# charles-kmc/Semi-blind-image-deblurring-problems-with-TV

Hardware: AMD Instinct MI355X
Metric: SALSA outer-iters/sec + final PSNR, 2048x2048 Gaussian blur (higher is better)
Workload: dtype f64; 1 GPU; SALSA_v2 TV deblur, one 2048x2048 image per GPU, Gaussian PSF 7x7, BSNR 30 dB, TViters=10; images_per_gpu=1, parallelism=images x1

## Files before the change

semi-blind-image-deblurring-problems-with-tv_amd/csrc/ctx.hip:

```cpp
#include <chrono>
#include <cmath>
#include <cstring>
#include <algorithm>
#include <mutex>
#include <thread>
#include <vector>

#include "sbtv_internal.h"

namespace sbtv {

static std::string g_error;
static std::mutex g_error_mu;

void set_global_error(const std::string &msg) {
    std::lock_guard<std::mutex> lk(g_error_mu);
    g_error = msg;
}

int fail(sbtv_ctx *ctx, int code, const std::string &msg) {
    if (ctx) ctx->err = msg;
    set_global_error(msg);
    return code;
}
// ... 348 lines not shown
    const int rc = init();
    if (rc != 0) {
        const std::string msg = ctx->err;
        (void)sbtv_ctx_destroy(ctx);
        return fail(nullptr, rc, msg);
    }
    *out = ctx;
    return 0;
}

int sbtv_ctx_destroy(sbtv_ctx *ctx) {
    if (!ctx) return 0;
    if (ctx->lanes) (void)sbtv_group_destroy(ctx->lanes);
    ctx->lanes = nullptr;
    (void)hipSetDevice(ctx->device);
    if (ctx->stream) (void)hipStreamSynchronize(ctx->stream);
    for (auto &kv : ctx->ws)
        if (kv.second.base) (void)hipFree(kv.second.base);
    if (ctx->canary_desc) (void)hipFree(ctx->canary_desc);
    if (ctx->canary_bad) (void)hipFree(ctx->canary_bad);
    for (auto &kv : ctx->twiddles) (void)hipFree(kv.second);
    for (auto &kv : ctx->any_axes) (void)hipFree(kv.second);
    if (ctx->pinned) (void)hipHostFree(ctx->pinned);
    for (auto &l : ctx->stage) {
        for (int k = 0; k < 2; ++k) {
            if (l.pin[k]) (void)hipHostFree(l.pin[k]);
            if (l.ev[k]) (void)hipEventDestroy(l.ev[k]);
        }
        if (l.s) (void)hipStreamDestroy(l.s);
    }
    for (auto &ev : ctx->ev)
        if (ev) (void)hipEventDestroy(ev);
    for (auto &ev : ctx->loop_ev)
        if (ev) (void)hipEventDestroy(ev);
    if (ctx->own_stream && ctx->stream) (void)hipStreamDestroy(ctx->stream);
    delete ctx;
    return 0;
}

int sbtv_ctx_set_stream(sbtv_ctx *ctx, void *hip_stream) {
    if (!ctx) return SBTV_ERR_BADARG;
    SBTV_HIP(ctx, hipSetDevice(ctx->device));
    SBTV_HIP(ctx, hipStreamSynchronize(ctx->stream));
    if (hip_stream == nullptr) {
        if (!ctx->own_stream) {
            SBTV_HIP(ctx, hipStreamCreateWithFlags(&ctx->stream, hipStreamNonBlocking));
            ctx->own_stream = true;
        }
        return 0;
    }
    if (ctx->own_stream && ctx->stream) SBTV_HIP(ctx, hipStreamDestroy(ctx->stream));
    ctx->stream = (hipStream_t)hip_stream;
    ctx->own_stream = false;
    return 0;
}

int sbtv_ctx_sync(sbtv_ctx *ctx) {
    if (!ctx) return SBTV_ERR_BADARG;
    SBTV_HIP(ctx, hipStreamSynchronize(ctx->stream));
    return 0;
}

int sbtv_callcounter_get(const sbtv_ctx *ctx, long long *calls) {
    if (!ctx || !calls) return SBTV_ERR_BADARG;
    *calls = ctx->calls;
    return 0;
}

int sbtv_callcounter_reset(sbtv_ctx *ctx) {
    if (!ctx) return SBTV_ERR_BADARG;
    ctx->calls = 0;
    return 0;
}

int sbtv_last_timing(const sbtv_ctx *ctx, double out[4]) {
    if (!ctx || !out) return SBTV_ERR_BADARG;
    for (int i = 0; i < 4; ++i) out[i] = ctx->timing[i];
    return 0;
}

int sbtv_last_host_stats(const sbtv_ctx *ctx, double out[14]) {
    if (!ctx || !out) return SBTV_ERR_BADARG;
    const HostStats &h = ctx->hstat;
    const double v[14] = {h.waits, h.ready_at_once, h.waits_slept, h.sleeps, h.stream_queries,
                          h.wait_s, h.wait_max_s, h.enqueue_s, h.enqueue_max_s, h.wait_max_outer,
                          h.nvcsw, h.nivcsw, h.minflt, h.majflt};
    for (int i = 0; i < 14; ++i) out[i] = v[i];
    return 0;
}

int sbtv_host_transpose(const double *src, double *dst, int batch, int rows, int cols) {
    if (!src || !dst || batch < 0 || rows < 0 || cols < 0) return SBTV_ERR_BADARG;
    constexpr int BS = 64;
    const long long nbr = ((long long)rows + BS - 1) / BS;
    const long long jobs = nbr * batch;
    auto work = [&](int t, int T) {
        for (long long job = t; job < jobs; job += T) {
            const int b = (int)(job / nbr), r0 = (int)(job % nbr) * BS, r1 = std::min(rows, r0 + BS);
            const double *s = src + (size_t)b * rows * cols;
            double *d = dst + (size_t)b * rows * cols;
            for (int c0 = 0; c0 < cols; c0 += BS) {
                const int c1 = std::min(cols, c0 + BS);
                for (int c = c0; c < c1; ++c)
                    for (int r = r0; r < r1; ++r) d[(size_t)c * rows + r] = s[(size_t)r * cols + c];
            }
        }
    };
    const size_t bytes = (size_t)batch * rows * cols * sizeof(double);
    const int T = bytes >= ((size_t)4 << 20) ? 4 : 1;
    std::vector<std::thread> th;
    int started = 1;
    try {
        for (int t = 1; t < T; ++t, ++started) th.emplace_back(work, t, T);
    } catch (...) {
    }
    work(0, T);
    for (auto &x : th) x.join();
    for (int t = started; t < T; ++t) work(t, T);
    return 0;
}

int sbtv_diag_solve_stats(const sbtv_ctx *ctx, double out[4]) {
    if (!ctx || !out) return SBTV_ERR_BADARG;
    for (int i = 0; i < 4; ++i) out[i] = ctx->solve_stats[i];
    if (ctx->lanes)
        for (int r = 0; r < sbtv_group_size(ctx->lanes); ++r)
            for (int i = 0; i < 4; ++i) out[i] += sbtv_group_ctx(ctx->lanes, r)->solve_stats[i];
    return 0;
}

int sbtv_diag_stage_stats(const sbtv_ctx *ctx, double out[4]) {
    if (!ctx || !out) return SBTV_ERR_BADARG;
    for (int i = 0; i < 4; ++i) out[i] = ctx->stage_stats[i];
    if (ctx->lanes)
        for (int r = 0; r < sbtv_group_size(ctx->lanes); ++r)
            for (int i = 0; i < 4; ++i) out[i] += sbtv_group_ctx(ctx->lanes, r)->stage_stats[i];
    return 0;
}

int sbtv_diag_workspace(sbtv_ctx *ctx, const char *name, void **dptr, size_t *bytes) {
    if (!ctx || !name || !dptr) return SBTV_ERR_BADARG;
    auto it = ctx->ws.find(name);
    if (it == ctx->ws.end() || !it->second.p) return fail(ctx, SBTV_ERR_BADARG, std::string("no workspace named '") + name + "'");
    *dptr = it->second.p;
    if (bytes) *bytes = it->second.bytes;
    return 0;
}

int sbtv_diag_switches(char *buf, size_t cap) {
    static const char *const names[] = {
        "SBTV_CANARY", "SBTV_COLLECT_RIDE", "SBTV_EXACT", "SBTV_FFT_WAVE", "SBTV_FISTA_FUSED_STEP", "SBTV_FISTA_LAG",
        "SBTV_FUSED_VARIANT", "SBTV_GRAPH", "SBTV_INLINE_CTRL", "SBTV_PROX_SPEC", "SBTV_SAPG_DEFER",
        "SBTV_SAPG_FUSED_MYULA", "SBTV_SAPG_HOST", "SBTV_SINGLE_STEP", "SBTV_SPIN", "SBTV_TAG_SPIN_US", "SBTV_TILE_ORDER", "SBTV_SALSA_NOX", "SBTV_CSALSA_SPECTRAL",
        "SBTV_CORAL_BATCH", "SBTV_ROWS_FOLD", "SBTV_ERR_SUBSET", "SBTV_LANES", "SBTV_LANE_COUNT", "SBTV_STAGE_THREADS", "SBTV_TEST_FAIL_SAPG", "SBTV_FUSED_STAGGER"};
    if (!buf || cap == 0) return SBTV_ERR_BADARG;
    std::string s;
    int nset = 0;
    for (const char *n : names)
        if (const char *e = getenv(n)) {
            s += (nset++ ? " " : "");
            s += n;
            s += "=";
            s += e;
        }
    if (s.size() + 1 > cap) s.resize(cap - 1);
    memcpy(buf, s.c_str(), s.size() + 1);
    return nset;
}

int sbtv_diag_canary(sbtv_ctx *ctx, int poke, int *enabled, int *nbuf, int *nbad) {
    if (!ctx) return SBTV_ERR_BADARG;
    SBTV_HIP(ctx, hipSetDevice(ctx->device));
    if (enabled) *enabled = ctx->canary ? 1 : 0;
    int nb = 0, bad = 0;
    if (ctx->canary && poke) {
        for (auto &kv : ctx->ws)
            if (kv.second.base) {
                SBTV_HIP(ctx, hipMemsetAsync(static_cast<unsigned char *>(kv.second.p) + kv.second.bytes, 0, 8, ctx->stream));
                break;
            }
    }
    std::string name;
    SBTV_TRY(canary_verify(ctx, &nb, &bad, &name));
    if (ctx->canary && poke && bad) {
        for (auto &kv : ctx->ws)
            if (kv.second.base) {
                SBTV_HIP(ctx, hipMemsetAsync(static_cast<unsigned char *>(kv.second.p) + kv.second.bytes, kGuardByte, kGuard, ctx->stream));
                break;
            }
        SBTV_HIP(ctx, hipStreamSynchronize(ctx->stream));
    }
    if (nbuf) *nbuf = nb;
    if (nbad) *nbad = bad;
    return 0;
}

int sbtv_malloc(sbtv_ctx *ctx, size_t bytes, void **dptr) {
    if (!ctx || !dptr) return SBTV_ERR_BADARG;
    SBTV_HIP(ctx, hipSetDevice(ctx->device));
    SBTV_HIP(ctx, hipMalloc(dptr, bytes));
    return 0;
}

int sbtv_free(sbtv_ctx *ctx, void *dptr) {
    if (!ctx) return SBTV_ERR_BADARG;
    SBTV_HIP(ctx, hipStreamSynchronize(ctx->stream));
    SBTV_HIP(ctx, hipFree(dptr));
    return 0;
}

int sbtv_memcpy_h2d(sbtv_ctx *ctx, void *dst, const void *src, size_t bytes) {
    if (!ctx) return SBTV_ERR_BADARG;
    SBTV_HIP(ctx, hipSetDevice(ctx->device));
    if (stage_threaded(bytes)) {
        SBTV_HIP(ctx, hipStreamSynchronize(ctx->stream));
        return stage_copy(ctx, dst, src, bytes, true);
    }
    SBTV_HIP(ctx, hipMemcpyAsync(dst, src, bytes, hipMemcpyHostToDevice, ctx->stream));
    SBTV_HIP(ctx, hipStreamSynchronize(ctx->stream));
    return 0;
}

int sbtv_memcpy_d2h(sbtv_ctx *ctx, void *dst, const void *src, size_t bytes) {
    if (!ctx) return SBTV_ERR_BADARG;
    SBTV_HIP(ctx, hipSetDevice(ctx->device));
    if (stage_threaded(bytes)) {
        SBTV_HIP(ctx, hipStreamSynchronize(ctx->stream));
        return stage_copy(ctx, dst, src, bytes, false);
    }
    SBTV_HIP(ctx, hipMemcpyAsync(dst, src, bytes, hipMemcpyDeviceToHost, ctx->stream));
    SBTV_HIP(ctx, hipStreamSynchronize(ctx->stream));
    return 0;
}

static double spectral_norm_sq(const double *D, int t) {
    double B[15 * 15];
    for (int i = 0; i < t; ++i)
        for (int j = 0; j < t; ++j) {
            double s = 0.0;
            for (int k = 0; k < t; ++k) s += D[i * t + k] * D[j * t + k];
            B[i * t + j] = s;
        }
    for (int sweep = 0; sweep < 60; ++sweep) {
        double off = 0.0, diag = 0.0;
        for (int i = 0; i < t; ++i)
            for (int j = 0; j < t; ++j) (i == j ? diag : off) += B[i * t + j] * B[i * t + j];
        if (off <= 1e-34 * diag || off == 0.0) break;
        for (int p = 0; p < t - 1; ++p)
            for (int q = p + 1; q < t; ++q) {
                const double apq = B[p * t + q];
                if (apq == 0.0) continue;
                const double theta = (B[q * t + q] - B[p * t + p]) / (2.0 * apq);
                const double tt = (theta >= 0 ? 1.0 : -1.0) / (fabs(theta) + sqrt(theta * theta + 1.0));
                const double cs = 1.0 / sqrt(tt * tt + 1.0), sn = tt * cs;
                for (int k = 0; k < t; ++k) {
                    const double bkp = B[k * t + p], bkq = B[k * t + q];
                    B[k * t + p] = cs * bkp - sn * bkq;
                    B[k * t + q] = sn * bkp + cs * bkq;
                }
                for (int k = 0; k < t; ++k) {
                    const double bpk = B[p * t + k], bqk = B[q * t + k];
                    B[p * t + k] = cs * bpk - sn * bqk;
                    B[q * t + k] = sn * bpk + cs * bqk;
                }
            }
    }
    double mx = 0.0;
    for (int i = 0; i < t; ++i) mx = fmax(mx, B[i * t + i]);
    return mx;
}

int sbtv_err_psf(int kind, int taille, const double *ps, int n, const double *p_true, double phi, double *out) {
    if (kind < 0 || kind > 2 || taille < 1 || taille > 15 || !ps || !p_true || !out || n < 1)
        return fail(nullptr, SBTV_ERR_PSF, "sbtv_err_psf: bad arguments");
    const int t2 = taille * taille;
    double truth[225], cur[225], D[225];
    double pt[3] = {p_true[0], kind == SBTV_PSF_LAPLACE ? 0.0 : p_true[1], kind == SBTV_PSF_GAUSSIAN ? phi : 0.0};
    int rc = sbtv_psf_taps(kind, taille, pt, truth, nullptr, nullptr);
    if (rc != 0) return rc;
    for (int i = 0; i < n; ++i) {
        if (kind == SBTV_PSF_MOFFAT && i == 0) {
            out[0] = 0.0;
            continue;
        }
        double p[3] = {ps[i], 0.0, kind == SBTV_PSF_GAUSSIAN ? phi : 0.0};
        if (kind == SBTV_PSF_GAUSSIAN) p[1] = ps[n + (i > 0 ? i - 1 : 0)];
        if (kind == SBTV_PSF_MOFFAT) p[1] = ps[n + i];
        rc = sbtv_psf_taps(kind, taille, p, cur, nullptr, nullptr);
        if (rc != 0) return rc;
        for (int q = 0; q < t2; ++q) D[q] = cur[q] - truth[q];
        out[i] = spectral_norm_sq(D, taille);
    }
    return 0;
}

int sbtv_psf_taps(int kind, int taille, const double *p, double *taps, double *d0, double *d1) {
    if (taille < 1 || taille > 15 || !p || !taps)
        return fail(nullptr, SBTV_ERR_PSF, "sbtv_psf_taps: bad arguments (1 <= taille <= 15)");
    const int t = taille;
    if (kind != SBTV_PSF_GAUSSIAN && kind != SBTV_PSF_MOFFAT && kind != SBTV_PSF_LAPLACE)
        return fail(nullptr, SBTV_ERR_PSF, "sbtv_psf_taps: unknown PSF kind");
    std::vector<double> f(t * t), e0(t * t, 0.0), e1(t * t, 0.0);
    double s = 0, s0 = 0, s1 = 0;
    for (int q = 0; q < t * t; ++q) psf_taps_point(kind, t, p, q, &f[q], &e0[q], &e1[q]);
    for (int q = 0; q < t * t; ++q) { s += f[q]; s0 += e0[q]; s1 += e1[q]; }
    for (int q = 0; q < t * t; ++q) {
        taps[q] = f[q] / s;
// ... 8 lines not shown
```

semi-blind-image-deblurring-problems-with-tv_amd/csrc/elementwise.hip:

```cpp
#include "sbtv_internal.h"

#pragma clang fp contract(off)

namespace sbtv {

constexpr int EWB = 256;

__device__ __forceinline__ double ew_wave_sum(double v) {
#pragma unroll
    for (int off = 32; off > 0; off >>= 1) v += __shfl_xor(v, off, 64);
    return v;
}

template <int NQ>
__device__ __forceinline__ void ew_block_sum(double (&v)[NQ], double *red ) {
    const int lane = threadIdx.x & 63, w = threadIdx.x >> 6;
#pragma unroll
    for (int c = 0; c < NQ; ++c) {
        const double a = ew_wave_sum(v[c]);
        if (lane == 0) red[c * 4 + w] = a;
    }
    __syncthreads();
    if (threadIdx.x == 0) {
#pragma unroll
        for (int c = 0; c < NQ; ++c) v[c] = (red[c * 4] + red[c * 4 + 1]) + (red[c * 4 + 2] + red[c * 4 + 3]);
    }
}

int ew_blocks(size_t P) {
    size_t nb = (P / 2 + EWB - 1) / EWB;
    if (nb > 1024) nb = 1024;
    if (nb < 1) nb = 1;
    return (int)nb;
}

__global__ __launch_bounds__(EWB) void salsa_zero_start_kernel(const double *__restrict__ y, const double *__restrict__ tru,
                                                                double *__restrict__ x, double *__restrict__ u,
                                                                double *__restrict__ bu, double *__restrict__ accp,
                                                                double *__restrict__ postp, size_t P, double scale) {
    const int b = blockIdx.y;
    __shared__ double red[2 * 4];
    const size_t base = (size_t)b * P;
    double acc[2] = {0, 0};
    for (size_t q = (size_t)blockIdx.x * EWB + threadIdx.x; q < P; q += (size_t)gridDim.x * EWB) {
        const double yv = y[base + q];
        const double tv = tru ? tru[base + q] : 0.0;
        acc[0] += yv * yv;
        acc[1] += tv * tv;
        x[base + q] = 0.0;
        u[base + q] = 0.0;
        bu[base + q] = 0.0;
    }
    ew_block_sum<2>(acc, red);
    if (threadIdx.x == 0) {
        const size_t G = gridDim.x;
        for (int q = 0; q < 3; ++q) accp[((size_t)b * 3 + q) * G + blockIdx.x] = (q == 0) ? acc[0] * scale : 0.0;
        for (int q = 0; q < 6; ++q) postp[((size_t)b * 6 + q) * G + blockIdx.x] = (q == 0) ? acc[1] : 0.0;
    }
}

__global__ __launch_bounds__(EWB) void pair_sums_kernel(const double *__restrict__ a, const double *__restrict__ c,
                                                         double *__restrict__ partials, size_t P) {
    const int b = blockIdx.y;
    __shared__ double red[3 * 4];
    __shared__ double redm[4];
    const size_t base = (size_t)b * P;
    double acc[3] = {0, 0, 0};
    double mx = -1.0e308;
    for (size_t q = (size_t)blockIdx.x * EWB + threadIdx.x; q < P; q += (size_t)gridDim.x * EWB) {
        const double av = a[base + q];
        const double cv = c ? c[base + q] : 0.0;
        const double d = av - cv;
        acc[0] += d * d;
        acc[1] += av * av;
        acc[2] += cv * cv;
        mx = fmax(mx, av);
    }
    for (int off = 32; off > 0; off >>= 1) mx = fmax(mx, __shfl_xor(mx, off, 64));
    if ((threadIdx.x & 63) == 0) redm[threadIdx.x >> 6] = mx;
    ew_block_sum<3>(acc, red);
    if (threadIdx.x == 0) {
        for (int q = 0; q < 3; ++q) partials[((size_t)b * 4 + q) * gridDim.x + blockIdx.x] = acc[q];
        partials[((size_t)b * 4 + 3) * gridDim.x + blockIdx.x] = fmax(fmax(redm[0], redm[1]), fmax(redm[2], redm[3]));
    }
}

__global__ __launch_bounds__(256) void reduce_max_kernel(const double *__restrict__ partials, int n,
                                                          double *__restrict__ out) {
    __shared__ double redm[4];
    const double *p = partials + (size_t)blockIdx.x * n;
    double mx = -1.0e308;
    for (int q = threadIdx.x; q < n; q += 256) mx = fmax(mx, p[q]);
    for (int off = 32; off > 0; off >>= 1) mx = fmax(mx, __shfl_xor(mx, off, 64));
    if ((threadIdx.x & 63) == 0) redm[threadIdx.x >> 6] = mx;
    __syncthreads();
    if (threadIdx.x == 0) out[blockIdx.x] = fmax(fmax(redm[0], redm[1]), fmax(redm[2], redm[3]));
}

__global__ __launch_bounds__(EWB) void axpy_kernel(double *__restrict__ y, const double *__restrict__ gr, double a,
                                                    size_t Ptot, ProxArm arm, int batch) {
    if (arm.ctrl && blockIdx.x == 0 && (int)threadIdx.x < batch) {
        const int b = threadIdx.x;
        ProxCtrl c = arm.ctrl[b];
        c.k = 0;
        c.done = (arm.frozen && arm.frozen[b]) ? 1 : 0;
        c.cur = 0;
        c.maxiter = arm.maxiter;
        c.redo = 0;
        c.f_valid = 0;
        c.err = 0.0;
        c.lambda = arm.lambda[b];
        c.tol = arm.tol;
        c.tau = arm.tau;
        arm.ctrl[b] = c;
    }
    for (size_t q = (size_t)blockIdx.x * EWB + threadIdx.x; q < Ptot / 2; q += (size_t)gridDim.x * EWB) {
        double2 yv = *reinterpret_cast<double2 *>(y + 2 * q);
        const double2 gv = *reinterpret_cast<const double2 *>(gr + 2 * q);
        yv.x = yv.x - a * gv.x;
        yv.y = yv.y - a * gv.y;
        *reinterpret_cast<double2 *>(y + 2 * q) = yv;
    }
}
__global__ __launch_bounds__(EWB) void fista_momentum_kernel(const double *__restrict__ x, const double *__restrict__ xold,
                                                              double *__restrict__ y, const double *__restrict__ tru,
                                                              double c, double *__restrict__ partials, size_t P,
                                                              const int *__restrict__ frozen) {
    const int b = blockIdx.y;
    if (frozen && frozen[b]) return;
    __shared__ double red[3 * 4];
    const size_t base = (size_t)b * P;
    double acc[3] = {0, 0, 0};
    for (size_t q = (size_t)blockIdx.x * EWB + threadIdx.x; q < P / 2; q += (size_t)gridDim.x * EWB) {
        const size_t o = base + 2 * q;
        const double2 xv = *reinterpret_cast<const double2 *>(x + o);
        const double2 xo = *reinterpret_cast<const double2 *>(xold + o);
        const double d0 = xv.x - xo.x, d1 = xv.y - xo.y;
        *reinterpret_cast<double2 *>(y + o) = make_double2(xv.x + c * d0, xv.y + c * d1);
        if (tru) {
            const double2 tv = *reinterpret_cast<const double2 *>(tru + o);
            const double e0 = xv.x - tv.x, e1 = xv.y - tv.y;
            acc[0] += e0 * e0 + e1 * e1;
        }
        acc[1] += d0 * d0 + d1 * d1;
        acc[2] += xv.x * xv.x + xv.y * xv.y;
    }
    ew_block_sum<3>(acc, red);
    if (threadIdx.x == 0)
        for (int q = 0; q < 3; ++q) partials[((size_t)b * 3 + q) * gridDim.x + blockIdx.x] = acc[q];
}

template <bool MOM>
__global__ __launch_bounds__(EWB) void myula_step_kernel(double *__restrict__ X, const double *__restrict__ prox,
                                                          const double *__restrict__ grad,
                                                          const double *__restrict__ Z,
                                                          const double *__restrict__ sigma2, double gam, double lamb,
                                                          double sq2g, size_t P, RngArgs rng, ProxArm arm, MomArgs mom) {
    const int b = blockIdx.y;
    if (arm.ctrl && blockIdx.x == 0 && threadIdx.x == 0) {
        ProxCtrl c = arm.ctrl[b];
        c.k = 0;
        c.done = 0;
        c.cur = 0;
        c.maxiter = arm.maxiter;
        c.redo = 0;
        c.f_valid = 0;
        c.err = 0.0;
        c.lambda = arm.lambda[b];
        c.tol = arm.tol;
        c.tau = arm.tau;
        arm.ctrl[b] = c;
    }
    const size_t base = (size_t)b * P;
    const double s2 = sigma2[b];
    const unsigned step = rng.step_dev ? (unsigned)rng.step_dev[0] : rng.step;
    const int k = MOM ? mom_sample(mom) : 0;
    const double rk = 1.0 / (double)(k > 0 ? k : 1);
    for (size_t q = (size_t)blockIdx.x * EWB + threadIdx.x; q < P / 2; q += (size_t)gridDim.x * EWB) {
        const size_t o = base + 2 * q;
        const double2 xv = *reinterpret_cast<const double2 *>(X + o);
        const double2 pv = *reinterpret_cast<const double2 *>(prox + o);
        const double2 gv = *reinterpret_cast<const double2 *>(grad + o);
        const double2 zv = Z ? *reinterpret_cast<const double2 *>(Z + o)
                             : philox_normal_pair(q, step, rng.chain0 + (unsigned)b, rng.seed);
        double2 r;
        r.x = myula_nocontract(xv.x, pv.x, gv.x, 1.0, zv.x, gam, lamb, s2, sq2g);
        r.y = myula_nocontract(xv.y, pv.y, gv.y, 1.0, zv.y, gam, lamb, s2, sq2g);
        *reinterpret_cast<double2 *>(X + o) = r;
        if (MOM && k > 0) moments_pair(mom, o, r, k, rk);
    }
}

template <bool MOM>
__global__ __launch_bounds__(EWB) void myula_plain_kernel(double *__restrict__ X, const double *__restrict__ prox,
                                                           const double *__restrict__ grad,
                                                           const double *__restrict__ Z,
                                                           const double *__restrict__ sigma2, double gam, double lamb,
                                                           double sq2g, size_t P, RngArgs rng, ProxArm arm, MomArgs mom) {
    const int b = blockIdx.y;
    if (arm.ctrl && blockIdx.x == 0 && threadIdx.x == 0) {
        ProxCtrl c = arm.ctrl[b];
        c.k = 0;
        c.done = 0;
        c.cur = 0;
        c.maxiter = arm.maxiter;
        c.redo = 0;
        c.f_valid = 0;
        c.err = 0.0;
        c.lambda = arm.lambda[b];
        c.tol = arm.tol;
        c.tau = arm.tau;
        arm.ctrl[b] = c;
    }
    const size_t base = (size_t)b * P;
    const double s2 = sigma2[b], keep = 1.0 - gam / lamb;
    const int k = MOM ? mom_sample(mom) : 0;
    const double rk = 1.0 / (double)(k > 0 ? k : 1);
    for (size_t q = (size_t)blockIdx.x * EWB + threadIdx.x; q < P / 2; q += (size_t)gridDim.x * EWB) {
        const size_t o = base + 2 * q;
        const double2 xv = *reinterpret_cast<const double2 *>(X + o);
        const double2 pv = *reinterpret_cast<const double2 *>(prox + o);
        const double2 gv = *reinterpret_cast<const double2 *>(grad + o);
        const double2 zv = Z ? *reinterpret_cast<const double2 *>(Z + o)
                             : philox_normal_pair(q, rng.step, rng.chain0 + (unsigned)b, rng.seed);
        double2 r;
        r.x = (keep * xv.x - gam * (gv.x / s2 - pv.x / lamb)) + sq2g * zv.x;
        r.y = (keep * xv.y - gam * (gv.y / s2 - pv.y / lamb)) + sq2g * zv.y;
        *reinterpret_cast<double2 *>(X + o) = r;
        if (MOM && k > 0) moments_pair(mom, o, r, k, rk);
    }
}

__global__ __launch_bounds__(EWB) void moments_seed_kernel(const double *__restrict__ X, double *__restrict__ mean,
                                                           double *__restrict__ m2, size_t n2) {
    const MomArgs m{mean, m2, 1, nullptr, 1, 1};
    for (size_t q = (size_t)blockIdx.x * EWB + threadIdx.x; q < n2; q += (size_t)gridDim.x * EWB)
        moments_pair(m, 2 * q, *reinterpret_cast<const double2 *>(X + 2 * q), 1, 1.0);
}

__global__ __launch_bounds__(EWB) void moments_finish_kernel(const double *__restrict__ mean, const double *__restrict__ m2,
                                                             size_t P, int batch, double n, int pooled, int raw,
                                                             double *__restrict__ mean_out, double *__restrict__ var_out) {
#pragma clang fp contract(off)
    const int b = blockIdx.y;
    for (size_t i = (size_t)blockIdx.x * EWB + threadIdx.x; i < P; i += (size_t)gridDim.x * EWB) {
        double mu = mean[(size_t)b * P + i], s = m2[(size_t)b * P + i], na = n;
        if (pooled) {
            for (int c = 1; c < batch; ++c) {
                const double mb = mean[(size_t)c * P + i], sb = m2[(size_t)c * P + i];
                const double nt = na + n, d = mb - mu;
                mu = mu + d * (n / nt);
                s = (s + sb) + d * d * (na * n / nt);
                na = nt;
            }
        }
        mean_out[(size_t)b * P + i] = mu;
        if (var_out) var_out[(size_t)b * P + i] = raw ? s : (na > 1.0 ? s / (na - 1.0) : 0.0);
    }
}

int myula_plain_step(sbtv_ctx *ctx, double *X, const double *prox, const double *grad, const double *Z,
                     const double *sigma2_dev, double gam, double lamb, size_t P, int batch, const RngArgs *rng,
                     const ProxArm *arm, const MomArgs *mom) {
    if (!Z && !rng) return fail(ctx, SBTV_ERR_BADARG, "myula_plain_step: neither a noise array nor generator arguments");
    const RngArgs r = rng ? *rng : RngArgs{0ull, 0u, 0u, nullptr};
    const ProxArm pa = arm ? *arm : ProxArm{nullptr, nullptr, 0, 0.0, 0.0, nullptr};
    if (mom)
        hipLaunchKernelGGL(myula_plain_kernel<true>, dim3(ew_blocks(P), batch), dim3(EWB), 0, ctx->stream, X, prox, grad, Z,
                           sigma2_dev, gam, lamb, sqrt(2 * gam), P, r, pa, *mom);
    else
        hipLaunchKernelGGL(myula_plain_kernel<false>, dim3(ew_blocks(P), batch), dim3(EWB), 0, ctx->stream, X, prox, grad, Z,
                           sigma2_dev, gam, lamb, sqrt(2 * gam), P, r, pa, MomArgs{});
    SBTV_HIP(ctx, hipGetLastError());
    return 0;
}

int moments_seed(sbtv_ctx *ctx, const double *X, double *mean, double *m2, size_t P, int batch) {
    const size_t n = P * batch;
    hipLaunchKernelGGL(moments_seed_kernel, dim3(ew_blocks(n)), dim3(EWB), 0, ctx->stream, X, mean, m2, n / 2);
    SBTV_HIP(ctx, hipGetLastError());
    return 0;
}

int moments_finish(sbtv_ctx *ctx, const double *mean, const double *m2, size_t P, int batch, long long n, const MomReq &req) {
    const int pooled = req.pooled && !req.raw;
    const size_t nout = P * (pooled ? 1 : batch);
    double *mo = nullptr, *vo = nullptr;
    const int fl = req.dev ? SBTV_DEVICE_PTRS : SBTV_HOST_PTRS;
    SBTV_TRY(stage_out_buf(ctx, "mom.mean_out", req.mean, nout, fl, &mo));
    if (req.var) SBTV_TRY(stage_out_buf(ctx, "mom.var_out", req.var, nout, fl, &vo));
    hipLaunchKernelGGL(moments_finish_kernel, dim3(ew_blocks(2 * P), pooled ? 1 : batch), dim3(EWB), 0, ctx->stream, mean,
                       m2, P, batch, (double)n, pooled, req.raw ? 1 : 0, mo, vo);
    SBTV_HIP(ctx, hipGetLastError());
    SBTV_TRY(stage_out_copy(ctx, req.mean, mo, nout, fl));
    if (req.var) SBTV_TRY(stage_out_copy(ctx, req.var, vo, nout, fl));
    if (req.count)
        for (size_t c = 0; c < (pooled ? 1 : (size_t)batch); ++c) req.count[c] = pooled ? n * batch : n;
    return 0;
}

int pair_sums(sbtv_ctx *ctx, const double *a, const double *c, size_t P, int batch, double *out4_dev) {
    const int nb = ew_blocks(P);
    double *partials = nullptr;
    SBTV_TRY(ws_get_t(ctx, "ew.pair.partials", (size_t)batch * 4 * nb, &partials));
    hipLaunchKernelGGL(pair_sums_kernel, dim3(nb, batch), dim3(EWB), 0, ctx->stream, a, c, partials, P);
    SBTV_HIP(ctx, hipGetLastError());
    for (int b = 0; b < batch; ++b) {
        SBTV_TRY(reduce_partials(ctx, partials + (size_t)b * 4 * nb, 3, nb, out4_dev + (size_t)b * 4));
        hipLaunchKernelGGL(reduce_max_kernel, dim3(1), dim3(256), 0, ctx->stream, partials + ((size_t)b * 4 + 3) * nb,
                           nb, out4_dev + (size_t)b * 4 + 3);
    }
    SBTV_HIP(ctx, hipGetLastError());
    return 0;
}

int salsa_zero_start(sbtv_ctx *ctx, const double *y, const double *tru, double *x, double *u, double *bu, size_t P, int batch,
                     double scale, double **accp, double **postp, int *nblk) {
    const int G = ew_blocks(2 * P);
    SBTV_TRY(ws_get_t(ctx, "ew.zero.acc", (size_t)batch * 3 * G, accp));
    SBTV_TRY(ws_get_t(ctx, "ew.zero.post", (size_t)batch * 6 * G, postp));
    hipLaunchKernelGGL(salsa_zero_start_kernel, dim3(G, batch), dim3(EWB), 0, ctx->stream, y, tru, x, u, bu, *accp, *postp, P,
                       scale);
    SBTV_HIP(ctx, hipGetLastError());
    *nblk = G;
    return 0;
}

int axpy(sbtv_ctx *ctx, double *y, const double *gr, double a, size_t Ptot, const ProxArm *arm, int batch) {
    if (arm && batch > EWB) return fail(ctx, SBTV_ERR_BADARG, "axpy: cannot arm more than 256 control blocks");
    const ProxArm pa = arm ? *arm : ProxArm{nullptr, nullptr, 0, 0.0, 0.0, nullptr};
    hipLaunchKernelGGL(axpy_kernel, dim3(ew_blocks(Ptot)), dim3(EWB), 0, ctx->stream, y, gr, a, Ptot, pa, batch);
    SBTV_HIP(ctx, hipGetLastError());
    return 0;
}

int fista_momentum(sbtv_ctx *ctx, const double *x, const double *xold, double *y, const double *tru, double coef,
                   double *partials, size_t P, int batch, const int *frozen) {
    hipLaunchKernelGGL(fista_momentum_kernel, dim3(ew_blocks(P), batch), dim3(EWB), 0, ctx->stream, x, xold, y, tru,
                       coef, partials, P, frozen);
    SBTV_HIP(ctx, hipGetLastError());
    return 0;
}

int myula_step(sbtv_ctx *ctx, double *X, const double *prox, const double *grad, const double *Z,
               const double *sigma2_dev, double gam, double lamb, size_t P, int batch, const RngArgs *rng,
               const ProxArm *arm, const MomArgs *mom) {
    if (!Z && !rng) return fail(ctx, SBTV_ERR_BADARG, "myula_step: neither a noise array nor generator arguments");
    const RngArgs r = rng ? *rng : RngArgs{0ull, 0u, 0u, nullptr};
    const ProxArm pa = arm ? *arm : ProxArm{nullptr, nullptr, 0, 0.0, 0.0, nullptr};
    if (mom)
        hipLaunchKernelGGL(myula_step_kernel<true>, dim3(ew_blocks(P), batch), dim3(EWB), 0, ctx->stream, X, prox, grad, Z,
                           sigma2_dev, gam, lamb, sqrt(2 * gam), P, r, pa, *mom);
    else
        hipLaunchKernelGGL(myula_step_kernel<false>, dim3(ew_blocks(P), batch), dim3(EWB), 0, ctx->stream, X, prox, grad, Z,
                           sigma2_dev, gam, lamb, sqrt(2 * gam), P, r, pa, MomArgs{});
    SBTV_HIP(ctx, hipGetLastError());
    return 0;
}

}

using namespace sbtv;

extern "C" {

static int metric_common(sbtv_ctx *ctx, const double *x_true, const double *x, int M, int N, int batch, double *out,
                         int flags, bool psnr) {
    if (!ctx) return SBTV_ERR_BADARG;
    if (!x_true || !x || !out || M < 1 || N < 1 || batch < 1) return fail(ctx, SBTV_ERR_BADARG, "metric: bad arguments");
    SBTV_HIP(ctx, hipSetDevice(ctx->device));
    const size_t P = (size_t)M * N;
    const double *a = nullptr, *c = nullptr;
    SBTV_TRY(stage_in(ctx, "metric.a", x_true, P * batch, flags, &a));
    SBTV_TRY(stage_in(ctx, "metric.c", x, P * batch, flags, &c));
    double *o4 = nullptr;
    SBTV_TRY(ws_get_t(ctx, "metric.out", (size_t)batch * 4, &o4));
    SBTV_TRY(pair_sums(ctx, a, c, P, batch, o4));
    std::vector<double> h((size_t)batch * 4);
    SBTV_HIP(ctx, hipMemcpyAsync(h.data(), o4, sizeof(double) * batch * 4, hipMemcpyDeviceToHost, ctx->stream));
    SBTV_HIP(ctx, hipStreamSynchronize(ctx->stream));
    for (int b = 0; b < batch; ++b) {
        const double se = h[(size_t)b * 4], mx = h[(size_t)b * 4 + 3];
        if (psnr)
            out[b] = 10 * log10(mx * mx) - 10 * log10(se / (double)P);
        else
            out[b] = 10 * log10(se / (double)P);
    }
    return canary_epilogue(ctx, 0);
}

int sbtv_PSNR(sbtv_ctx *ctx, const double *x_true, const double *x, int M, int N, int batch, double *out, int flags) {
    return metric_common(ctx, x_true, x, M, N, batch, out, flags, true);
}
int sbtv_MSE(sbtv_ctx *ctx, const double *x_true, const double *x, int M, int N, int batch, double *out, int flags) {
    return metric_common(ctx, x_true, x, M, N, batch, out, flags, false);
}

}
```

semi-blind-image-deblurring-problems-with-tv_amd/csrc/fft.hip:

```cpp
#include <type_traits>

#include "sbtv_internal.h"

namespace sbtv {

__device__ __forceinline__ double2 cadd(double2 a, double2 b) { return make_double2(a.x + b.x, a.y + b.y); }
__device__ __forceinline__ double2 csub(double2 a, double2 b) { return make_double2(a.x - b.x, a.y - b.y); }
__device__ __forceinline__ double2 cmul(double2 a, double2 b) {
    return make_double2(a.x * b.x - a.y * b.y, a.x * b.y + a.y * b.x);
}
__device__ __forceinline__ double2 cmulc(double2 a, double2 b) {
    return make_double2(a.x * b.x + a.y * b.y, a.y * b.x - a.x * b.y);
}
__device__ __forceinline__ double2 cconj(double2 a) { return make_double2(a.x, -a.y); }
__device__ __forceinline__ double2 cscale(double2 a, double s) { return make_double2(a.x * s, a.y * s); }
__device__ __forceinline__ double cabs2(double2 a) { return a.x * a.x + a.y * a.y; }

constexpr int TWS = 2;
constexpr int TW = 1 << TWS;
__device__ __forceinline__ size_t s_tiled(int k, int l, int n1) {
    return (((size_t)(l >> TWS) * n1 + k) << TWS) + (l & (TW - 1));
}
__device__ __forceinline__ size_t u_tiled(int k, int l, int n1) { return ((size_t)(l >> TWS) * (n1 + 1) + k) * TW + (l & (TW - 1)); }

// ... 839 lines not shown
    hipLaunchKernelGGL((fft_cols_inv_kernel<L, true>), dim3(cd.wgs, pl.batch), dim3(cd.threads), 0,
                       ctx->stream, S, x, pl.tw_n1, pl.tw_M, pl.N, scale, frozen, post);
}

#define SBTV_DISPATCH_LOG2(L, CALL)                                    \
    switch (L) {                                                       \
        case 3: CALL(3); break;                                        \
        case 4: CALL(4); break;                                        \
        case 5: CALL(5); break;                                        \
        case 6: CALL(6); break;                                        \
        case 7: CALL(7); break;                                        \
        case 8: CALL(8); break;                                        \
        case 9: CALL(9); break;                                        \
        case 10: CALL(10); break;                                      \
        case 11: CALL(11); break;                                      \
        default: return fail(ctx, SBTV_ERR_SIZE, "unsupported FFT length"); \
    }

bool fft_cols_tv_ok(const FftPlan &pl) { return !pl.generic; }
int fft_cols_fwd_f(sbtv_ctx *ctx, const FftPlan &pl, const double *x, const double *add, double2 *S,
                   const int *frozen, double *tvp) {
    if (tvp && (!fft_cols_tv_ok(pl) || add)) return fail(ctx, SBTV_ERR_BADARG, "fft_cols_fwd: TV partials not available for this call");
    if (pl.generic) return any_cols_fwd(ctx, pl, x, add, S, frozen);
    if (pl.wave) {
        const PassDims cd = cols_dims(pl);
        const dim3 grid(cd.wgs, pl.batch), block(cd.threads);
        if (pl.n1 == 1024)
            hipLaunchKernelGGL((cols_fwd_wave_kernel<10, 16>), grid, block, 0, ctx->stream, x, add, S, pl.tw_n1, pl.tw_M,
                               pl.N, frozen, tvp);
        else
            hipLaunchKernelGGL((cols_fwd_wave_kernel<9, 8>), grid, block, 0, ctx->stream, x, add, S, pl.tw_n1, pl.tw_M,
                               pl.N, frozen, tvp);
        SBTV_HIP(ctx, hipGetLastError());
        return 0;
    }
    const int L = ilog2(pl.n1);
#define CALL(LL) launch_cols_fwd<LL>(ctx, pl, x, add, S, frozen, tvp)
    SBTV_DISPATCH_LOG2(L, CALL)
#undef CALL
    SBTV_HIP(ctx, hipGetLastError());
    return 0;
}
int fft_cols_fwd(sbtv_ctx *ctx, const FftPlan &pl, const double *x, const double *add, double2 *S) {
    return fft_cols_fwd_f(ctx, pl, x, add, S, nullptr, nullptr);
}

int fft_cols_inv_f(sbtv_ctx *ctx, const FftPlan &pl, const double2 *S, double *x, double scale, const int *frozen) {
    if (pl.generic) return any_cols_inv(ctx, pl, S, x, scale, frozen, nullptr);
    if (pl.wave) {
        const PassDims cd = cols_dims(pl);
        const dim3 grid(cd.wgs, pl.batch), block(cd.threads);
        if (pl.n1 == 1024)
            hipLaunchKernelGGL((cols_inv_wave_kernel<10, 16, 0>), grid, block, 0, ctx->stream, S, x, pl.tw_n1,
                               pl.tw_M, pl.N, scale, frozen, ColsPost{});
        else
            hipLaunchKernelGGL((cols_inv_wave_kernel<9, 8, 0>), grid, block, 0, ctx->stream, S, x, pl.tw_n1, pl.tw_M,
                               pl.N, scale, frozen, ColsPost{});
        SBTV_HIP(ctx, hipGetLastError());
        return 0;
    }
    const int L = ilog2(pl.n1);
#define CALL(LL) launch_cols_inv<LL>(ctx, pl, S, x, scale, frozen)
    SBTV_DISPATCH_LOG2(L, CALL)
#undef CALL
    SBTV_HIP(ctx, hipGetLastError());
    return 0;
}
bool fft_cols_inv_step_ok(const FftPlan &pl) { return !pl.generic && pl.wave; }
static int fft_cols_step_check(sbtv_ctx *ctx, const FftPlan &pl, const char *who) {
    if (!fft_cols_inv_step_ok(pl)) return fail(ctx, SBTV_ERR_BADARG, std::string(who) + ": size not on the wave-granular path");
    return 0;
}
int fft_cols_inv_step(sbtv_ctx *ctx, const FftPlan &pl, const double2 *S, double *y, double scale, double alpha,
                      const int *frozen) {
    SBTV_TRY(fft_cols_step_check(ctx, pl, "fft_cols_inv_step"));
    ColsPost post;
    post.ystep = y;
    post.alpha = alpha;
    const PassDims cd = cols_dims(pl);
        const dim3 grid(cd.wgs, pl.batch), block(cd.threads);
    if (pl.n1 == 1024)
        hipLaunchKernelGGL((cols_inv_wave_kernel<10, 16, 8>), grid, block, 0, ctx->stream, S, (double *)nullptr, pl.tw_n1,
                           pl.tw_M, pl.N, scale, frozen, post);
    else
        hipLaunchKernelGGL((cols_inv_wave_kernel<9, 8, 8>), grid, block, 0, ctx->stream, S, (double *)nullptr, pl.tw_n1, pl.tw_M,
                           pl.N, scale, frozen, post);
    SBTV_HIP(ctx, hipGetLastError());
    return 0;
}
int fft_cols_inv_sub(sbtv_ctx *ctx, const FftPlan &pl, const double2 *S, double *x, double scale, const double *b, double *g) {
    SBTV_TRY(fft_cols_step_check(ctx, pl, "fft_cols_inv_sub"));
    ColsPost post;
    post.bu_in = b;
    post.g = g;
    const PassDims cd = cols_dims(pl);
        const dim3 grid(cd.wgs, pl.batch), block(cd.threads);
    if (pl.n1 == 1024)
        hipLaunchKernelGGL((cols_inv_wave_kernel<10, 16, 64>), grid, block, 0, ctx->stream, S, x, pl.tw_n1, pl.tw_M, pl.N, scale,
                           (const int *)nullptr, post);
    else
        hipLaunchKernelGGL((cols_inv_wave_kernel<9, 8, 64>), grid, block, 0, ctx->stream, S, x, pl.tw_n1, pl.tw_M, pl.N, scale,
                           (const int *)nullptr, post);
    SBTV_HIP(ctx, hipGetLastError());
    return 0;
}
int fft_cols_inv_myula(sbtv_ctx *ctx, const FftPlan &pl, const double2 *S, double scale, double *X, const double *prox,
                       const double *Z, const double *sigma2_dev, double gam, double lamb, const RngArgs *rng,
                       const ProxArm *arm, const MomArgs *mom) {
    SBTV_TRY(fft_cols_step_check(ctx, pl, "fft_cols_inv_myula"));
    if (!Z && !rng) return fail(ctx, SBTV_ERR_BADARG, "fft_cols_inv_myula: neither a noise array nor generator arguments");
    ColsPost post;
    post.ystep = X;
    post.mprox = prox;
    post.mZ = Z;
    post.msig2 = sigma2_dev;
    post.mgam = gam;
    post.mlamb = lamb;
    post.msq2g = sqrt(2 * gam);
    if (rng) post.mrng = *rng;
    if (arm) post.marm = *arm;
    const PassDims cd = cols_dims(pl);
        const dim3 grid(cd.wgs, pl.batch), block(cd.threads);
    if (mom) {
        post.mom = *mom;
        if (pl.n1 == 1024)
            hipLaunchKernelGGL((cols_inv_wave_kernel<10, 16, 16 | 128>), grid, block, 0, ctx->stream, S, (double *)nullptr,
                               pl.tw_n1, pl.tw_M, pl.N, scale, (const int *)nullptr, post);
        else
            hipLaunchKernelGGL((cols_inv_wave_kernel<9, 8, 16 | 128>), grid, block, 0, ctx->stream, S, (double *)nullptr,
                               pl.tw_n1, pl.tw_M, pl.N, scale, (const int *)nullptr, post);
    } else if (pl.n1 == 1024)
        hipLaunchKernelGGL((cols_inv_wave_kernel<10, 16, 16>), grid, block, 0, ctx->stream, S, (double *)nullptr, pl.tw_n1,
                           pl.tw_M, pl.N, scale, (const int *)nullptr, post);
    else
        hipLaunchKernelGGL((cols_inv_wave_kernel<9, 8, 16>), grid, block, 0, ctx->stream, S, (double *)nullptr, pl.tw_n1, pl.tw_M,
                           pl.N, scale, (const int *)nullptr, post);
    SBTV_HIP(ctx, hipGetLastError());
    return 0;
}
int fft_cols_inv(sbtv_ctx *ctx, const FftPlan &pl, const double2 *S, double *x, double scale) {
    return fft_cols_inv_f(ctx, pl, S, x, scale, nullptr);
}
int fft_cols_blocks(const FftPlan &pl) { return (pl.wave || pl.generic) ? pl.N : pl.N / cols_nseq(pl); }
int fft_cols_inv_post(sbtv_ctx *ctx, const FftPlan &pl, const double2 *S, double *x, double scale, const int *frozen,
                      const ColsPost &post) {
    if ((!pl.wave && (post.bu_in || post.skip_x)) || (post.bu_in && !post.skip_x))
        return fail(ctx, SBTV_ERR_BADARG, "fft_cols_inv_post: bu_in + skip_x go together and need the wave-granular column pass");
    if (pl.generic) return any_cols_inv(ctx, pl, S, x, scale, frozen, &post);
    if (pl.wave) {
        const PassDims cd = cols_dims(pl);
        const dim3 grid(cd.wgs, pl.batch), block(cd.threads);
        if (post.skip_x && (!post.bu_in || post.bu_in == post.bu || post.xprev))
            return fail(ctx, SBTV_ERR_BADARG, "fft_cols_inv_post: skip_x needs a separate bu_in and no xprev");
        const int pm = 1 + (post.tru ? 2 : 0) + (post.xprev ? 4 : 0) + (post.skip_x ? 32 : 0);
#define SBTV_POST_CASE(PM_)                                                                                          \
    case PM_:                                                                                                        \
        if (pl.n1 == 1024)                                                                                           \
            hipLaunchKernelGGL((cols_inv_wave_kernel<10, 16, PM_>), grid, block, 0, ctx->stream, S, x, pl.tw_n1,       \
                               pl.tw_M, pl.N, scale, frozen, post);                                                  \
        else                                                                                                         \
            hipLaunchKernelGGL((cols_inv_wave_kernel<9, 8, PM_>), grid, block, 0, ctx->stream, S, x, pl.tw_n1,         \
                               pl.tw_M, pl.N, scale, frozen, post);                                                  \
        break;
        switch (pm) {
            SBTV_POST_CASE(1)
            SBTV_POST_CASE(3)
            SBTV_POST_CASE(5)
            SBTV_POST_CASE(7)
            SBTV_POST_CASE(33)
            SBTV_POST_CASE(35)
        }
#undef SBTV_POST_CASE
        SBTV_HIP(ctx, hipGetLastError());
        return 0;
    }
    const int L = ilog2(pl.n1);
#define CALL(LL) launch_cols_inv_post<LL>(ctx, pl, S, x, scale, frozen, post)
    SBTV_DISPATCH_LOG2(L, CALL)
#undef CALL
    SBTV_HIP(ctx, hipGetLastError());
    return 0;
}

static inline int rows_rk(const FftPlan &pl) {
    const int N = pl.N;
    if (N == 4096) return 2;
    const int rk = (N >= 512) ? 4 : 8;
    const int small = (N == 512) ? 1 : (N == 256) ? 2 : rk;
    return (pl.n1 / rk < 128) ? small : rk;
}
static inline PassDims rows_dims(const FftPlan &pl) {
    if (pl.generic) return {0, ANY_SPEC_THREADS, ANY_SPEC_BLOCKS};
    if (pl.wave) return {4, pl.N / 4, pl.n1 / 4};
    const int rk = rows_rk(pl);
    return {rk, rk * (pl.N / 8), pl.n1 / rk};
}
bool fft_rows_csalsa_ok(const FftPlan &pl) { return !pl.generic; }
static int fft_rows_check(sbtv_ctx *ctx, const FftPlan &pl, int op) {
    if (op == OP_CSALSA && !fft_rows_csalsa_ok(pl)) return fail(ctx, SBTV_ERR_SIZE, "row pass: OP_CSALSA is not built for this plan");
    return 0;
}
int fft_rows_blocks(const FftPlan &pl) {
    return rows_dims(pl).wgs;
}

static inline bool rows_fold_ok(const FftPlan &pl, int shared_spec) {
    static const bool fold_wanted = [] {
        const char *e = getenv("SBTV_ROWS_FOLD");
        return !(e && e[0] == '0');
    }();
    return fold_wanted && pl.wave && shared_spec && pl.batch > 1 && ((pl.n1 / 4) % 8 == 0);
}
template <int L>
static void launch_rows_pipe(sbtv_ctx *ctx, const FftPlan &pl, const RowsParams &p0) {
    RowsParams p = p0;
    const bool fold = rows_fold_ok(pl, p.shared_spec);
    p.fold = fold ? pl.batch : 0;
    const PassDims rd = rows_dims(pl);
    const dim3 grid(fold ? rd.wgs * pl.batch : rd.wgs, fold ? 1 : pl.batch), block(rd.threads);
#define SBTV_ROWS_OP(OP_)                                                                                     \
    case OP_: hipLaunchKernelGGL((rows_pipe_kernel<L, OP_>), grid, block, 0, ctx->stream, p); break;
    switch (p.op) {
        SBTV_ROWS_OP(OP_NONE)
        SBTV_ROWS_OP(OP_MUL_H)
        SBTV_ROWS_OP(OP_MUL_HC)
        SBTV_ROWS_OP(OP_INVLS)
        SBTV_ROWS_OP(OP_SALSA)
        SBTV_ROWS_OP(OP_RESID)
        SBTV_ROWS_OP(OP_GRAD)
        SBTV_ROWS_OP(OP_ATA)
        SBTV_ROWS_OP(OP_GRADF)
        SBTV_ROWS_OP(OP_CSALSA)
        default: break;
    }
#undef SBTV_ROWS_OP
}

template <int L, int RK>
static void launch_rows(sbtv_ctx *ctx, const FftPlan &pl, const RowsParams &p) {
    const PassDims rd = rows_dims(pl);
    const dim3 grid(rd.wgs, pl.batch), block(rd.threads);
#define SBTV_ROWS_OP(OP_)                                                                                     \
    case OP_: hipLaunchKernelGGL((fft_rows_kernel<L, RK, OP_>), grid, block, 0, ctx->stream, p); break;
    switch (p.op) {
        SBTV_ROWS_OP(OP_NONE)
        SBTV_ROWS_OP(OP_MUL_H)
        SBTV_ROWS_OP(OP_MUL_HC)
        SBTV_ROWS_OP(OP_INVLS)
        SBTV_ROWS_OP(OP_SALSA)
        SBTV_ROWS_OP(OP_RESID)
        SBTV_ROWS_OP(OP_GRAD)
        SBTV_ROWS_OP(OP_ATA)
        SBTV_ROWS_OP(OP_GRADF)
        SBTV_ROWS_OP(OP_CSALSA)
        default: break;
    }
#undef SBTV_ROWS_OP
}

int fft_rows(sbtv_ctx *ctx, const FftPlan &pl, const double2 *Sin, double2 *Sout, const RowsArgs &a) {
    RowsParams p;
    p.Sin = Sin;
    p.Sout = Sout;
    p.tw = pl.tw_N;
    p.H = a.H;
    p.Y = a.Y;
    p.D1 = a.D1;
    p.D2 = a.D2;
    p.E = a.E;
    p.cs = a.cs;
    p.mu = a.mu;
    p.acc = a.acc;
    p.frozen = a.frozen;
    p.n1 = pl.n1;
    p.fwd = a.dir_fwd;
    p.inv = a.dir_inv;
    p.op = a.op;
    p.shared_spec = a.shared_spec;
    p.fold = 0;
    p.u_img = pl.u_img;
    p.u_tiled = pl.u_tiled;
    SBTV_TRY(fft_rows_check(ctx, pl, a.op));
    if (pl.generic) return any_rows(ctx, pl, p, Sout);
    const int L = ilog2(pl.N);
    if (L > 12) return fail(ctx, SBTV_ERR_SIZE, "row FFT: N must be <= 4096");
    if (pl.wave) {
        if (L == 11) launch_rows_pipe<11>(ctx, pl, p);
        else launch_rows_pipe<10>(ctx, pl, p);
        SBTV_HIP(ctx, hipGetLastError());
        return 0;
    }
    if (pl.N >= 512) {
        switch (L) {
            case 9:
                if (rows_rk(pl) == 1) launch_rows<9, 1>(ctx, pl, p);
                else launch_rows<9, 4>(ctx, pl, p);
                break;
            case 10: launch_rows<10, 4>(ctx, pl, p); break;
            case 11: launch_rows<11, 4>(ctx, pl, p); break;
            case 12: launch_rows<12, 2>(ctx, pl, p); break;
            default: break;
        }
    } else {
        switch (L) {
            case 4: launch_rows<4, 8>(ctx, pl, p); break;
            case 5: launch_rows<5, 8>(ctx, pl, p); break;
            case 6: launch_rows<6, 8>(ctx, pl, p); break;
            case 7: launch_rows<7, 8>(ctx, pl, p); break;
            case 8:
                if (rows_rk(pl) == 2) launch_rows<8, 2>(ctx, pl, p);
                else launch_rows<8, 8>(ctx, pl, p);
                break;
            default: return fail(ctx, SBTV_ERR_SIZE, "row FFT: N must be >= 16");
        }
    }
    SBTV_HIP(ctx, hipGetLastError());
    return 0;
}

int spec_unpack(sbtv_ctx *ctx, const FftPlan &pl, const double2 *S, double2 *U) {
    if (pl.generic) {
        SBTV_HIP(ctx, hipMemcpyAsync(U, S, sizeof(double2) * pl.s_img * pl.batch, hipMemcpyDeviceToDevice, ctx->stream));
        return 0;
    }
    if (pl.wave) {
        hipLaunchKernelGGL(spec_unpack_tiled_kernel, dim3((pl.N + 63) / 64, pl.n1 + 1, pl.batch), dim3(64), 0,
                           ctx->stream, S, U, pl.n1, pl.N, pl.u_tiled);
        SBTV_HIP(ctx, hipGetLastError());
        return 0;
    }
    const int thr = 64;
    hipLaunchKernelGGL(spec_unpack_kernel, dim3((pl.n1 + 1 + thr - 1) / thr, pl.N, pl.batch), dim3(thr), 0,
                       ctx->stream, S, U, pl.n1, pl.N);
    SBTV_HIP(ctx, hipGetLastError());
    return 0;
}

static inline int psf_lch(const FftPlan &pl) {
    const size_t elems = (size_t)(pl.n1 + 1) * pl.N * pl.batch;
    const int lch = (int)(elems >> 19);
    return lch < 1 ? 1 : (lch > 16 ? 16 : lch);
}
int psf_spectrum_sets(sbtv_ctx *ctx, const FftPlan &pl, const double *const *taps_dev, int taille, double2 *const *U, int nsets) {
    const int thr = 64;
    if (taille > PSF_TMAX) return fail(ctx, SBTV_ERR_PSF, "PSF larger than 15 x 15");
    if (nsets < 1 || nsets > 3) return fail(ctx, SBTV_ERR_BADARG, "psf_spectrum_sets: 1..3 tap sets");
    if (pl.generic) {
        for (int q = 0; q < nsets; ++q) SBTV_TRY(any_psf_spectrum(ctx, pl, taps_dev[q], taille, U[q]));
        return 0;
    }
    const int lch = psf_lch(pl);
    PsfSets ps{};
    for (int q = 0; q < 3; ++q) {
        ps.taps[q] = taps_dev[q < nsets ? q : 0];
        ps.U[q] = U[q < nsets ? q : 0];
    }
    const dim3 grid = pl.u_tiled ? dim3(((pl.n1 + 1) * 4 + thr - 1) / thr, ((pl.N >> 2) + lch - 1) / lch, pl.batch * nsets)
                                 : dim3((pl.n1 + 1 + thr - 1) / thr, (pl.N + lch - 1) / lch, pl.batch * nsets);
    if (taille == 7)
        hipLaunchKernelGGL(psf_spectrum_kernel<7>, grid, dim3(thr), 0, ctx->stream, ps, taille, pl.batch, pl.n1, pl.M, pl.N,
                           pl.tw_M, pl.tw_N, lch, pl.u_tiled);
    else
        hipLaunchKernelGGL(psf_spectrum_kernel<0>, grid, dim3(thr), 0, ctx->stream, ps, taille, pl.batch, pl.n1, pl.M, pl.N,
                           pl.tw_M, pl.tw_N, lch, pl.u_tiled);
    SBTV_HIP(ctx, hipGetLastError());
    return 0;
}
int psf_spectrum(sbtv_ctx *ctx, const FftPlan &pl, const double *taps_dev, int taille, double2 *U) {
    return psf_spectrum_sets(ctx, pl, &taps_dev, taille, &U, 1);
}

}

using namespace sbtv;

extern "C" {

int sbtv_rfft2_packed(sbtv_ctx *ctx, const double *in, double *out, int M, int N, int batch, int inverse, int flags) {
    if (!ctx) return SBTV_ERR_BADARG;
    if (!in || !out || batch < 1) return fail(ctx, SBTV_ERR_BADARG, "rfft2_packed: bad arguments");
    SBTV_HIP(ctx, hipSetDevice(ctx->device));
    FftPlan pl;
    SBTV_TRY(fft_plan(ctx, M, N, batch, &pl));
    if (pl.generic)
        return fail(ctx, SBTV_ERR_SIZE, "rfft2_packed: the packed half-spectrum format exists for powers of two 16..4096 only");
// ... 397 lines not shown
```

semi-blind-image-deblurring-problems-with-tv_amd/csrc/fft_wave.inc:

```


struct SyncWave {
    static __device__ __forceinline__ void sync() {
        __builtin_amdgcn_fence(__ATOMIC_RELEASE, "wavefront");
        __builtin_amdgcn_wave_barrier();
        __builtin_amdgcn_fence(__ATOMIC_ACQUIRE, "wavefront");
    }
};
struct SyncBlock {
    static __device__ __forceinline__ void sync() { __syncthreads(); }
};

template <class SYNC>
struct XSeq {
    double2 *buf;
    static __device__ __forceinline__ int idx(int pos) { return pos + (pos >> 4); }
    static __device__ __forceinline__ void sync() { SYNC::sync(); }
};
template <class SYNC>
struct XSwz {
    double2 *buf;
    static __device__ __forceinline__ int idx(int pos) {
        const int m = pos >> 4;
        return pos ^ ((m & 7) ^ ((m & 4) << 1));
// ... 59 lines not shown
        } else {
            bfly2<INV>(v[q], v[q + G]);
        }
    }
}

template <int V, int LOG2N, int LOG2NS, int LR, bool INV, class TW>
__device__ __forceinline__ void twiddles_v(double2 (&v)[V], int t, TW tw) {
    if constexpr (LOG2NS > 0) {
        constexpr int T = (1 << LOG2N) / V;
        constexpr int R = 1 << LR, G = V / R;
        constexpr int SH = LOG2N - LOG2NS - LR;
#pragma unroll
        for (int q = 0; q < G; ++q) {
            const int k = (t + q * T) & ((1 << LOG2NS) - 1);
            if constexpr (R == 16) {
                const double2 w1 = twid<INV>(tw, k << SH), w2 = twid<INV>(tw, (2 * k) << SH);
                const double2 w4 = twid<INV>(tw, (4 * k) << SH), w8 = twid<INV>(tw, (8 * k) << SH);
                const double2 w3 = cmul(w1, w2), w5 = cmul(w1, w4), w6 = cmul(w2, w4), w7 = cmul(w3, w4);
                v[q + 1 * G] = cmul(v[q + 1 * G], w1);
                v[q + 2 * G] = cmul(v[q + 2 * G], w2);
                v[q + 3 * G] = cmul(v[q + 3 * G], w3);
                v[q + 4 * G] = cmul(v[q + 4 * G], w4);
                v[q + 5 * G] = cmul(v[q + 5 * G], w5);
                v[q + 6 * G] = cmul(v[q + 6 * G], w6);
                v[q + 7 * G] = cmul(v[q + 7 * G], w7);
                v[q + 8 * G] = cmul(v[q + 8 * G], w8);
                v[q + 9 * G] = cmul(v[q + 9 * G], cmul(w1, w8));
                v[q + 10 * G] = cmul(v[q + 10 * G], cmul(w2, w8));
                v[q + 11 * G] = cmul(v[q + 11 * G], cmul(w3, w8));
                v[q + 12 * G] = cmul(v[q + 12 * G], cmul(w4, w8));
                v[q + 13 * G] = cmul(v[q + 13 * G], cmul(w5, w8));
                v[q + 14 * G] = cmul(v[q + 14 * G], cmul(w6, w8));
                v[q + 15 * G] = cmul(v[q + 15 * G], cmul(w7, w8));
            } else {
#pragma unroll
                for (int r = 1; r < R; ++r) v[q + r * G] = cmul(v[q + r * G], twid<INV>(tw, (r * k) << SH));
            }
        }
    }
}

template <int V, int LOG2N, int LOG2NS, int LR, class X>
__device__ __forceinline__ void exchange_v(double2 (&v)[V], int t, const X &x) {
    constexpr int T = (1 << LOG2N) / V;
    constexpr int R = 1 << LR, G = V / R;
#pragma unroll
    for (int q = 0; q < G; ++q) {
        const int j = t + q * T;
        const int k = j & ((1 << LOG2NS) - 1);
        const int j0 = ((j >> LOG2NS) << (LOG2NS + LR)) + k;
#pragma unroll
        for (int r = 0; r < R; ++r) x.buf[X::idx(j0 + (r << LOG2NS))] = v[q + r * G];
    }
    X::sync();
#pragma unroll
    for (int s = 0; s < V; ++s) v[s] = x.buf[X::idx(t + s * T)];
    X::sync();
}

template <int V, int LOG2N, int LOG2NS, bool INV, class X, class TW>
__device__ __forceinline__ void stages_v(double2 (&v)[V], int t, TW tw, const X &x) {
    constexpr int left = LOG2N - LOG2NS;
    constexpr int LV = (V == 16) ? 4 : 3;
    if constexpr (left > 0) {
        constexpr int LR = left >= LV ? LV : left;
        twiddles_v<V, LOG2N, LOG2NS, LR, INV>(v, t, tw);
        butterflies_v<V, LR, INV>(v);
        if constexpr (left - LR > 0) {
            exchange_v<V, LOG2N, LOG2NS, LR>(v, t, x);
            stages_v<V, LOG2N, LOG2NS + LR, INV>(v, t, tw, x);
        }
    }
}

template <int LOG2N, int V>
__global__ __launch_bounds__(64 * TW, 2) void cols_fwd_wave_kernel(const double *__restrict__ x,
                                                                 const double *__restrict__ add,
                                                                 double2 *__restrict__ S,
                                                                 const double2 *__restrict__ tw_n1,
                                                                 const double2 *__restrict__ tw_M, int N,
                                                                 const int *__restrict__ frozen,
                                                                 double *__restrict__ tvp) {
    constexpr int n = 1 << LOG2N;
    static_assert(n == 64 * V, "one wave per column");
    constexpr int REG = xseq_elems(n);
    __shared__ __attribute__((aligned(16))) double2 lds[TW * REG];
    const int b = blockIdx.y;
    if (frozen && frozen[b]) return;
    const int w = __builtin_amdgcn_readfirstlane(threadIdx.x >> 6), lane = threadIdx.x & 63;
    const int tile = blockIdx.x;
    const int j = tile * TW + w;
    const size_t colbase = ((size_t)b * N + j) * n;
    const double2 *__restrict__ xin = reinterpret_cast<const double2 *>(x) + colbase;
    XSeq<SyncWave> X{lds + w * REG};
    double2 v[V];
#pragma unroll
    for (int s = 0; s < V; ++s) v[s] = xin[lane + s * 64];
    if (tvp) {
        constexpr int M = 2 * n;
        const double *__restrict__ xl = x + ((size_t)b * N + (j > 0 ? j - 1 : N - 1)) * M;
        double carry = __shfl(v[V - 1].y, 63, 64);
        double a = 0.0;
#pragma unroll
        for (int s = 0; s < V; ++s) {
            const double2 ul = *reinterpret_cast<const double2 *>(xl + 2 * (size_t)(lane + s * 64));
            double upv = __shfl_up(v[s].y, 1, 64);
            if (lane == 0) upv = carry;
            carry = __shfl(v[s].y, 63, 64);
            const double h0 = v[s].x - ul.x, v0 = v[s].x - upv, h1 = v[s].y - ul.y, v1 = v[s].y - v[s].x;
            a += sqrt(h0 * h0 + v0 * v0) + sqrt(h1 * h1 + v1 * v1);
        }
#pragma unroll
        for (int off = 32; off > 0; off >>= 1) a += __shfl_xor(a, off, 64);
        if (lane == 0) tvp[(size_t)b * N + j] = a;
    }
    if (add) {
        const double2 *__restrict__ ain = reinterpret_cast<const double2 *>(add) + colbase;
#pragma unroll
        for (int s = 0; s < V; ++s) v[s] = cadd(v[s], ain[lane + s * 64]);
    }
    stages_v<V, LOG2N, 0, false>(v, lane, tw_n1, X);
    SyncWave::sync();
#pragma unroll
    for (int s = 0; s < V; ++s) X.buf[XSeq<SyncWave>::idx(lane + s * 64)] = v[s];
    __syncthreads();
    double2 *__restrict__ out = S + ((size_t)b * (N >> TWS) + tile) * ((size_t)n << TWS);
#pragma unroll
    for (int i = 0; i < V; ++i) {
        const int flat = i * (64 * TW) + threadIdx.x;
        const int k = flat >> TWS, c = flat & (TW - 1);
        const double2 *reg = lds + c * REG;
        const double2 Z = reg[XSeq<SyncWave>::idx(k)];
        const double2 Zm = cconj(reg[XSeq<SyncWave>::idx((n - k) & (n - 1))]);
        double2 r;
        if (k == 0) {
            r = make_double2(Z.x + Z.y, Z.x - Z.y);
        } else {
            const double2 wv = tw_M[k];
            const double2 su = cadd(Z, Zm), di = csub(Z, Zm);
            const double2 wd = cmul(wv, di);
            r = make_double2(0.5 * (su.x + wd.y), 0.5 * (su.y - wd.x));
        }
        out[flat] = r;
    }
}

__device__ __forceinline__ double2 step_nocontract(double2 y, double a, double2 x) {
#pragma clang fp contract(off)
    const double t0 = a * x.x, t1 = a * x.y;
    return make_double2(y.x - t0, y.y - t1);
}

template <int LOG2N, int V, int PM>
__global__ __launch_bounds__(64 * TW, 2) void cols_inv_wave_kernel(const double2 *__restrict__ S, double *__restrict__ x,
                                                                 const double2 *__restrict__ tw_n1,
                                                                 const double2 *__restrict__ tw_M, int N, double scale,
                                                                 const int *__restrict__ frozen, ColsPost post) {
    constexpr int n = 1 << LOG2N;
    constexpr bool POST = (PM & 1) != 0, HAS_TRU = (PM & 2) != 0, HAS_XPREV = (PM & 4) != 0;
    constexpr bool NOX = (PM & 32) != 0;
    static_assert(n == 64 * V, "one wave per column");
    constexpr int REG = xseq_elems(n);
    __shared__ __attribute__((aligned(16))) double2 lds[TW * REG];
    const int b = blockIdx.y;
    if (frozen && frozen[b]) return;
    const int w = __builtin_amdgcn_readfirstlane(threadIdx.x >> 6), lane = threadIdx.x & 63;
    const int tile = blockIdx.x;
    const int j = tile * TW + w;
    const double2 *__restrict__ in = S + ((size_t)b * (N >> TWS) + tile) * ((size_t)n << TWS);
    {
        double2 a[V];
#pragma unroll
        for (int i = 0; i < V; ++i) a[i] = in[i * (64 * TW) + threadIdx.x];
#pragma unroll
        for (int i = 0; i < V; ++i) {
            const int flat = i * (64 * TW) + threadIdx.x;
            lds[(flat & (TW - 1)) * REG + XSeq<SyncWave>::idx(flat >> TWS)] = a[i];
        }
    }
    __syncthreads();
    XSeq<SyncWave> X{lds + w * REG};
    double2 v[V];
#pragma unroll
    for (int s = 0; s < V; ++s) {
        const int e = lane + s * 64;
        const double2 Xk = X.buf[XSeq<SyncWave>::idx(e)];
        const double2 Xm = cconj(X.buf[XSeq<SyncWave>::idx((n - e) & (n - 1))]);
        if (e == 0) {
            v[s] = make_double2(0.5 * (Xk.x + Xk.y), 0.5 * (Xk.x - Xk.y));
        } else {
            const double2 E = cscale(cadd(Xk, Xm), 0.5);
            const double2 O = cmulc(cscale(csub(Xk, Xm), 0.5), tw_M[e]);
            v[s] = make_double2(E.x - O.y, E.y + O.x);
        }
        if ((s & 3) == 3) __builtin_amdgcn_sched_barrier(0);
    }
    SyncWave::sync();
    stages_v<V, LOG2N, 0, true>(v, lane, tw_n1, X);
    const size_t colbase = ((size_t)b * N + j) * n;
    double2 *__restrict__ out = reinterpret_cast<double2 *>(x) + colbase;
    if constexpr (PM == 8) {
        double2 *__restrict__ yp = reinterpret_cast<double2 *>(post.ystep) + colbase;
        double2 yv[V];
#pragma unroll
        for (int s = 0; s < V; ++s) yv[s] = yp[lane + s * 64];
#pragma unroll
        for (int s = 0; s < V; ++s) {
            const double2 xv = cscale(v[s], scale);
            yp[lane + s * 64] = step_nocontract(yv[s], post.alpha, xv);
        }
    } else if constexpr ((PM & ~128) == 16) {
        if (post.marm.ctrl && blockIdx.x == 0 && threadIdx.x == 0) {
            ProxCtrl c = post.marm.ctrl[b];
            c.k = 0;
            c.done = 0;
            c.cur = 0;
            c.maxiter = post.marm.maxiter;
            c.redo = 0;
            c.f_valid = 0;
            c.err = 0.0;
            c.lambda = post.marm.lambda[b];
            c.tol = post.marm.tol;
            c.tau = post.marm.tau;
            post.marm.ctrl[b] = c;
        }
        double2 *__restrict__ xp = reinterpret_cast<double2 *>(post.ystep) + colbase;
        const double2 *__restrict__ pp = reinterpret_cast<const double2 *>(post.mprox) + colbase;
        const double2 *__restrict__ zp = post.mZ ? reinterpret_cast<const double2 *>(post.mZ) + colbase : nullptr;
        const double s2 = post.msig2[b];
        const unsigned step = post.mrng.step_dev ? (unsigned)post.mrng.step_dev[0] : post.mrng.step;
        const size_t q0 = (size_t)j * n;
        constexpr bool MOM = (PM & 128) != 0;
        int mk = 0;
        double mrk = 1.0;
        if constexpr (MOM) {
            mk = mom_sample(post.mom);
            mrk = 1.0 / (double)(mk > 0 ? mk : 1);
        }
        constexpr int CH = 4;
#pragma unroll
        for (int c0 = 0; c0 < V; c0 += CH) {
            double2 xv[CH], pv[CH], zv[CH];
#pragma unroll
            for (int q = 0; q < CH; ++q) {
                const int e = lane + (c0 + q) * 64;
                xv[q] = xp[e];
                pv[q] = pp[e];
                if (zp) zv[q] = zp[e];
            }
#pragma unroll
            for (int q = 0; q < CH; ++q) {
                const int e = lane + (c0 + q) * 64;
                if (!zp) zv[q] = philox_normal_pair(q0 + e, step, post.mrng.chain0 + (unsigned)b, post.mrng.seed);
                const double2 gv = cscale(v[c0 + q], scale);
                double2 r;
                r.x = myula_nocontract(xv[q].x, pv[q].x, gv.x, 1.0, zv[q].x, post.mgam, post.mlamb, s2, post.msq2g);
                r.y = myula_nocontract(xv[q].y, pv[q].y, gv.y, 1.0, zv[q].y, post.mgam, post.mlamb, s2, post.msq2g);
                xp[e] = r;
                if constexpr (MOM)
                    if (mk > 0) moments_pair(post.mom, 2 * (colbase + e), r, mk, mrk);
            }
            __builtin_amdgcn_sched_barrier(0);
        }
    } else if constexpr (PM == 64) {
        const double2 *__restrict__ bp = reinterpret_cast<const double2 *>(post.bu_in) + colbase;
        double2 *__restrict__ gp = reinterpret_cast<double2 *>(post.g) + colbase;
        double2 bb[V];
#pragma unroll
        for (int s = 0; s < V; ++s) bb[s] = bp[lane + s * 64];
#pragma unroll
        for (int s = 0; s < V; ++s) {
            const double2 xv = cscale(v[s], scale);
            out[lane + s * 64] = xv;
            gp[lane + s * 64] = make_double2(xv.x - bb[s].x, xv.y - bb[s].y);
        }
    } else if constexpr (!POST) {
#pragma unroll
        for (int s = 0; s < V; ++s) out[lane + s * 64] = cscale(v[s], scale);
    } else {
        constexpr int M = 2 * n;
        const size_t ibase = (size_t)b * N * M;
        const size_t cb = ibase + (size_t)j * M;
        const size_t cl = ibase + (size_t)(j > 0 ? j - 1 : N - 1) * M;
        const double *__restrict__ up_ = post.u + cb + 2 * lane, *__restrict__ ulp = post.u + cl + 2 * lane;
        double *__restrict__ bup = post.bu + cb + 2 * lane, *__restrict__ gp = post.g + cb + 2 * lane;
        const double *__restrict__ bin = NOX ? post.bu_in + cb + 2 * lane : nullptr;
        const double *__restrict__ trp = HAS_TRU ? post.tru + cb + 2 * lane : nullptr;
        const double *__restrict__ xpp = HAS_XPREV ? post.xprev + cb + 2 * lane : nullptr;
        double acc[6] = {0.0, 0.0, 0.0, 0.0, 0.0, 0.0};
        constexpr int CH = 2, NCH = V / CH;
        double2 ub[2][CH], bb[2][CH], tb[2][CH], lb[2][CH], xb[2][CH];
        auto fetch = [&](int c, int slot) {
#pragma unroll
            for (int q = 0; q < CH; ++q) {
                const int off = (c * CH + q) * 128;
                ub[slot][q] = *reinterpret_cast<const double2 *>(up_ + off);
                bb[slot][q] = *reinterpret_cast<const double2 *>((NOX ? bin : (const double *)bup) + off);
                lb[slot][q] = *reinterpret_cast<const double2 *>(ulp + off);
                if constexpr (HAS_TRU) tb[slot][q] = nt_load2(trp + off);
                if constexpr (HAS_XPREV) xb[slot][q] = *reinterpret_cast<const double2 *>(xpp + off);
            }
        };
        __builtin_amdgcn_sched_barrier(0);
        double carry = post.u[cb + M - 1];
        fetch(0, 0);
#pragma unroll
        for (int c = 0; c < NCH; ++c) {
            if (c + 1 < NCH) fetch(c + 1, (c + 1) & 1);
            __builtin_amdgcn_sched_barrier(0);
#pragma unroll
            for (int q = 0; q < CH; ++q) {
                const int s = c * CH + q, off = s * 128;
                const double2 xv = cscale(v[s], scale);
                if constexpr (!NOX) nt_store2(reinterpret_cast<double *>(out + lane + s * 64), xv);
                const double2 uv = ub[c & 1][q], ul = lb[c & 1][q];
                double2 bv = bb[c & 1][q];
                bv.x = bv.x + (uv.x - xv.x);
                bv.y = bv.y + (uv.y - xv.y);
                *reinterpret_cast<double2 *>(bup + off) = bv;
                *reinterpret_cast<double2 *>(gp + off) = make_double2(xv.x - bv.x, xv.y - bv.y);
                if constexpr (HAS_TRU) {
                    const double2 tv = tb[c & 1][q];
                    const double e0 = xv.x - tv.x, e1 = xv.y - tv.y;
                    acc[0] += e0 * e0 + e1 * e1;
                }
                const double d0 = xv.x - uv.x, d1 = xv.y - uv.y;
                acc[1] += d0 * d0 + d1 * d1;
                acc[2] += xv.x * xv.x + xv.y * xv.y;
                acc[3] += uv.x * uv.x + uv.y * uv.y;
                if constexpr (HAS_XPREV) {
                    const double2 xo = xb[c & 1][q];
                    const double p0 = xv.x - xo.x, p1 = xv.y - xo.y;
                    acc[4] += p0 * p0 + p1 * p1;
                }
                double upv = __shfl_up(uv.y, 1, 64);
                if (lane == 0) upv = carry;
                carry = __shfl(uv.y, 63, 64);
                const double h0 = uv.x - ul.x, v0 = uv.x - upv, h1 = uv.y - ul.y, v1 = uv.y - uv.x;
                acc[5] += sqrt(h0 * h0 + v0 * v0) + sqrt(h1 * h1 + v1 * v1);
            }
            __builtin_amdgcn_sched_barrier(0);
        }
#pragma unroll
        for (int c = 0; c < 6; ++c) {
#pragma unroll
            for (int off = 32; off > 0; off >>= 1) acc[c] += __shfl_xor(acc[c], off, 64);
        }
        if (lane == 0) {
#pragma unroll
            for (int c = 0; c < 6; ++c) post.partials[((size_t)b * 6 + c) * N + j] = acc[c];
        }
    }
}

template <int LOG2N, int OP>
__global__ __launch_bounds__((1 << LOG2N) / 4, 1) void rows_pipe_kernel(RowsParams p) {
    constexpr int N = 1 << LOG2N, V = 8, T = N / V, RK = 2, NT = RK * T, NW = NT / 64;
    constexpr int REG = N;
    constexpr bool needH = (OP != OP_NONE);
    constexpr bool CS = (OP == OP_CSALSA);
    constexpr bool needY = (OP == OP_SALSA || OP == OP_RESID || OP == OP_GRADF || OP == OP_GRAD || CS);
    constexpr bool needD = (OP == OP_GRAD);
    constexpr bool needD1 = needD || CS, noAhead = needD || CS;
#ifndef SBTV_CS_LATE_Y
#define SBTV_CS_LATE_Y 1
#endif
    constexpr bool lateY = CS && (SBTV_CS_LATE_Y != 0) && LOG2N == 11;
    __shared__ __attribute__((aligned(16))) double2 lds[RK * REG];
    __shared__ __attribute__((aligned(16))) double2 twl_buf[LdsTw::elems(N)];
    const LdsTw twl{twl_buf};
    __shared__ double red[3 * NW];
    const int fold = p.fold;
    const int ntk = fold ? (int)gridDim.x / fold : (int)gridDim.x;
    int b = blockIdx.y;
    int kb;
    {
        const int bid = blockIdx.x, xx = bid & 7;
        int o = bid >> 3;
        if (fold) {
            b = o % fold;
            o /= fold;
        }
        const int q8 = ntk >> 3, r8 = ntk & 7;
        kb = (xx < r8 ? xx * (q8 + 1) : r8 * (q8 + 1) + (xx - r8) * q8) + o;
    }
    if (p.frozen && p.frozen[b]) return;
    const int q = (threadIdx.x >> 5) & 1, t = (threadIdx.x & 31) | ((threadIdx.x >> 6) << 5);
    const int n1 = p.n1;
    const int k0 = kb * RK + q, k1 = (n1 >> 1) + kb * RK + q;
    const size_t ibase = (size_t)b * n1 * N;
    const double2 *__restrict__ in = p.Sin + ibase;
    double2 *__restrict__ out = p.Sout ? p.Sout + ibase : nullptr;
    XSwz<SyncBlock> X{lds + q * REG};
    const size_t hbase = p.shared_spec ? 0 : (size_t)b * p.u_img;
    const double mu = p.mu ? p.mu[b] : 0.0;
    const double2 z = make_double2(0.0, 0.0);
    const int sb = p.u_tiled ? 1 : n1 + 1, sc = p.u_tiled ? TW : 1;
    auto uidx = [&](int kk, int l) -> size_t {
        return hbase + (size_t)(l >> TWS) * (TW * (n1 + 1)) + (size_t)((l & (TW - 1)) * sb + kk * sc);
    };
    for (int i = threadIdx.x; i < N; i += NT) twl_buf[LdsTw::idx(i)] = p.tw[i];
    __syncthreads();

    double2 v[V], sn[V], h[V], y[V], d1[needD1 ? V : 1], d2[needD ? V : 1];
    if constexpr (!needD1) d1[0] = z;
    const CsPar cp = CS ? CsPar{p.cs[0], p.cs[1], p.cs[2]} : CsPar{0.0, 0.0, 0.0};
    auto apply = [&](double2 V_, double2 H_, double2 Y_, double2 &E_, double2 D2_, double wgt, double (&acc_)[3]) -> double2 {
        if constexpr (CS) return spec_apply_cs(V_, H_, Y_, E_, mu, cp, wgt, acc_);
        else return spec_apply<OP>(V_, H_, Y_, E_, D2_, mu, wgt, acc_);
    };
    auto dd1 = [&](int s) -> double2 & { return d1[needD1 ? s : 0]; };
    auto dd2 = [&](int s) -> double2 { return needD ? d2[needD ? s : 0] : z; };
#pragma unroll
    for (int s = 0; s < V; ++s) v[s] = in[s_tiled(k0, t + s * T, n1)];
    if constexpr (needH) {
#pragma unroll
        for (int s = 0; s < V; ++s) {
            h[s] = p.H[uidx(k0, t + s * T)];
            if constexpr (needY && !lateY) y[s] = p.Y[uidx(k0, t + s * T)];
            if constexpr (needD) {
                d1[s] = p.D1[uidx(k0, t + s * T)];
                d2[s] = p.D2[uidx(k0, t + s * T)];
            }
            if constexpr (CS) d1[s] = p.E[uidx(k0, t + s * T)];
        }
    }
    if constexpr (!noAhead) {
#pragma unroll
        for (int s = 0; s < V; ++s) sn[s] = in[s_tiled(k1, t + s * T, n1)];
    }
    double acc[3] = {0.0, 0.0, 0.0};

    if (p.fwd) stages_v<V, LOG2N, 0, false>(v, t, twl, X);
    if constexpr (lateY) {
#pragma unroll
        for (int s = 0; s < V; ++s) y[s] = p.Y[uidx(k0, t + s * T)];
    }
    if constexpr (needH) {
        if (kb == 0) {
#pragma unroll
            for (int s = 0; s < V; ++s) X.buf[XSwz<SyncBlock>::idx(t + s * T)] = v[s];
            SyncBlock::sync();
#pragma unroll
            for (int s = 0; s < V; ++s) {
                const int l = t + s * T;
                if (q == 0) {
                    const size_t hn = uidx(n1, l);
                    const double2 P = v[s], Q = cconj(X.buf[XSwz<SyncBlock>::idx((N - l) & (N - 1))]);
                    const double2 A = cscale(cadd(P, Q), 0.5);
                    const double2 dB = csub(P, Q);
                    const double2 B = make_double2(0.5 * dB.y, -0.5 * dB.x);
                    double2 en = needD ? p.D1[hn] : (CS ? p.E[hn] : z);
                    const double2 A2 = apply(A, h[s], needY ? y[s] : z, dd1(s), dd2(s), 1.0, acc);
                    const double2 B2 = apply(B, p.H[hn], needY ? p.Y[hn] : z, en, needD ? p.D2[hn] : z, 1.0, acc);
                    if constexpr (CS) p.E[hn] = en;
                    v[s] = make_double2(A2.x - B2.y, A2.y + B2.x);
                } else {
                    v[s] = apply(v[s], h[s], needY ? y[s] : z, dd1(s), dd2(s), 2.0, acc);
                }
                if constexpr (CS) p.E[uidx(k0, t + s * T)] = d1[s];
            }
            SyncBlock::sync();
        } else {
#pragma unroll
            for (int s = 0; s < V; ++s) {
                v[s] = apply(v[s], h[s], needY ? y[s] : z, dd1(s), dd2(s), 2.0, acc);
                if constexpr (CS) p.E[uidx(k0, t + s * T)] = d1[s];
            }
        }
        asm volatile("" : "+v"(acc[0]), "+v"(acc[1]), "+v"(acc[2]));
#pragma unroll
        for (int s = 0; s < V; ++s) {
            h[s] = p.H[uidx(k1, t + s * T)];
            if constexpr (needY && !lateY) y[s] = p.Y[uidx(k1, t + s * T)];
            if constexpr (needD) {
                d1[s] = p.D1[uidx(k1, t + s * T)];
                d2[s] = p.D2[uidx(k1, t + s * T)];
            }
            if constexpr (CS) d1[s] = p.E[uidx(k1, t + s * T)];
        }
    }
    if (p.inv) stages_v<V, LOG2N, 0, true>(v, t, twl, X);
    int ts = t;
    asm volatile("" : "+v"(ts));
    if (out) {
#pragma unroll
        for (int s = 0; s < V; ++s) out[s_tiled(k0, ts + s * T, n1)] = v[s];
    }
#pragma unroll
    for (int s = 0; s < V; ++s) v[s] = noAhead ? in[s_tiled(k1, t + s * T, n1)] : sn[s];
    if (p.fwd) stages_v<V, LOG2N, 0, false>(v, t, twl, X);
    if constexpr (lateY) {
#pragma unroll
        for (int s = 0; s < V; ++s) y[s] = p.Y[uidx(k1, t + s * T)];
    }
    if constexpr (needH) {
#pragma unroll
        for (int s = 0; s < V; ++s) {
            v[s] = apply(v[s], h[s], needY ? y[s] : z, dd1(s), dd2(s), 2.0, acc);
            if constexpr (CS) p.E[uidx(k1, t + s * T)] = d1[s];
        }
        asm volatile("" : "+v"(acc[0]), "+v"(acc[1]), "+v"(acc[2]));
    }
    if (p.inv) stages_v<V, LOG2N, 0, true>(v, t, twl, X);
    asm volatile("" : "+v"(ts));
    if (out) {
#pragma unroll
        for (int s = 0; s < V; ++s) out[s_tiled(k1, ts + s * T, n1)] = v[s];
    }
    if constexpr (needY) {
        const int lane = threadIdx.x & 63, w = threadIdx.x >> 6;
#pragma unroll
        for (int c = 0; c < 3; ++c) {
#pragma unroll
            for (int off = 32; off > 0; off >>= 1) acc[c] += __shfl_xor(acc[c], off, 64);
        }
        if (lane == 0) {
#pragma unroll
            for (int c = 0; c < 3; ++c) red[c * NW + w] = acc[c];
        }
        __syncthreads();
        if (threadIdx.x < 3) {
            double a = 0.0;
            for (int ww = 0; ww < NW; ++ww) a += red[threadIdx.x * NW + ww];
            p.acc[((size_t)b * 3 + threadIdx.x) * ntk + kb] = a;
        }
    }
}

__global__ void s_relayout_kernel(const double2 *__restrict__ in, double2 *__restrict__ out, int n1, int N, int to_tiled) {
    const size_t per = (size_t)n1 * N;
    const double2 *ib = in + (size_t)blockIdx.y * per;
    double2 *ob = out + (size_t)blockIdx.y * per;
    for (size_t q = (size_t)blockIdx.x * blockDim.x + threadIdx.x; q < per; q += (size_t)gridDim.x * blockDim.x) {
        const int c = (int)(q & (TW - 1));
        const size_t rest = q >> TWS;
        const int k = (int)(rest % n1), lt = (int)(rest / n1);
        const size_t plain = (size_t)(lt * TW + c) * n1 + k;
        if (to_tiled) ob[q] = ib[plain];
        else ob[plain] = ib[q];
    }
}

__global__ void spec_unpack_tiled_kernel(const double2 *__restrict__ S, double2 *__restrict__ U, int n1, int N, int utiled) {
    const int b = blockIdx.z;
    const int l = blockIdx.x * blockDim.x + threadIdx.x;
    const int k = blockIdx.y;
    if (l >= N) return;
    const double2 *s = S + (size_t)b * n1 * N;
    double2 *u = U + (size_t)b * (n1 + 1) * N;
    double2 r;
    if (k == 0 || k == n1) {
        const double2 P = s[s_tiled(0, l, n1)];
        const double2 Q = cconj(s[s_tiled(0, (N - l) & (N - 1), n1)]);
        if (k == 0) {
            r = cscale(cadd(P, Q), 0.5);
        } else {
            const double2 d = csub(P, Q);
            r = make_double2(0.5 * d.y, -0.5 * d.x);
        }
    } else {
        r = s[s_tiled(k, l, n1)];
    }
    if (utiled) u[u_tiled(k, l, n1)] = r;
    else u[(size_t)l * (n1 + 1) + k] = r;
}
```

semi-blind-image-deblurring-problems-with-tv_amd/csrc/salsa.hip:

```cpp
#include <algorithm>
#include <chrono>
#include <cmath>

#include <time.h>

#include "sbtv_internal.h"

namespace sbtv {

__global__ void salsa_setup_kernel(const double *__restrict__ src, double *__restrict__ par, int npar, int *__restrict__ frozen,
                                   int batch) {
    for (int i = threadIdx.x; i < npar; i += blockDim.x) par[i] = src[i];
    for (int b = threadIdx.x; b < batch; b += blockDim.x) frozen[b] = 0;
}

__global__ __launch_bounds__(256) void salsa_recover_x_kernel(const double *__restrict__ g, const double *__restrict__ bu,
                                                               double *__restrict__ x, size_t P) {
#pragma clang fp contract(off)
    for (size_t q = (size_t)blockIdx.x * 256 + threadIdx.x; q < P / 2; q += (size_t)gridDim.x * 256) {
        const double2 a = *reinterpret_cast<const double2 *>(g + 2 * q), b = *reinterpret_cast<const double2 *>(bu + 2 * q);
        *reinterpret_cast<double2 *>(x + 2 * q) = make_double2(a.x + b.x, a.y + b.y);
    }
}

__global__ __launch_bounds__(256) void salsa_collect_kernel(Collect c, ProxCtrl *__restrict__ ctrl,
                                                             unsigned long long out_addr,
                                                             const int *__restrict__ frozen, int rearm,
                                                             unsigned long long tags_addr, double seq) {
    __shared__ double red[4];
    salsa_collect_block(c, ctrl, out_addr, frozen, rearm, tags_addr, seq, blockIdx.x, blockIdx.y, red);
}

}

using namespace sbtv;

extern "C" {

void sbtv_salsa_opts_default(sbtv_salsa_opts *o) {
    if (!o) return;
    o->stopcriterion = 1;
    o->maxiter = 10000;
    o->TViters = 5;
    o->initialization = 0;
    o->compute_mse = 0;
    o->speculate = 1;
    o->tolA = 0.001;
    o->chambolle_tol = 1e-3;
    o->chambolle_tau = 0.249;
}

}

namespace {

struct SalsaRun {
    sbtv_ctx *ctx; const double *yd; int M, N, batch; const double *taps; int taille; const double *tau, *mu;
    const sbtv_salsa_opts *opts; const double *td, *xi; double *x_out, *objective, *distance, *times, *mses;
    int *numA, *numAt, *n_outer; int flags; bool spec_wanted;

    BlurOp op{};
    ProxPlan pp;
    size_t P = 0, cnt = 0, npar = 0;
    int maxiter = 0, lag = 0, nrb = 0, npb = 0, nl_prox = 0;
    bool want_mse = false, crit2 = false, zero_start = false, direct_last_ok = false, direct_last = false, nox = false,
         spec_ok = false, use_graph = false;
    double *xbuf[2] = {nullptr, nullptr}, *u = nullptr, *gb[2] = {nullptr, nullptr}, *bub[2] = {nullptr, nullptr};
    double *par = nullptr, *taps_d = nullptr, *mu_d = nullptr, *thr_d = nullptr;
    double *acc = nullptr, *postp = nullptr, *o4 = nullptr;
    int *frozen_d = nullptr;
    SalsaScal *scal_h = nullptr, *scal_hd = nullptr, *init_h = nullptr, *init_hd = nullptr;
    double *psum_h = nullptr, *psum_hd = nullptr, *tags_h = nullptr, *tags_hd = nullptr, *init_tags_h = nullptr,
           *init_tags_hd = nullptr;
    int *frozen_h = nullptr;
    hipEvent_t ev_done[2], ev_p0[2], ev_p1[2];

    std::vector<int> h_numA, h_numAt, frozen, h_nouter;
    std::vector<double> obj_prev;
    bool init_read = false;
    int active = 0;
    double ms_prox = 0.0;
    long long prox_iters_run = 0, prox_iters_timed = 0;
    GraphExecs graphs;
    std::chrono::steady_clock::time_point t0;
    bool prox_timed[2] = {false, false}, slot_tagged[2] = {false, false}, slot_spec[2] = {false, false};
    struct PendingCollect {
        bool valid = false;
        int outer = 0;
        bool spec = false;
    } pend;

    int open() {
        SBTV_TRY(op_open(ctx, "salsa", M, N, batch, "Y", &op));
        SBTV_TRY(prox_plan(ctx, M, N, batch, &pp));
        P = op.P;
        cnt = P * batch;
        maxiter = opts->maxiter;
        want_mse = (td != nullptr);
        crit2 = (opts->stopcriterion == 2);
        zero_start = (opts->initialization == 0);
        lag = (opts->speculate & 1) ? 1 : 0;
        SBTV_TRY(ws_get_t(ctx, "salsa.x0", cnt, &xbuf[0]));
        SBTV_TRY(ws_get_t(ctx, "salsa.x1", cnt, &xbuf[1]));
        direct_last_ok = x_out && (flags & SBTV_DEVICE_PTRS) && !graph_wanted(cnt) && !overlaps(yd, x_out, cnt) &&
                         !overlaps(td, x_out, cnt) && !overlaps(xi, x_out, cnt);
        SBTV_TRY(ws_get_t(ctx, "salsa.u", cnt, &u));
        SBTV_TRY(ws_get_t(ctx, "salsa.bu", cnt, &bub[0]));
        SBTV_TRY(ws_get_t(ctx, "salsa.g", cnt, &gb[0]));
        static const bool env_nox = [] {
            const char *e = getenv("SBTV_SALSA_NOX");
            return !(e && e[0] == '0');
        }();
        nox = env_nox && fft_cols_inv_step_ok(op.fp) && !crit2 && !graph_wanted(cnt) && x_out != nullptr;
        gb[1] = gb[0];
        bub[1] = bub[0];
        if (nox) {
            SBTV_TRY(ws_get_t(ctx, "salsa.bu1", cnt, &bub[1]));
            SBTV_TRY(ws_get_t(ctx, "salsa.g1", cnt, &gb[1]));
        }
        direct_last = direct_last_ok && !nox;
        const size_t nt = (size_t)batch * taille * taille;
        npar = nt + 2 * (size_t)batch;
        SBTV_TRY(ws_get_t(ctx, "salsa.par", npar, &par));
        taps_d = par;
        mu_d = par + nt;
        thr_d = mu_d + batch;
        SBTV_TRY(ws_get_t(ctx, "salsa.frozen", (size_t)batch, &frozen_d));
        nrb = fft_rows_blocks(op.fp);
        npb = fft_cols_blocks(op.fp);
        SBTV_TRY(ws_get_t(ctx, "salsa.acc", (size_t)batch * 3 * nrb, &acc));
        SBTV_TRY(ws_get_t(ctx, "salsa.post", (size_t)batch * 6 * npb, &postp));
        SalsaScal *scal_d = nullptr;
        SBTV_TRY(ws_get_t(ctx, "salsa.scal", 2 * (size_t)batch, &scal_d));
        SBTV_TRY(ws_get_t(ctx, "salsa.o4", (size_t)batch * 4, &o4));

        PinnedLayout lay;
        const auto f_scal = lay.add<SalsaScal>(2 * (size_t)batch);
        const auto f_init = lay.add<SalsaScal>((size_t)batch);
        const auto f_psum = lay.add<double>(2 * (size_t)batch * FSTRIDE);
        const auto f_tags = lay.add<double>(2 * (size_t)batch * SALSA_TAGS);
        const auto f_itag = lay.add<double>((size_t)batch * SALSA_TAGS);
        const auto f_par = lay.add<double>(npar);
        const auto f_frozen = lay.add<int>((size_t)batch);
        void *ph = nullptr, *pd = nullptr;
        SBTV_TRY(pinned_get(ctx, lay.bytes(), &ph, &pd));
        scal_h = f_scal.at(ph), scal_hd = f_scal.at(pd);
        init_h = f_init.at(ph), init_hd = f_init.at(pd);
        psum_h = f_psum.at(ph), psum_hd = f_psum.at(pd);
        tags_h = f_tags.at(ph), tags_hd = f_tags.at(pd);
        init_tags_h = f_itag.at(ph), init_tags_hd = f_itag.at(pd);
        frozen_h = f_frozen.at(ph);
        for (int b = 0; b < batch; ++b) frozen_h[b] = 0;
        for (size_t i = 0; i < f_tags.count; ++i) tags_h[i] = 0.0;
        for (size_t i = 0; i < f_itag.count; ++i) init_tags_h[i] = 0.0;
        double *par_stage = f_par.at(ph);
        for (size_t q = 0; q < nt; ++q) par_stage[q] = taps[q];
        for (int b = 0; b < batch; ++b) {
            par_stage[nt + b] = mu[b];
            par_stage[nt + batch + b] = tau[b] / mu[b];
        }
        hipLaunchKernelGGL(salsa_setup_kernel, dim3(1), dim3(256), 0, ctx->stream, (const double *)f_par.at(pd), par, (int)npar,
                           frozen_d, batch);
        SBTV_HIP(ctx, hipGetLastError());
        return 0;
    }

    int spectra() {
        const long long dims[6] = {M, N, batch, taille, op.fp.u_tiled, (long long)op.fp.u_img};
        const size_t nt = (size_t)batch * taille * taille;
        const bool same = ctx->salsa_h_ptr == (const void *)op.Hs && std::equal(dims, dims + 6, ctx->salsa_h_dims) &&
                          ctx->salsa_h_taps.size() == nt && std::equal(taps, taps + nt, ctx->salsa_h_taps.begin());
        if (!same) {
            ctx->salsa_h_ptr = nullptr;
            SBTV_TRY(psf_spectrum(ctx, op.fp, taps_d, taille, op.Hs));
            ctx->salsa_h_taps.assign(taps, taps + nt);
            std::copy(dims, dims + 6, ctx->salsa_h_dims);
            ctx->salsa_h_ptr = (const void *)op.Hs;
        }
        SBTV_TRY(op_spectrum(ctx, op.fp, yd, nullptr, op.S, op.Ys));
        h_numA.assign(batch, 0);
        h_numAt.assign(batch, 1);
        ctx->calls += 2LL * batch;
        return 0;
    }

    int start() {
        double *x = xbuf[0], *bu = bub[0], *g = gb[0];
        if (zero_start) ctx->calls += batch;
        else SBTV_TRY(op_init_x(ctx, op, opts->initialization, yd, xi, x));
        if (!zero_start) {
            SBTV_HIP(ctx, hipMemcpyAsync(u, x, sizeof(double) * cnt, hipMemcpyDeviceToDevice, ctx->stream));
            SBTV_HIP(ctx, hipMemcpyAsync(g, x, sizeof(double) * cnt, hipMemcpyDeviceToDevice, ctx->stream));
            SBTV_HIP(ctx, hipMemsetAsync(bu, 0, sizeof(double) * cnt, ctx->stream));
        }
        SBTV_TRY(prox_reset(ctx, pp, thr_d, 1.0, opts->TViters, opts->chambolle_tol, opts->chambolle_tau, false, nullptr));
        obj_prev.assign(batch, 0.0);
        Collect c{};
        if (zero_start) {
            double *accz = nullptr, *postz = nullptr;
            int nz = 0;
            SBTV_TRY(salsa_zero_start(ctx, yd, want_mse ? td : nullptr, x, u, bu, P, batch, (double)M * (double)N, &accz, &postz,
                                      &nz));
            c = Collect{accz, nz, nullptr, 0, postz, nz, nullptr, 0, 0, 0ull, nullptr};
        } else {
            double *tvp = nullptr;
            int ntv = 0;
            RowsArgs a{};
            a.dir_fwd = 1;
            a.op = OP_RESID;
            a.H = op.Hs;
            a.Y = op.Ys;
            a.acc = acc;
            SBTV_TRY(fft_cols_fwd(ctx, op.fp, x, nullptr, op.S));
            SBTV_TRY(tvnorm_partials(ctx, u, M, N, batch, &tvp, &ntv));
            SBTV_TRY(fft_rows(ctx, op.fp, op.S, nullptr, a));
            if (want_mse) SBTV_TRY(pair_sums(ctx, x, td, P, batch, o4));
            c = Collect{acc, nrb, tvp, ntv, nullptr, 0, nullptr, 0, 0, 0ull, want_mse ? o4 : nullptr};
        }
        hipLaunchKernelGGL(salsa_collect_kernel, dim3(7, batch), dim3(256), 0, ctx->stream, c, (ProxCtrl *)nullptr,
                           (unsigned long long)(uintptr_t)init_hd, (const int *)nullptr, 0,
                           (unsigned long long)(uintptr_t)init_tags_hd, 1.0);
        SBTV_HIP(ctx, hipGetLastError());
        ctx->calls += batch;
        return 0;
    }

    int read_initial() {
        if (init_read) return 0;
        init_read = true;
        volatile const double *tg = init_tags_h;
        for (unsigned spin = 0;; ++spin) {
            bool ready = true;
            for (int b = 0; b < batch && ready; ++b)
                for (int i = 0; i < 8 && ready; ++i) ready = (tg[(size_t)b * SALSA_TAGS + i] == 1.0);
            if (ready) break;
            if (spin > 2000) {
                SBTV_HIP(ctx, hipStreamSynchronize(ctx->stream));
                break;
            }
            struct timespec ts = {0, 5000};
            nanosleep(&ts, nullptr);
        }
        __atomic_thread_fence(__ATOMIC_ACQUIRE);
        for (int b = 0; b < batch; ++b) {
            h_numA[b] += 1;
            const double f0 = 0.5 * (init_h[b].resid2 * op.parseval) + tau[b] * init_h[b].tv_u;
            obj_prev[b] = f0;
            if (objective) objective[(size_t)b * (maxiter + 1)] = f0;
            if (times) times[(size_t)b * (maxiter + 1)] = 0.0;
            if (mses && want_mse) mses[(size_t)b * (maxiter + 1)] = init_h[b].mse_num / (double)P;
        }
        return 0;
    }

    Collect make_collect(int outer, bool spec) const {
        const int slot = outer & 1;
        return Collect{acc, nrb, nullptr, 0, postp, npb, spec ? pp.partials + (size_t)slot * pp.part_stride : nullptr, pp.fnblk,
                       opts->TViters, (unsigned long long)(uintptr_t)(psum_hd + (size_t)slot * batch * FSTRIDE), nullptr};
    }
    int launch_collect(int outer, bool spec, bool tagged) {
        const int slot = outer & 1;
        const Collect c = make_collect(outer, spec);
        hipLaunchKernelGGL(salsa_collect_kernel, dim3(spec ? 7 + opts->TViters : 7, batch), dim3(256), 0, ctx->stream, c, pp.ctrl,
                           (unsigned long long)(uintptr_t)(scal_hd + (size_t)slot * batch), (const int *)frozen_d, 1,
                           tagged ? (unsigned long long)(uintptr_t)(tags_hd + (size_t)slot * batch * SALSA_TAGS) : 0ull, (double)outer);
        SBTV_HIP(ctx, hipGetLastError());
        return 0;
    }
    int flush_pending() {
        if (!pend.valid) return 0;
        pend.valid = false;
        return launch_collect(pend.outer, pend.spec, true);
    }

    int enqueue_body(int outer, bool eager) {
        static const bool piggyback = [] {
            const char *e = getenv("SBTV_COLLECT_RIDE");
            return !(e && e[0] == '0');
        }();
        const int slot = outer & 1;
        const bool tagged = eager;
        const bool spec = spec_ok && outer >= 2;
        const bool timed = eager && ((outer & 31) == 4 || outer == 12);
        slot_tagged[slot] = tagged;
        slot_spec[slot] = spec;
        double *xn = (direct_last && outer == maxiter) ? x_out : xbuf[slot];
        const double *xprev = xbuf[slot ^ 1];
        SideJob side{};
        if (pend.valid && spec) {
            const int ps = pend.outer & 1;
            side.c = make_collect(pend.outer, pend.spec);
            side.out_addr = (unsigned long long)(uintptr_t)(scal_hd + (size_t)ps * batch);
            side.tags_addr = (unsigned long long)(uintptr_t)(tags_hd + (size_t)ps * batch * SALSA_TAGS);
            side.frozen = frozen_d;
            side.seq = (double)pend.outer;
            side.nblocks = 7 + (pend.spec ? opts->TViters : 0);
            pend.valid = false;
        } else {
            SBTV_TRY(flush_pending());
        }
        if (timed) SBTV_HIP(ctx, hipEventRecord(ev_p0[slot], ctx->stream));
        ProxPlan pps = pp;
        pps.partials = pp.partials + (size_t)slot * pp.part_stride;
        if (!(zero_start && outer == 1))
            SBTV_TRY(prox_iterate(ctx, pps, gb[(outer - 1) & 1], opts->TViters, u, outer == (zero_start ? 2 : 1), spec,
                                  spec ? ((outer - 2) * nl_prox) & 1 : 0, side.nblocks ? &side : nullptr));
        if (timed) SBTV_HIP(ctx, hipEventRecord(ev_p1[slot], ctx->stream));
        prox_timed[slot] = timed;
        RowsArgs a{};
        a.dir_fwd = 1;
        a.dir_inv = 1;
        a.op = OP_SALSA;
        a.H = op.Hs;
        a.Y = op.Ys;
        a.mu = mu_d;
        a.acc = acc;
        a.frozen = frozen_d;
        SBTV_TRY(fft_cols_fwd_f(ctx, op.fp, u, bub[(outer - 1) & 1], op.S, frozen_d));
        SBTV_TRY(fft_rows(ctx, op.fp, op.S, op.S, a));
        ColsPost cp;
        cp.u = u;
        cp.bu = bub[outer & 1];
        cp.g = gb[outer & 1];
        if (nox) {
            cp.bu_in = bub[(outer - 1) & 1];
            cp.skip_x = 1;
        }
        cp.tru = td;
        cp.xprev = crit2 ? xprev : nullptr;
        cp.partials = postp;
        SBTV_TRY(fft_cols_inv_post(ctx, op.fp, op.S, xn, op.inv_scale, frozen_d, cp));
        if (spec && eager && lag == 1 && outer < maxiter && piggyback) {
            pend.valid = true;
            pend.outer = outer;
            pend.spec = spec;
            return 0;
        }
        return launch_collect(outer, spec, tagged);
    }
    int enqueue(int outer) {
        const int slot = outer & 1;
        hipGraphExec_t(&gexec)[2] = graphs.g;
        if (use_graph && outer >= 3) {
            if (!gexec[slot]) {
                if (graph_begin(ctx) != 0 || graph_end(ctx, enqueue_body(outer, false), &gexec[slot]) != 0) {
                    use_graph = false;
                    gexec[slot] = nullptr;
                }
            }
            if (gexec[slot]) {
                SBTV_HIP(ctx, hipGraphLaunch(gexec[slot], ctx->stream));
                SBTV_HIP(ctx, hipEventRecord(ev_done[slot], ctx->stream));
                return 0;
            }
        }
        return enqueue_body(outer, true);
    }

    int process(int outer) {
        const int slot = outer & 1;
        SBTV_TRY(read_initial());
        if (pend.valid && pend.outer == outer) SBTV_TRY(flush_pending());
        if (slot_tagged[slot])
            SBTV_TRY(wait_tags(ctx, tags_h + (size_t)slot * batch * SALSA_TAGS, batch, SALSA_TAGS, 8,
                               slot_spec[slot] ? opts->TViters : 0, (double)outer));
        else SBTV_TRY(wait_event(ctx, ev_done[slot]));
        if (prox_timed[slot]) {
            float ms = 0.f;
            SBTV_HIP(ctx, hipEventSynchronize(ev_p1[slot]));
            SBTV_HIP(ctx, hipEventElapsedTime(&ms, ev_p0[slot], ev_p1[slot]));
            ms_prox += ms;
            for (int b = 0; b < batch; ++b)
                if (!frozen[b]) prox_iters_timed += slot_spec[slot] ? (long long)opts->TViters : (long long)scal_h[(size_t)slot * batch + b].pad;
            prox_timed[slot] = false;
        }
        if (slot_spec[slot])
            SBTV_TRY(spec_stop_rule(ctx, pp, psum_h + (size_t)slot * batch * FSTRIDE, opts->TViters, opts->chambolle_tol,
                                    frozen.data()));
        const double tnow = std::chrono::duration<double>(std::chrono::steady_clock::now() - t0).count();
        bool changed = false;
        for (int b = 0; b < batch; ++b) {
            if (frozen[b]) continue;
            const SalsaScal &s = scal_h[(size_t)slot * batch + b];
            h_numA[b] += 1;
            h_nouter[b] = outer;
            double prox_k = s.pad;
            if (zero_start && outer == 1) prox_k = 1.0;
            if (slot_spec[slot]) prox_k = (double)opts->TViters;
            prox_iters_run += (long long)prox_k;
            ctx->calls += 2;
            const double f = 0.5 * (s.resid2 * op.parseval) + tau[b] * s.tv_u;
            if (objective) objective[(size_t)b * (maxiter + 1) + outer] = f;
            if (mses && want_mse) mses[(size_t)b * (maxiter + 1) + outer] = s.mse_num / (double)P;
            if (distance) distance[(size_t)b * maxiter + (outer - 1)] = sqrt(s.dist_num) / sqrt(s.x2 + s.u2);
            if (times) times[(size_t)b * (maxiter + 1) + outer] = tnow;
            const bool stop = salsa_stop(opts->stopcriterion, outer, f, obj_prev[b], s.dx2, s.x2, opts->tolA);
            obj_prev[b] = f;
            if (stop) {
                frozen[b] = 1;
                frozen_h[b] = 1;
                --active;
                changed = true;
            }
        }
        if (changed && active > 0) SBTV_TRY(upload_frozen(ctx, frozen_h, frozen_d, batch, pp.ctrl));
        return 0;
    }

    int result() {
        if (!x_out) return 0;
        for (int b = 0; b < batch; ++b) {
            double *out = x_out + (size_t)b * P;
            if (!nox) {
                if (direct_last && h_nouter[b] == maxiter) continue;
                const double *src = xbuf[h_nouter[b] & 1] + (size_t)b * P;
                if (flags & SBTV_DEVICE_PTRS)
                    SBTV_HIP(ctx, hipMemcpyAsync(out, src, sizeof(double) * P, hipMemcpyDeviceToDevice, ctx->stream));
                else
                    SBTV_TRY(stage_out_copy(ctx, out, src, P, flags));
                continue;
            }
            const int par = h_nouter[b] & 1;
            const bool dev_direct = direct_last_ok;
            double *dst = dev_direct ? out : xbuf[0] + (size_t)b * P;
            const int nblk = (int)std::min<size_t>((P / 2 + 255) / 256, 2048);
            if (h_nouter[b] == 0) {
                SBTV_HIP(ctx, hipMemcpyAsync(dst, xbuf[0] + (size_t)b * P, sizeof(double) * P, hipMemcpyDeviceToDevice, ctx->stream));
            } else {
                hipLaunchKernelGGL(salsa_recover_x_kernel, dim3(nblk), dim3(256), 0, ctx->stream,
                                   (const double *)(gb[par] + (size_t)b * P), (const double *)(bub[par] + (size_t)b * P), dst, P);
                SBTV_HIP(ctx, hipGetLastError());
            }
            if (!dev_direct && (flags & SBTV_DEVICE_PTRS))
                SBTV_HIP(ctx, hipMemcpyAsync(out, dst, sizeof(double) * P, hipMemcpyDeviceToDevice, ctx->stream));
            else if (!dev_direct)
                SBTV_TRY(stage_out_copy(ctx, out, dst, P, flags));
        }
        return 0;
    }

    int finish() {
        SBTV_TRY(loop_timing(ctx, prox_iters_timed > 0 ? ms_prox * ((double)prox_iters_run / (double)prox_iters_timed) : 0.0,
                             prox_iters_run, batch, P));
        for (int b = 0; b < batch; ++b) {
            if (numA) numA[b] = h_numA[b];
            if (numAt) numAt[b] = h_numAt[b];
            if (n_outer) n_outer[b] = h_nouter[b];
        }
        return 0;
    }

    int run() {
        SBTV_TRY(open());
        SBTV_TRY(spectra());
        SBTV_TRY(start());
        frozen.assign(batch, 0);
        h_nouter.assign(batch, 0);
        active = batch;
        for (auto &e : ctx->loop_ev)
            if (!e) SBTV_HIP(ctx, hipEventCreate(&e));
        for (int s = 0; s < 2; ++s) {
            ev_done[s] = ctx->loop_ev[s];
            ev_p0[s] = ctx->loop_ev[2 + s];
            ev_p1[s] = ctx->loop_ev[4 + s];
        }
        t0 = std::chrono::steady_clock::now();
        spec_ok = spec_wanted && !graph_wanted(cnt) && prox_spec_ok(pp, gb[0], u, opts->TViters);
        nl_prox = prox_launches(pp, opts->TViters);
        use_graph = graph_wanted(cnt);
        int done = 0;
        SBTV_TRY(pipelined_loop(ctx, &done, maxiter, lag, true, [&](int k) { return enqueue(k); }, [&](int k) { return process(k); },
                                [&] { return active > 0; }));
        SBTV_TRY(read_initial());
        SBTV_HIP(ctx, hipEventRecord(ctx->ev[1], ctx->stream));
        SBTV_TRY(result());
        SBTV_HIP(ctx, hipStreamSynchronize(ctx->stream));
        return finish();
    }
};

}

extern "C" int sbtv_SALSA_v2(sbtv_ctx *ctx, const double *y, int M, int N, int batch, const double *taps, int taille,
                             const double *tau, const double *mu, const sbtv_salsa_opts *opts, const double *true_x,
                             const double *x_init, double *x_out, double *objective, double *distance, double *times,
                             double *mses, int *numA, int *numAt, int *n_outer, int flags) {
    if (!ctx) return SBTV_ERR_BADARG;
    if (!tau || !mu) return fail(ctx, SBTV_ERR_BADARG, "SALSA_v2: missing required argument");
    SBTV_TRY(check_common(ctx, "SALSA_v2", y, taps, opts, x_init, M, N, batch, taille, "x_init", true, false));
    for (int b = 0; b < batch; ++b)
        if (!(mu[b] > 0.0)) return fail(ctx, SBTV_ERR_MISSING_LS, "(A^T A + mu I)^(-1) must be specified: mu must be > 0");
    SBTV_HIP(ctx, hipSetDevice(ctx->device));
    if (sbtv_group *lg = lanes_group(ctx, batch, false)) {
        LaneCall lc(ctx, lg);
        return lc.done(salsa_sharded(lg, y, M, N, batch, taps, taille, tau, mu, opts, true_x, x_init, x_out, objective,
                                     distance, times, mses, numA, numAt, n_outer, flags), batch);
    }
    SBTV_HIP(ctx, hipEventRecord(ctx->ev[0], ctx->stream));
    const size_t cnt = (size_t)M * N * batch;
    const double *yd = nullptr, *td = nullptr, *xi = nullptr;
    SBTV_TRY(stage_in(ctx, "salsa.y", y, cnt, flags, &yd));
    SBTV_TRY(stage_in(ctx, "salsa.true", true_x, cnt, flags, &td));
    SBTV_TRY(stage_in(ctx, "salsa.xinit", x_init, cnt, flags, &xi));
    return canary_epilogue(ctx, solve_with_exact_repeat(ctx, !(opts->speculate & 2), [&](bool spec) {
        SalsaRun r{ctx, yd, M, N, batch, taps, taille, tau, mu, opts, td, xi, x_out, objective, distance, times, mses,
                   numA, numAt, n_outer, flags, spec};
        return r.run();
    }));
}
```

semi-blind-image-deblurring-problems-with-tv_amd/csrc/sbtv_internal.h:

```cpp
#pragma once
#include <hip/hip_runtime.h>

#include <chrono>
#include <map>
#include <string>
#include <vector>

#include "../../include/sbtv.h"
#include "pinned_layout.h"

namespace sbtv {

constexpr int kWave = 64;

struct ProxCtrl {
    int k;
    int done;
    int cur;
    int maxiter;
    int redo;
    int f_valid;
    double err;
    double lambda;
    double tol;
    double tau;
};

__device__ __forceinline__ double mb_step_sum(const double *__restrict__ p, int nblk, int lane) {
    double acc = 0.0;
    for (int q0 = 0; q0 < nblk; q0 += 64 * 16) {
        double v[16];
#pragma unroll
        for (int r = 0; r < 16; ++r) {
            const int q = q0 + r * 64 + lane;
            v[r] = (q < nblk) ? p[q] : 0.0;
        }
#pragma unroll
        for (int r = 0; r < 16; ++r) acc += v[r];
    }
#pragma unroll
    for (int off = 32; off > 0; off >>= 1) acc += __shfl_xor(acc, off, 64);
    return acc;
}
__device__ __forceinline__ void mb_apply_rule(ProxCtrl &c, const double *tots, int total, int base, int extra) {
    int k = total;
    for (int st = 0; st < total; ++st) {
        if (!((st + 1 < total) && (sqrt(tots[st]) > c.tol))) {
            k = st + 1;
            break;
        }
    }
    c.k = k;
    c.err = sqrt(tots[k - 1]);
    c.done = 1;
    if (k == total) {
        c.redo = 0;
        c.f_valid = 1;
    } else {
        int l = 0, start = 0;
        for (;; ++l) {
            const int len = base + (l < extra ? 1 : 0);
            if (k <= start + len) break;
            start += len;
        }
        c.cur = l;
        c.redo = k - start;
        c.f_valid = 0;
    }
}

struct SalsaScal {
    double resid2;
    double tv_u;
    double mse_num;
    double dist_num;
    double x2;
    double u2;
    double dx2;
    double pad;
};

struct HostStats {
    double waits = 0;
    double ready_at_once = 0;
    double waits_slept = 0;
    double sleeps = 0;
    double stream_queries = 0;
    double wait_s = 0, wait_max_s = 0;
    double enqueue_s = 0, enqueue_max_s = 0;
    double wait_max_outer = 0;
    double nvcsw = 0, nivcsw = 0, minflt = 0, majflt = 0;
};

struct DevBuf {
    void *p = nullptr;
    void *base = nullptr;
    size_t bytes = 0;
};

}

struct sbtv_ctx {
    int device = 0;
    hipStream_t stream = nullptr;
    bool own_stream = true;
    std::string err;
    long long calls = 0;
    double timing[4] = {0, 0, 0, 0};
    sbtv::HostStats hstat;
    std::map<std::string, sbtv::DevBuf> ws;
    std::vector<double> salsa_h_taps;
    long long salsa_h_dims[6] = {0, 0, 0, 0, 0, 0};
    const void *salsa_h_ptr = nullptr;
    std::map<int, double2 *> twiddles;
    std::map<int, double2 *> any_axes;
    bool any_attr_done = false;
    void *pinned = nullptr;
    size_t pinned_bytes = 0;
    hipEvent_t ev[4] = {nullptr, nullptr, nullptr, nullptr};
    hipEvent_t loop_ev[6] = {nullptr, nullptr, nullptr, nullptr, nullptr, nullptr};
    int cu_count = 256;
    struct StageLane {
        hipStream_t s = nullptr;
        void *pin[2] = {nullptr, nullptr};
        hipEvent_t ev[2] = {nullptr, nullptr};
    } stage[4];
    bool stage_ready = false;
    double stage_stats[4] = {0, 0, 0, 0};
    double solve_stats[4] = {0, 0, 0, 0};
    struct sbtv_group *lanes = nullptr;
    int lanes_mode = 0;
    bool is_lane = false;
    bool canary = false;
    bool canary_dirty = true;
    void *canary_desc = nullptr;
    int *canary_bad = nullptr;
    int canary_n = 0, canary_cap = 0;
};

namespace sbtv {

int fail(sbtv_ctx *ctx, int code, const std::string &msg);
int fail_hip(sbtv_ctx *ctx, hipError_t e, const char *what, const char *file, int line);
void set_global_error(const std::string &msg);

#define SBTV_HIP(ctx, expr)                                                     \
    do {                                                                        \
        hipError_t e__ = (expr);                                                \
        if (e__ != hipSuccess) return sbtv::fail_hip((ctx), e__, #expr, __FILE__, __LINE__); \
    } while (0)

#define SBTV_TRY(expr)             \
    do {                           \
        int rc__ = (expr);         \
        if (rc__ != 0) return rc__; \
    } while (0)

int ws_get(sbtv_ctx *ctx, const char *name, size_t bytes, void **out);
template <typename T>
inline int ws_get_t(sbtv_ctx *ctx, const char *name, size_t count, T **out) {
    void *p = nullptr;
    int rc = ws_get(ctx, name, count * sizeof(T), &p);
    *out = static_cast<T *>(p);
    return rc;
}
int pinned_get(sbtv_ctx *ctx, size_t bytes, void **out);
template <typename T>
inline int pinned_get(sbtv_ctx *ctx, size_t bytes, T **host, T **dev) {
    void *h = nullptr, *d = nullptr;
    SBTV_TRY(pinned_get(ctx, bytes, &h));
    SBTV_HIP(ctx, hipHostGetDevicePointer(&d, h, 0));
    *host = static_cast<T *>(h);
    *dev = static_cast<T *>(d);
    return 0;
}
template <class T>
inline T *off(T *p, size_t o) { return p ? p + o : p; }
inline bool overlaps(const double *a, const double *b, size_t n) { return a && b && a < b + n && b < a + n; }
int canary_epilogue(sbtv_ctx *ctx, int rc);
int canary_verify(sbtv_ctx *ctx, int *nbuf, int *nbad, std::string *first_bad);
int twiddle_get(sbtv_ctx *ctx, int n, const double2 **out);

inline bool is_pow2(int v) { return v > 0 && (v & (v - 1)) == 0; }
inline int ilog2(int v) { int l = 0; while ((1 << l) < v) ++l; return l; }

int stage_in(sbtv_ctx *ctx, const char *name, const double *p, size_t count, int flags, const double **dev);
int stage_out_buf(sbtv_ctx *ctx, const char *name, double *p, size_t count, int flags, double **dev);
int stage_out_copy(sbtv_ctx *ctx, double *host, const double *dev, size_t count, int flags);

__device__ __forceinline__ double fast_rcp(double d) {
    const double r = __builtin_amdgcn_rcp(d);
    const double e = __builtin_fma(-d, r, 1.0);
    return __builtin_fma(r, __builtin_fma(e, e, e), r);
}

__device__ __forceinline__ void philox_round(unsigned &c0, unsigned &c1, unsigned &c2, unsigned &c3, unsigned k0,
                                             unsigned k1) {
    const unsigned long long p0 = 0xD2511F53ull * c0, p1 = 0xCD9E8D57ull * c2;
    const unsigned h0 = (unsigned)(p0 >> 32), l0 = (unsigned)p0, h1 = (unsigned)(p1 >> 32), l1 = (unsigned)p1;
    c0 = h1 ^ c1 ^ k0;
    c1 = l1;
    c2 = h0 ^ c3 ^ k1;
    c3 = l0;
}
__device__ __forceinline__ double2 philox_normal_pair(size_t q, unsigned step, unsigned chain, unsigned long long seed) {
#pragma clang fp contract(off)
    unsigned c0 = (unsigned)q, c1 = (unsigned)(q >> 32), c2 = step, c3 = chain;
    unsigned k0 = (unsigned)seed, k1 = (unsigned)(seed >> 32);
#pragma unroll
    for (int r = 0; r < 10; ++r) {
        philox_round(c0, c1, c2, c3, k0, k1);
        k0 += 0x9E3779B9u;
        k1 += 0xBB67AE85u;
    }
    const unsigned long long a = ((unsigned long long)c0 << 32) | c1, bb = ((unsigned long long)c2 << 32) | c3;
    const double u1 = ((double)(a >> 11) + 0.5) * (1.0 / 9007199254740992.0);
    const double u2 = ((double)(bb >> 11) + 0.5) * (1.0 / 9007199254740992.0);
    const double r = sqrt(-2.0 * log(u1));
    double s, c;
    sincospi(2.0 * u2, &s, &c);
    return make_double2(r * c, r * s);
}
__device__ __forceinline__ double myula_nocontract(double x, double p, double v, double scale, double z, double gam,
                                                   double lamb, double s2, double sq2g) {
#pragma clang fp contract(off)
    const double g = v * scale;
    return fabs(((x + gam * (p - x) / lamb) - gam * (g / s2)) + sq2g * z);
}
__device__ __forceinline__ void welford_nocontract(double &mean, double &m2, double x, int k, double rk) {
#pragma clang fp contract(off)
    if (k == 1) {
        mean = x;
        m2 = 0.0;
        return;
    }
    const double d = x - mean;
    mean = mean + d * rk;
    m2 = m2 + d * (x - mean);
}
struct MomArgs {
    double *mean, *m2;
    int k;
    const int *it;
    int first, thin;
};
__device__ __forceinline__ int mom_sample(const MomArgs &m) {
    if (m.k > 0) return m.k;
    const int ii = m.it[0];
    if (ii < m.first || (ii - m.first) % m.thin != 0) return 0;
    return (ii - m.first) / m.thin + 1;
}
__device__ __forceinline__ void moments_pair(const MomArgs &m, size_t o, double2 r, int k, double rk) {
    double2 mu = make_double2(0.0, 0.0), s = make_double2(0.0, 0.0);
    if (k > 1) {
        mu = *reinterpret_cast<const double2 *>(m.mean + o);
        s = *reinterpret_cast<const double2 *>(m.m2 + o);
    }
    welford_nocontract(mu.x, s.x, r.x, k, rk);
    welford_nocontract(mu.y, s.y, r.y, k, rk);
    *reinterpret_cast<double2 *>(m.mean + o) = mu;
    *reinterpret_cast<double2 *>(m.m2 + o) = s;
}
struct MomReq {
    int first, thin, pooled;
    double *mean, *var;
    long long *count;
    bool dev;
    bool raw;
};
inline int mom_sample_of(const MomReq *mr, int ii) {
    if (!mr || ii < mr->first || (ii - mr->first) % mr->thin != 0) return 0;
    return (ii - mr->first) / mr->thin + 1;
}
inline long long mom_count(const MomReq &mr, int last) { return (last - mr.first) / mr.thin + 1; }
int moments_seed(sbtv_ctx *ctx, const double *X, double *mean, double *m2, size_t P, int batch);
int moments_finish(sbtv_ctx *ctx, const double *mean, const double *m2, size_t P, int batch, long long n, const MomReq &req);

struct RngArgs {
    unsigned long long seed;
    unsigned step, chain0;
    const double *step_dev;
};

struct ProxArm {
    ProxCtrl *ctrl;
    const double *lambda;
    int maxiter;
    double tol, tau;
    const int *frozen;
};

::sbtv_group *lanes_group(sbtv_ctx *ctx, int n_items, bool shared);
struct LaneCall {
    sbtv_ctx *ctx;
    ::sbtv_group *g;
    long long calls0[8];
    LaneCall(sbtv_ctx *c, ::sbtv_group *grp);
    int done(int rc, int n_items);
};
int salsa_sharded(::sbtv_group *g, const double *y, int M, int N, int n_items, const double *taps, int taille,
                  const double *tau, const double *mu, const sbtv_salsa_opts *opts, const double *true_x,
                  const double *x_init, double *x_out, double *objective, double *distance, double *times, double *mses,
                  int *numA, int *numAt, int *n_outer, int flags);
int sapg_sharded(::sbtv_group *g, const double *y, int M, int N, int n_items, const sbtv_sapg_opts *op,
                 const double *x0, const double *noise, double *thetas, double *ps, double *sigmas, double *logpi,
                 double *logpi_wu, double *gx, double *grads, double *eb, double *x_last, int flags,
                 const MomReq *mom = nullptr);
int sapg_impl(sbtv_ctx *ctx, const double *y, int M, int N, int batch, const sbtv_sapg_opts *op, const double *x0,
              const double *noise, double *thetas, double *ps, double *sigmas, double *logpi, double *logpi_wu, double *gx,
              double *grads, double *eb, double *x_last, sbtv_allreduce_fn reduce_fn, void *reduce_user, int flags,
              const MomReq *mom);
int fista_sharded(::sbtv_group *g, const double *b, int M, int N, int n_items, const double *taps, int taille,
                  const double *tau, double L, int prox_iters, int stopcriterion, double tolerance, int maxiters,
                  int zero_start, const double *true_x, double *x_out, double *objective, double *mses, int *n_iter,
                  int flags);
int csalsa_sharded(::sbtv_group *g, const double *y, int M, int N, int n_items, const double *taps, int taille,
                   const double *mu1, const double *mu2, const double *sigma, const double *epsilon,
                   double continuationfactor, const sbtv_salsa_opts *opts, const double *true_x, const double *x_init,
                   double *x_out, double *objective, double *distance1, double *distance2, double *criterion,
                   double *times, double *mses, int *numA, int *numAt, int *n_outer, int flags);
int coral_sharded(::sbtv_group *g, const double *y, int M, int N, int n_items, const double *taps, int taille,
                  const double *tau1, const double *tau2, const double *mu1, const double *mu2, const double *mu_ls,
                  int TViters2, const sbtv_salsa_opts *opts, const double *true_x, const double *x_init, double *x_out,
                  double *objective, double *distance, double *times, double *mses, int *numA, int *numAt, int *n_outer,
                  int flags);
int masked_sharded(::sbtv_group *g, const double *y, const double *mask, int M, int N, int n_items, const double *taps,
                   int taille, const double *tau, const double *mu1, const double *mu2, const sbtv_salsa_opts *opts,
                   const double *true_x, const double *x_init, double *x_out, double *objective, double *distance,
                   double *times, double *mses, int *numA, int *numAt, int *n_outer, int flags);

int wait_event(sbtv_ctx *ctx, hipEvent_t ev);
int wait_stream(sbtv_ctx *ctx);
int wait_tags(sbtv_ctx *ctx, const double *tags, int batch, int stride, int nscal, int nstep, double seq);

bool graph_wanted(size_t total_px);
int graph_begin(sbtv_ctx *ctx);
int graph_end(sbtv_ctx *ctx, int body_rc, hipGraphExec_t *exec);
struct GraphExecs {
    hipGraphExec_t g[2] = {nullptr, nullptr};
    ~GraphExecs() {
        for (auto e : g)
            if (e) (void)hipGraphExecDestroy(e);
    }
};

int loop_timing(sbtv_ctx *ctx, double prox_ms, long long prox_iters, int batch, size_t P);
void host_stats_begin(sbtv_ctx *ctx);
void host_stats_end(sbtv_ctx *ctx);

template <class Enqueue, class Process, class Active>
int pipelined_loop(sbtv_ctx *ctx, int *done, int maxiter, int lag, bool stats, Enqueue &&enqueue, Process &&process,
                   Active &&active) {
    if (stats) host_stats_begin(ctx);
    int rc = 0, enq = *done;
    while (rc == 0 && active() && *done < maxiter) {
        while (rc == 0 && enq < maxiter && enq - *done <= lag) {
            const auto te = std::chrono::steady_clock::now();
            rc = enqueue(++enq);
            const double d = std::chrono::duration<double>(std::chrono::steady_clock::now() - te).count();
            if (stats) {
                ctx->hstat.enqueue_s += d;
                if (d > ctx->hstat.enqueue_max_s) ctx->hstat.enqueue_max_s = d;
            }
        }
        if (rc == 0) rc = process(++*done);
    }
    if (rc != 0) {
        (void)hipStreamSynchronize(ctx->stream);
        return rc;
    }
    if (stats) host_stats_end(ctx);
    return 0;
}

struct ProxPlan {
    int M, N, batch;
    int tiles_i, tiles_j, nblk;
    int ftiles_i, ftiles_j, fnblk;
    int cj, nw, minw, rpl;
    ProxCtrl *ctrl;
    double *pbuf;
    int pairs;
    std::string tag;
    double *partials;
    size_t part_stride;
    unsigned *counters;
    const int *order;
    int esub_off;
};
int prox_plan(sbtv_ctx *ctx, int M, int N, int batch, ProxPlan *plan, const char *tag = "prox");
int prox_reset(sbtv_ctx *ctx, const ProxPlan &pl, const double *lambda_dev, double lambda_scale,
               int maxiter, double tol, double tau, bool keep_cur, const int *frozen);
int prox_zero_duals(sbtv_ctx *ctx, const ProxPlan &pl);
int prox_set_duals(sbtv_ctx *ctx, const ProxPlan &pl, const double *px, const double *py);
int prox_get_duals(sbtv_ctx *ctx, const ProxPlan &pl, double *px, double *py);
constexpr int FSMAX = 10;
constexpr double SPEC_TOL_GUARD = 1.0 + 1e-12;
constexpr double ESUB_MARGIN = 32.0;
constexpr int FSTRIDE = 32;
constexpr int SALSA_TAGS = 8 + FSTRIDE;
struct Collect {
    const double *acc;
    int nrb;
    const double *tvp;
    int ntv;
    const double *post;
    int npb;
    const double *ppart;
    int pnblk, psteps;
    unsigned long long psum_addr;
    const double *mse0;
};
struct SideJob {
    Collect c;
    unsigned long long out_addr, tags_addr;
    const int *frozen;
    double seq;
    int nblocks;
};
#ifdef __HIPCC__
#include "collect.inc"
#endif

int prox_iterate(sbtv_ctx *ctx, const ProxPlan &pl, const double *g, int maxiter, double *f_out = nullptr,
                 bool cold = false, int spec = 0, int spec_parity = 0, const SideJob *side = nullptr);
int prox_reserve_pairs(sbtv_ctx *ctx, ProxPlan *pl, int pairs);
int prox_launches(const ProxPlan &pl, int maxiter);
bool prox_spec_ok(const ProxPlan &pl, const double *g, const double *f_out, int maxiter);
constexpr double CHAMBOLLE_TOL = 1e-3, CHAMBOLLE_TAU = 0.249;

constexpr int SOLVE_RESTART_EXACT = 12345;
int spec_stop_rule(sbtv_ctx *ctx, ProxPlan &pp, const double *stepsums, int K, double tol, const int *frozen = nullptr);
template <class Body>
int solve_with_exact_repeat(sbtv_ctx *ctx, bool spec, Body &&body) {
    const long long calls0 = ctx->calls;
    const int rc = body(spec);
    if (rc != SOLVE_RESTART_EXACT) return rc;
    ctx->calls = calls0;
    ctx->solve_stats[0] += 1;
    return body(false);
}
int upload_frozen(sbtv_ctx *ctx, const int *frozen_h, int *frozen_d, int batch, ProxCtrl *park_ctrl);
int prox_finish(sbtv_ctx *ctx, const ProxPlan &pl, const double *g, double *f);
int tvnorm_dev(sbtv_ctx *ctx, const double *x, int M, int N, int batch, double *out_dev);
int tvnorm_partials(sbtv_ctx *ctx, const double *x, int M, int N, int batch, double **partials, int *nblk);

enum SpecOp {
    OP_NONE = 0,
    OP_MUL_H = 1,
    OP_MUL_HC = 2,
    OP_INVLS = 3,
    OP_SALSA = 4,
    OP_RESID = 5,
    OP_GRAD = 6,
    OP_ATA = 7,
    OP_GRADF = 8,
    OP_CSALSA = 9,
};
struct FftPlan {
    int M, N, batch;
    int n1;
    int wave;
    int u_tiled;
    size_t u_img;
    size_t s_img;
    int generic;
    const double2 *tw_n1;
    const double2 *tw_M;
    const double2 *tw_N;
};
int fft_plan(sbtv_ctx *ctx, int M, int N, int batch, FftPlan *plan);
int fft_cols_fwd(sbtv_ctx *ctx, const FftPlan &pl, const double *x, const double *add, double2 *S);
int fft_cols_inv(sbtv_ctx *ctx, const FftPlan &pl, const double2 *S, double *x, double scale);
struct ColsPost {
    const double *u = nullptr;
    double *bu = nullptr;
    double *g = nullptr;
    const double *bu_in = nullptr;
    int skip_x = 0;
    const double *tru = nullptr;
    const double *xprev = nullptr;
    double *partials = nullptr;
    double *ystep = nullptr;
    double alpha = 0.0;
    const double *mprox = nullptr, *msig2 = nullptr, *mZ = nullptr;
    double mgam = 0.0, mlamb = 0.0, msq2g = 0.0;
    RngArgs mrng = {0ull, 0u, 0u, nullptr};
    ProxArm marm = {nullptr, nullptr, 0, 0.0, 0.0, nullptr};
    MomArgs mom = {nullptr, nullptr, 0, nullptr, 1, 1};
};
int fft_cols_inv_myula(sbtv_ctx *ctx, const FftPlan &pl, const double2 *S, double scale, double *X, const double *prox,
                       const double *Z, const double *sigma2_dev, double gam, double lamb, const RngArgs *rng,
                       const ProxArm *arm, const MomArgs *mom = nullptr);
int fft_cols_blocks(const FftPlan &pl);
bool fft_cols_inv_step_ok(const FftPlan &pl);
int fft_cols_inv_step(sbtv_ctx *ctx, const FftPlan &pl, const double2 *S, double *y, double scale, double alpha,
                      const int *frozen);
int fft_cols_inv_sub(sbtv_ctx *ctx, const FftPlan &pl, const double2 *S, double *x, double scale, const double *b, double *g);
int fft_cols_inv_post(sbtv_ctx *ctx, const FftPlan &pl, const double2 *S, double *x, double scale, const int *frozen,
                      const ColsPost &post);
struct RowsArgs {
    int dir_fwd;
    int dir_inv;
    int op;
    const double2 *H;
    const double2 *Y;
    const double2 *D1, *D2;
    double2 *E;
    const double *cs;
    const double *mu;
    double *acc;
    const int *frozen;
    int shared_spec;
};
int fft_rows(sbtv_ctx *ctx, const FftPlan &pl, const double2 *Sin, double2 *Sout, const RowsArgs &a);
int fft_rows_blocks(const FftPlan &pl);
bool fft_rows_csalsa_ok(const FftPlan &pl);
int spec_unpack(sbtv_ctx *ctx, const FftPlan &pl, const double2 *S, double2 *U);
int psf_spectrum(sbtv_ctx *ctx, const FftPlan &pl, const double *taps_dev, int taille, double2 *U);
int psf_spectrum_sets(sbtv_ctx *ctx, const FftPlan &pl, const double *const *taps_dev, int taille, double2 *const *U, int nsets);

int reduce_partials(sbtv_ctx *ctx, const double *partials, int nvec, int n, double *out);
struct RedJobs {
    const double *src[4] = {nullptr, nullptr, nullptr, nullptr};
    double *dst[4] = {nullptr, nullptr, nullptr, nullptr};
    int nvec[4] = {0, 0, 0, 0};
    int n[4] = {0, 0, 0, 0};
    int dropped = 0;
    void add(const double *s, int nv, int nn, double *d) {
        for (int q = 0; q < 4; ++q)
            if (nvec[q] == 0) {
                src[q] = s;
                dst[q] = d;
                nvec[q] = nv;
                n[q] = nn;
                return;
            }
        ++dropped;
    }
};
int reduce_jobs(sbtv_ctx *ctx, const RedJobs &jb);
int ew_blocks(size_t P);
int pair_sums(sbtv_ctx *ctx, const double *a, const double *c, size_t P, int batch, double *out4_dev);
int salsa_zero_start(sbtv_ctx *ctx, const double *y, const double *tru, double *x, double *u, double *bu, size_t P, int batch,
                     double scale, double **accp, double **postp, int *nblk);
int axpy(sbtv_ctx *ctx, double *y, const double *gr, double a, size_t Ptot, const ProxArm *arm = nullptr, int batch = 0);
int fista_momentum(sbtv_ctx *ctx, const double *x, const double *xold, double *y, const double *tru, double coef,
                   double *partials, size_t P, int batch, const int *frozen);
int myula_step(sbtv_ctx *ctx, double *X, const double *prox, const double *grad, const double *Z,
               const double *sigma2_dev, double gam, double lamb, size_t P, int batch, const RngArgs *rng = nullptr,
               const ProxArm *arm = nullptr, const MomArgs *mom = nullptr);
int myula_plain_step(sbtv_ctx *ctx, double *X, const double *prox, const double *grad, const double *Z,
                     const double *sigma2_dev, double gam, double lamb, size_t P, int batch, const RngArgs *rng,
                     const ProxArm *arm, const MomArgs *mom = nullptr);
int fft_cols_fwd_f(sbtv_ctx *ctx, const FftPlan &pl, const double *x, const double *add, double2 *S, const int *frozen,
                   double *tvp = nullptr);
bool fft_cols_tv_ok(const FftPlan &pl);
int fft_cols_inv_f(sbtv_ctx *ctx, const FftPlan &pl, const double2 *S, double *x, double scale, const int *frozen);

struct BlurOp {
    FftPlan fp;
    int batch;
    size_t P;
    double2 *S, *Hs, *Ys;
    double inv_scale, parseval;
};
int op_open(sbtv_ctx *ctx, const char *prefix, int M, int N, int batch, const char *y_name, BlurOp *op);
int op_spectrum(sbtv_ctx *ctx, const FftPlan &fp, const double *in, const double *add, double2 *S, double2 *U);
int op_apply(sbtv_ctx *ctx, const BlurOp &c, int op, const double *in, double *out, const double *mu = nullptr);
int op_solve(sbtv_ctx *ctx, const BlurOp &c, const double *in, const double *add, const double2 *Y, const double *mu,
             double *acc, double *out);
int op_resid(sbtv_ctx *ctx, const BlurOp &c, const double *x, double *acc, const int *frozen = nullptr, double *tvp = nullptr);
int op_gradf(sbtv_ctx *ctx, const BlurOp &c, const double *x, double *acc, double *grad);
int op_init_x(sbtv_ctx *ctx, const BlurOp &c, int initialization, const double *yd, const double *xi, double *x);

int check_psf_fits(sbtv_ctx *ctx, int taille, int M, int N);
int check_even_pixels(sbtv_ctx *ctx, int M, int N);
int check_common(sbtv_ctx *ctx, const char *who, const double *y, const double *taps, const sbtv_salsa_opts *opts,
                 const double *x_init, int M, int N, int batch, int taille, const char *x_init_name = "x_init", bool tv = true,
                 bool maxiter_positive = true);
inline bool salsa_stop(int stopcriterion, int outer, double f, double obj_prev, double num, double den, double tolA) {
    if (outer <= 1) return false;
    double crit;
    if (stopcriterion == 1)
        crit = fabs(f - obj_prev) / obj_prev;
    else if (stopcriterion == 2)
        crit = fabs(sqrt(num) / sqrt(den));
    else
        crit = f;
    return crit < tolA;
}

struct WavPlan {
    int M, N, K, J;
    double f0[8], f1[8];
    int bands() const { return 3 * J + 1; }
};
int wav_plan(sbtv_ctx *ctx, int M, int N, const double *h, int hlen, int levels, bool orthonormal, WavPlan *pl);
int wav_analysis(sbtv_ctx *ctx, const WavPlan &pl, const double *x, double *z, int batch);
int wav_synthesis(sbtv_ctx *ctx, const WavPlan &pl, const double *z, double *x, int batch);
int wav_synthesis(sbtv_ctx *ctx, const WavPlan &pl, const double *z, double *x, int batch, const MomArgs *mom);
__device__ __forceinline__ double wav_soft(double x, double T) { return copysign(fmax(fabs(x) - T, 0.0), x); }
__device__ __forceinline__ double wav_myula_nocontract(double x, double g, double z, double T, double gam, double lamb,
                                                       double s2, double sq2g) {
#pragma clang fp contract(off)
    return ((x + gam * (wav_soft(x, T) - x) / lamb) - gam * (g / s2)) + sq2g * z;
}
constexpr int WAV_EWB = 256;
constexpr int WAV_EW_MAXBLK = 2048;
inline int wav_ew_blocks(size_t dimX) {
    const size_t nb = (dimX / 2 + WAV_EWB - 1) / WAV_EWB;
    return nb > (size_t)WAV_EW_MAXBLK ? WAV_EW_MAXBLK : (nb < 1 ? 1 : (int)nb);
}
__device__ __forceinline__ double wav_wave_sum(double v) {
#pragma unroll
    for (int off = 32; off > 0; off >>= 1) v += __shfl_xor(v, off, 64);
    return v;
}
__device__ __forceinline__ double wav_block_sum(double v, double *red) {
    v = wav_wave_sum(v);
    __syncthreads();
    if ((threadIdx.x & 63) == 0) red[threadIdx.x >> 6] = v;
    __syncthreads();
    return (red[0] + red[1]) + (red[2] + red[3]);
}
struct WavThetaStep {
    double eta, th;
    double sum_eta, n_eta;
    double tol, mean;
};
__device__ __forceinline__ WavThetaStep wav_theta_step(double eta, double th_cur, double g, double delta, double dimX,
                                                       double min_eta, double max_eta, bool burn, double sum_eta,
                                                       double n_eta) {
#pragma clang fp contract(off)
    WavThetaStep t;
    const double etaii = eta + delta * (dimX / th_cur - g) * exp(eta);
    t.eta = fmin(fmax(etaii, min_eta), max_eta);
    t.th = exp(t.eta);
    const double nan = __builtin_nan("");
    const double m0 = n_eta > 0.0 ? exp(sum_eta / n_eta) : nan;
    t.sum_eta = burn ? sum_eta + t.eta : sum_eta;
    t.n_eta = burn ? n_eta + 1.0 : n_eta;
    t.mean = t.n_eta > 0.0 ? exp(t.sum_eta / t.n_eta) : nan;
    t.tol = fabs(t.mean - m0) / m0;
    return t;
}

struct WavChain {
    WavPlan wp;
    BlurOp op;
    int batch, nblk, nrb;
    size_t P, cnt, dimX, ccnt;
    const double *yd, *x0d;
    const double *noise;
    double *X, *G, *img, *Z;
};
int wav_chain_buffers(sbtv_ctx *ctx, const char *prefix, const WavPlan &wp, int batch, const double *y, const double *xw0,
                      const double *noise, double *xw_last, int flags, WavChain *c);
int wav_chain_start(sbtv_ctx *ctx, const WavChain &c);
int wav_chain_spectrum(sbtv_ctx *ctx, const WavChain &c, const MomArgs *mom = nullptr);
int wav_chain_rows(sbtv_ctx *ctx, const WavChain &c, int op, double *acc, const double2 *D1 = nullptr,
                   const double2 *D2 = nullptr);
int wav_abs_sum(sbtv_ctx *ctx, const WavChain &c, double *part);
struct WavStepPar {
    const double *theta, *sigma2;
    int stride;
};
int wav_chain_step(sbtv_ctx *ctx, const WavChain &c, const WavStepPar &par, double gam, double lamb, const RngArgs &rng,
                   double *part, const MomArgs *mom = nullptr);

// ... 19 lines not shown
```

semi-blind-image-deblurring-problems-with-tv_amd/csrc/tv.hip:

```cpp
#include <mutex>

#include <algorithm>
#include "sbtv_internal.h"

#pragma clang fp contract(off)

namespace sbtv {

constexpr int TI = 128;
constexpr int TJ = 16;
constexpr int CJ = TJ / 4;
constexpr int ULD = TI + 2;
constexpr int TVB = 256;

__device__ __forceinline__ double wave_sum(double v) {
#pragma unroll
    for (int off = 32; off > 0; off >>= 1) v += __shfl_xor(v, off, 64);
    return v;
}

__device__ __forceinline__ double block_sum_256(double v, double *red ) {
    v = wave_sum(v);
    const int lane = threadIdx.x & 63, w = threadIdx.x >> 6;
    if (lane == 0) red[w] = v;
// ... 409 lines not shown
    __syncthreads();
    if (threadIdx.x != 0) return;
    ProxCtrl c = ctrl[b];
    if (c.done) return;
    mb_apply_rule(c, tots, total, base, extra);
    ctrl[b] = c;
}

__global__ __launch_bounds__(256) void chambolle_ctrl_kernel(ProxCtrl *__restrict__ ctrl,
                                                              const double *__restrict__ partials, int nblk) {
    const int b = blockIdx.x;
    ProxCtrl *c = &ctrl[b];
    if (c->done) return;
    __shared__ double red[4];
    const double *p = partials + (size_t)b * nblk;
    double s = 0.0;
    for (int q = threadIdx.x; q < nblk; q += 256) s += p[q];
    const double tot = block_sum_256(s, red);
    if (threadIdx.x == 0) {
        const int k = c->k + 1;
        const double err = sqrt(tot);
        c->k = k;
        c->err = err;
        c->cur ^= 1;
        c->done = !((k < c->maxiter) && (err > c->tol));
    }
}

__global__ void prox_reset_kernel(ProxCtrl *__restrict__ ctrl, const double *__restrict__ lambda,
                                  double lambda_scale, int maxiter, double tol, double tau, int keep_cur,
                                  int batch, const int *__restrict__ frozen) {
    const int b = blockIdx.x * blockDim.x + threadIdx.x;
    if (b >= batch) return;
    ProxCtrl c = ctrl[b];
    c.k = 0;
    c.done = (frozen && frozen[b]) ? 1 : 0;
    c.cur = keep_cur ? (c.cur & 1) : 0;
    c.maxiter = maxiter;
    c.redo = 0;
    c.f_valid = 0;
    c.err = 0.0;
    c.lambda = lambda[b] * lambda_scale;
    c.tol = tol;
    c.tau = tau;
    ctrl[b] = c;
}

template <bool VEC>
__global__ __launch_bounds__(TVB) void chambolle_finish_kernel(const double *__restrict__ g,
                                                                const double *__restrict__ pbuf,
                                                                const ProxCtrl *__restrict__ ctrl,
                                                                double *__restrict__ f, int M, int N, int batch) {
    const int b = blockIdx.z;
    const ProxCtrl c = ctrl[b];
    const size_t P = (size_t)M * N;
    const size_t plane = P * batch;
    const double *__restrict__ px = pbuf + (size_t)((c.cur & 1) * 2 + 0) * plane + (size_t)b * P;
    const double *__restrict__ py = pbuf + (size_t)((c.cur & 1) * 2 + 1) * plane + (size_t)b * P;
    const int lane = threadIdx.x & 63, w = threadIdx.x >> 6;
    const int i = blockIdx.x * TI + 2 * lane;
    const bool ok0 = i < M, ok1 = i + 1 < M;
    const double lambda = c.lambda;
#pragma unroll
    for (int c4 = 0; c4 < CJ; ++c4) {
        const int j = blockIdx.y * TJ + w * CJ + c4;
        if (j >= N) break;
        const size_t off = (size_t)j * M + i;
        const double2 pxv = ld2<VEC>(px, off, ok0, ok1);
        const double2 pyv = ld2<VEC>(py, off, ok0, ok1);
        const double2 gv = ld2<VEC>(g + (size_t)b * P, off, ok0, ok1);
        const double2 pym = (j > 0) ? ld2<VEC>(py, off - M, ok0, ok1) : make_double2(0.0, 0.0);
        double pxm = __shfl_up(pxv.y, 1, 64);
        if (lane == 0) pxm = (i > 0 && ok0) ? px[off - 1] : 0.0;
        double2 r;
        r.x = gv.x - lambda * (div1(pyv.x, pym.x, j, N) + div1(pxv.x, pxm, i, M));
        r.y = gv.y - lambda * (div1(pyv.y, pym.y, j, N) + div1(pxv.y, pxv.x, i + 1, M));
        st2<VEC>(f + (size_t)b * P, off, r, ok0, ok1);
    }
}

template <bool VEC>
__global__ __launch_bounds__(TVB) void tvnorm_kernel(const double *__restrict__ x, double *__restrict__ partials,
                                                      int M, int N, int tiles_i) {
    const int b = blockIdx.z;
    const size_t P = (size_t)M * N;
    const double *__restrict__ xb = x + (size_t)b * P;
    __shared__ double red[4];
    const int lane = threadIdx.x & 63, w = threadIdx.x >> 6;
    const int i = blockIdx.x * TI + 2 * lane;
    const bool ok0 = i < M, ok1 = i + 1 < M;
    double s = 0.0;
#pragma unroll
    for (int c4 = 0; c4 < CJ; ++c4) {
        const int j = blockIdx.y * TJ + w * CJ + c4;
        if (j >= N) break;
        const size_t off = (size_t)j * M + i;
        const int jm = (j > 0) ? j - 1 : N - 1;
        const double2 xv = ld2<VEC>(xb, off, ok0, ok1);
        const double2 xl = ld2<VEC>(xb, (size_t)jm * M + i, ok0, ok1);
        double xu = __shfl_up(xv.y, 1, 64);
        if (lane == 0 && ok0) xu = xb[(size_t)j * M + ((i > 0) ? i - 1 : M - 1)];
        if (ok0) {
            const double dh = xv.x - xl.x, dv = xv.x - xu;
            s += sqrt(dh * dh + dv * dv);
        }
        if (ok1) {
            const double dh = xv.y - xl.y, dv = xv.y - xv.x;
            s += sqrt(dh * dh + dv * dv);
        }
    }
    const double bs = block_sum_256(s, red);
    if (threadIdx.x == 0) partials[(size_t)b * (gridDim.x * gridDim.y) + (size_t)blockIdx.y * tiles_i + blockIdx.x] = bs;
}

__global__ __launch_bounds__(256) void reduce_partials_kernel(const double *__restrict__ partials, int n,
                                                               double *__restrict__ out) {
    __shared__ double red[4];
    const double *p = partials + (size_t)blockIdx.x * n;
    double s = 0.0;
    for (int q = threadIdx.x; q < n; q += 256) s += p[q];
    const double tot = block_sum_256(s, red);
    if (threadIdx.x == 0) out[blockIdx.x] = tot;
}

__global__ __launch_bounds__(256) void reduce_jobs_kernel(RedJobs jb) {
    __shared__ double red[4];
    int v = blockIdx.x, q = 0;
    while (q < 3 && v >= jb.nvec[q]) v -= jb.nvec[q++];
    const int n = jb.n[q];
    const double *p = jb.src[q] + (size_t)v * n;
    double s = 0.0;
    for (int i = threadIdx.x; i < n; i += 256) s += p[i];
    const double tot = block_sum_256(s, red);
    if (threadIdx.x == 0) jb.dst[q][v] = tot;
}

__global__ void copy_duals_kernel(double *__restrict__ dst0, double *__restrict__ dst1,
                                  const double *__restrict__ pbuf, const ProxCtrl *__restrict__ ctrl, size_t P,
                                  int batch) {
    const int b = blockIdx.y;
    const ProxCtrl c = ctrl[b];
    const size_t plane = P * batch;
    const double *px = pbuf + (size_t)((c.cur & 1) * 2 + 0) * plane + (size_t)b * P;
    const double *py = pbuf + (size_t)((c.cur & 1) * 2 + 1) * plane + (size_t)b * P;
    for (size_t q = (size_t)blockIdx.x * blockDim.x + threadIdx.x; q < P; q += (size_t)gridDim.x * blockDim.x) {
        dst0[(size_t)b * P + q] = px[q];
        dst1[(size_t)b * P + q] = py[q];
    }
}


static inline bool vec_ok(const void *p, int M) { return (M % 2 == 0) && ((reinterpret_cast<uintptr_t>(p) & 15) == 0); }

int prox_plan(sbtv_ctx *ctx, int M, int N, int batch, ProxPlan *pl, const char *tag) {
    pl->M = M;
    pl->N = N;
    pl->batch = batch;
    pl->tiles_i = (M + TI - 1) / TI;
    pl->tiles_j = (N + TJ - 1) / TJ;
    pl->nblk = pl->tiles_i * pl->tiles_j;
    {
        static std::once_flag env_once;
        std::call_once(env_once, [] {
            if (const char *e = getenv("SBTV_FUSED_VARIANT")) {
                int cj = 0, nw = 0, mw = 0, rpl = 2;
                static const int known[][4] = {{4, 8, 4, 2}, {4, 8, 4, 1}};
                bool ok = false;
                if (sscanf(e, "%d,%d,%d,%d", &cj, &nw, &mw, &rpl) >= 3)
                    for (auto &k4 : known) ok = ok || (k4[0] == cj && k4[1] == nw && k4[2] == mw && k4[3] == rpl);
                if (ok) {
                    g_fused_forced = true;
                    g_fused.cj = cj;
                    g_fused.nw = nw;
                    g_fused.minw = mw;
                    g_fused.rpl = rpl;
                }
            }
            if (getenv("SBTV_EXACT") != nullptr) g_fused.fast = 0;
        });
    }
    auto geometry = [&](int cj, int nw, int rpl) {
        const int core_rows = (rpl == 1) ? F1CI : FCI, core_cols = cj * nw - FHL - FHJ;
        pl->ftiles_i = (M + core_rows - 1) / core_rows;
        pl->ftiles_j = (N + core_cols - 1) / core_cols;
        pl->fnblk = pl->ftiles_i * pl->ftiles_j;
        pl->cj = cj;
        pl->nw = nw;
        pl->rpl = rpl;
    };
    geometry(g_fused.cj, g_fused.nw, g_fused.rpl);
    pl->minw = g_fused.minw;
    if (!g_fused_forced && (size_t)pl->fnblk * batch < 256) {
        geometry(4, 8, 1);
        pl->minw = 4;
    }
    pl->esub_off = 0;
    const size_t P = (size_t)M * N;
    size_t npart = (size_t)batch * pl->nblk;
    if ((size_t)batch * FSTRIDE * pl->fnblk > npart) npart = (size_t)batch * FSTRIDE * pl->fnblk;
    const std::string t(tag ? tag : "prox");
    SBTV_TRY(ws_get_t(ctx, (t + ".ctrl").c_str(), (size_t)batch, &pl->ctrl));
    SBTV_TRY(ws_get_t(ctx, (t + ".pbuf").c_str(), 4 * P * batch, &pl->pbuf));
    pl->pairs = 2;
    pl->tag = t;
    SBTV_TRY(ws_get_t(ctx, (t + ".partials").c_str(), 2 * npart, &pl->partials));
    pl->part_stride = npart;
    pl->order = nullptr;
    {
        static const bool env_off = [] {
            const char *e = getenv("SBTV_TILE_ORDER");
            return e && e[0] == '0';
        }();
        const int nt = pl->fnblk;
        if (!env_off && pl->rpl == 2 && nt > 2 * 256) {
            int *od = nullptr;
            const std::string name = "prox.order." + std::to_string(M) + "x" + std::to_string(N) + "." + std::to_string(pl->cj) +
                                     "." + std::to_string(pl->nw);
            const bool built = ctx->ws.find(name) != ctx->ws.end();
            SBTV_TRY(ws_get_t(ctx, name.c_str(), (size_t)nt, &od));
            if (!built) {
                std::vector<int> h(nt);
                const int q8 = nt >> 3, r8 = nt & 7, ti_n = pl->ftiles_i, tj_n = pl->ftiles_j;
                for (int x = 0; x < 8; ++x) {
                    const int c0 = (x < r8 ? x * (q8 + 1) : r8 * (q8 + 1) + (x - r8) * q8);
                    const int len = q8 + (x < r8 ? 1 : 0);
                    int o = 0;
                    static const int env_mode = [] {
                        const char *e = getenv("SBTV_TILE_ORDER");
                        return e ? atoi(e) : 1;
                    }();
                    std::vector<int> chunk;
                    for (int t2 = c0; t2 < c0 + len; ++t2) chunk.push_back(t2);
                    if (env_mode >= 2)
                        std::stable_sort(chunk.begin(), chunk.end(), [&](int a, int b2) { return (a % ti_n) < (b2 % ti_n); });
                    for (int pass = 0; pass < 2; ++pass)
                        for (int t2 : chunk) {
                            const int ti = t2 % ti_n, tj = t2 / ti_n;
                            const bool border = (ti == 0 || ti == ti_n - 1 || tj == 0 || tj == tj_n - 1);
                            if (env_mode == 3 ? (pass == 0) : (border == (pass == 0))) h[(size_t)(o++) * 8 + x] = t2;
                        }
                }
                SBTV_HIP(ctx, hipStreamSynchronize(ctx->stream));
                SBTV_HIP(ctx, hipMemcpy(od, h.data(), sizeof(int) * nt, hipMemcpyHostToDevice));
            }
            pl->order = od;
        }
    }
    SBTV_TRY(ws_get_t(ctx, (t + ".counters").c_str(), (size_t)batch, &pl->counters));
    SBTV_HIP(ctx, hipMemsetAsync(pl->counters, 0, sizeof(unsigned) * batch, ctx->stream));
    return 0;
}

int prox_reserve_pairs(sbtv_ctx *ctx, ProxPlan *pl, int pairs) {
    if (pairs <= pl->pairs) return 0;
    if (pairs > 15) return fail(ctx, SBTV_ERR_BADARG, "prox_reserve_pairs: at most 15 dual buffers");
    const size_t P = (size_t)pl->M * pl->N;
    SBTV_TRY(ws_get_t(ctx, (pl->tag + ".pbuf").c_str(), (size_t)2 * pairs * P * pl->batch, &pl->pbuf));
    pl->pairs = pairs;
    return 0;
}

int prox_reset(sbtv_ctx *ctx, const ProxPlan &pl, const double *lambda_dev, double lambda_scale, int maxiter,
               double tol, double tau, bool keep_cur, const int *frozen) {
    const int thr = 64;
    hipLaunchKernelGGL(prox_reset_kernel, dim3((pl.batch + thr - 1) / thr), dim3(thr), 0, ctx->stream, pl.ctrl,
                       lambda_dev, lambda_scale, maxiter, tol, tau, keep_cur ? 1 : 0, pl.batch, frozen);
    SBTV_HIP(ctx, hipGetLastError());
    return 0;
}

int prox_zero_duals(sbtv_ctx *ctx, const ProxPlan &pl) {
    const size_t P = (size_t)pl.M * pl.N;
    SBTV_HIP(ctx, hipMemsetAsync(pl.pbuf, 0, 2 * P * pl.batch * sizeof(double), ctx->stream));
    return 0;
}

int prox_set_duals(sbtv_ctx *ctx, const ProxPlan &pl, const double *px, const double *py) {
    const size_t P = (size_t)pl.M * pl.N * pl.batch;
    SBTV_HIP(ctx, hipMemcpyAsync(pl.pbuf, px, P * sizeof(double), hipMemcpyDeviceToDevice, ctx->stream));
    SBTV_HIP(ctx, hipMemcpyAsync(pl.pbuf + P, py, P * sizeof(double), hipMemcpyDeviceToDevice, ctx->stream));
    return 0;
}

int prox_get_duals(sbtv_ctx *ctx, const ProxPlan &pl, double *px, double *py) {
    const size_t P = (size_t)pl.M * pl.N;
    hipLaunchKernelGGL(copy_duals_kernel, dim3(256, pl.batch), dim3(256), 0, ctx->stream, px, py, pl.pbuf, pl.ctrl,
                       P, pl.batch);
    SBTV_HIP(ctx, hipGetLastError());
    return 0;
}

int g_force_single_step = 0;

int prox_finish(sbtv_ctx *ctx, const ProxPlan &pl, const double *g, double *f);

bool prox_spec_ok(const ProxPlan &pl, const double *g, const double *f_out, int maxiter) {
    static const bool env_single = (getenv("SBTV_SINGLE_STEP") != nullptr);
    static const bool env_off = [] {
        const char *e = getenv("SBTV_PROX_SPEC");
        return e && e[0] == '0';
    }();
    return !env_off && !env_single && !g_force_single_step && maxiter <= FSTRIDE && vec_ok(g, pl.M) &&
           vec_ok(pl.pbuf, pl.M) && (!f_out || vec_ok(f_out, pl.M));
}

int prox_launches(const ProxPlan &pl, int maxiter) {
    return (maxiter + FHJ - 1) / FHJ;
}

int prox_iterate(sbtv_ctx *ctx, const ProxPlan &pl, const double *g, int maxiter, double *f_out, bool cold, int spec,
                 int spec_parity, const SideJob *side) {
    const bool spec_cur = spec != 0;
    const bool mb = spec >= 2;
    const bool mb_main = spec != 4, mb_ctrl = spec == 2, mb_redo = spec == 2 || spec == 4;
    if (mb && (!cold || !f_out || (size_t)pl.pairs < (size_t)prox_launches(pl, maxiter) + 2))
        return fail(ctx, SBTV_ERR_BADARG, "prox_iterate: the multi-buffer mode needs a cold prox with f output and prox_reserve_pairs()");
    const dim3 grid(pl.tiles_i, pl.tiles_j, pl.batch);
    const bool v = vec_ok(g, pl.M) && vec_ok(pl.pbuf, pl.M);
    static const bool env_single = (getenv("SBTV_SINGLE_STEP") != nullptr);
    if (spec_cur && !prox_spec_ok(pl, g, f_out, maxiter))
        return fail(ctx, SBTV_ERR_BADARG, "prox_iterate: optimistic mode is not available for this plan");
    if (v && !env_single && !g_force_single_step && (!f_out || vec_ok(f_out, pl.M))) {
        dim3 fgrid(pl.fnblk, 1, pl.batch);
        const SideJob no_side{};
        const int nl = prox_launches(pl, maxiter);
        const int base = maxiter / nl, extra = maxiter % nl;
        static const char *env_inl = getenv("SBTV_INLINE_CTRL");
        const bool env_inline = env_inl ? (env_inl[0] != '0') : ((size_t)pl.fnblk * pl.batch <= 512);
        int spec_off = 0, spec_l = 0;
        auto launch_fused = [&](int steps, int redo, int write_f) -> int {
            bool launched = false;
            const SideJob &sj = (spec_cur && side && spec_l == 0) ? *side : no_side;
            fgrid.x = pl.fnblk + sj.nblocks;
            const int inl = (!redo && env_inline && !spec_cur) ? 1 : 0;
            int kflags = inl | (cold ? 2 : 0);
            if (spec_cur) {
                if (mb && redo) {
                    kflags = 4 | 8 | 2 | ((nl + 1) << 24);
                } else if (mb) {
                    kflags = 4 | 8 | 2 | (spec_off << 12) | (spec_l << 20) | ((spec_l + 1) << 24);
                } else {
                    kflags = 4 | (cold ? 2 : 0) | ((spec_l & 1) << 8) | ((spec_parity & 1) << 9) | (spec_off << 12);
                }
                if (!redo) {
                    ++spec_l;
                    spec_off += steps;
                }
            }
#define SBTV_FUSED_CASE(CJ_, NW_, MW_)                                                                               \
    if (pl.rpl == 2 && pl.cj == CJ_ && pl.nw == NW_ && pl.minw == MW_) {                         \
        launched = true;                                                                                             \
        if (g_fused.fast)                                                                                            \
            hipLaunchKernelGGL((chambolle_fused_kernel<CJ_, NW_, MW_, true>), fgrid, dim3(64 * NW_), 0, ctx->stream, \
                               g, pl.pbuf, pl.ctrl, pl.partials, pl.M, pl.N, pl.batch, pl.ftiles_i, pl.fnblk, steps, \
                               redo, f_out, write_f, pl.counters, kflags, sj, pl.order, FusedStagger{fused_stagger(pl.fnblk)});  \
        else                                                                                                         \
            hipLaunchKernelGGL((chambolle_fused_kernel<CJ_, NW_, MW_, false>), fgrid, dim3(64 * NW_), 0,             \
                               ctx->stream, g, pl.pbuf, pl.ctrl, pl.partials, pl.M, pl.N, pl.batch, pl.ftiles_i,     \
                               pl.fnblk, steps, redo, f_out, write_f, pl.counters, kflags, sj, pl.order, FusedStagger{fused_stagger(pl.fnblk)}); \
    }
            static const bool esub_wanted = [] {
                const char *e = getenv("SBTV_ERR_SUBSET");
                return !(e && e[0] == '0');
            }();
            if (esub_wanted && !pl.esub_off && spec == 1 && !redo && pl.rpl == 2 && pl.cj == 4 && pl.nw == 8 && pl.minw == 4 &&
                g_fused.fast) {
                launched = true;
                hipLaunchKernelGGL((chambolle_fused_kernel<4, 8, 4, true, true>), fgrid, dim3(64 * 8), 0, ctx->stream, g, pl.pbuf,
                                   pl.ctrl, pl.partials, pl.M, pl.N, pl.batch, pl.ftiles_i, pl.fnblk, steps, redo, f_out, write_f,
                                   pl.counters, kflags, sj, pl.order, FusedStagger{fused_stagger(pl.fnblk)});
            } else
            SBTV_FUSED_CASE(4, 8, 4)
#undef SBTV_FUSED_CASE
#define SBTV_FUSED1_CASE(CJ_, NW_, MW_)                                                                              \
    if (pl.rpl == 1 && pl.cj == CJ_ && pl.nw == NW_ && pl.minw == MW_) {                         \
        launched = true;                                                                                             \
        if (g_fused.fast)                                                                                            \
            hipLaunchKernelGGL((chambolle_fused1_kernel<CJ_, NW_, MW_, true>), fgrid, dim3(64 * NW_), 0,             \
                               ctx->stream, g, pl.pbuf, pl.ctrl, pl.partials, pl.M, pl.N, pl.batch, pl.ftiles_i,     \
                               pl.fnblk, steps, redo, f_out, write_f, pl.counters, kflags, sj);                         \
        else                                                                                                         \
            hipLaunchKernelGGL((chambolle_fused1_kernel<CJ_, NW_, MW_, false>), fgrid, dim3(64 * NW_), 0,            \
                               ctx->stream, g, pl.pbuf, pl.ctrl, pl.partials, pl.M, pl.N, pl.batch, pl.ftiles_i,     \
                               pl.fnblk, steps, redo, f_out, write_f, pl.counters, kflags, sj);                         \
    }
            if (esub_wanted && !pl.esub_off && spec == 1 && !redo && pl.rpl == 1 && pl.cj == 4 && pl.nw == 8 && pl.minw == 4 && g_fused.fast) {
                launched = true;
                hipLaunchKernelGGL((chambolle_fused1_kernel<4, 8, 4, true, true>), fgrid, dim3(64 * 8), 0, ctx->stream, g, pl.pbuf,
                                   pl.ctrl, pl.partials, pl.M, pl.N, pl.batch, pl.ftiles_i, pl.fnblk, steps, redo, f_out, write_f,
                                   pl.counters, kflags, sj);
            } else
            SBTV_FUSED1_CASE(4, 8, 4)
#undef SBTV_FUSED1_CASE
            if (!launched)
                return fail(ctx, SBTV_ERR_BADARG, "prox_iterate: no fused Chambolle kernel is compiled for this tile geometry");
            if (!inl && !redo && !spec_cur)
                hipLaunchKernelGGL(chambolle_fused_ctrl_kernel, dim3(pl.batch), dim3(64 * FSMAX), 0, ctx->stream,
                                   pl.ctrl, pl.partials, pl.fnblk, steps, redo, write_f);
            return 0;
        };
        const int wf = f_out ? 1 : 0;
        if (mb_main)
// ... 207 lines not shown
```

Baseline: 4718 SALSA outer-iterations/s.

## Trim first and last SALSA iteration work and fold setup launches

With zero start, the kernel no longer zero-fills x/u/bu. The first outer iteration reads from a persistent zero buffer instead, and a new OP_SALSA0 row pass fuses the y spectrum stash with the first iteration's solve, skipping the forward column FFT of zeros. The last iteration can write recovered x (g+bu) straight into the output from the inverse-column kernel, removing a separate recover pass. Prox control reset and counter clearing are folded into the setup kernel. Together these cut launches and memory traffic per call, at the cost of more code paths and an env switch with several bit flags.

```diff
diff --git a/semi-blind-image-deblurring-problems-with-tv_amd/csrc/ctx.hip b/semi-blind-image-deblurring-problems-with-tv_amd/csrc/ctx.hip
--- a/semi-blind-image-deblurring-problems-with-tv_amd/csrc/ctx.hip
+++ b/semi-blind-image-deblurring-problems-with-tv_amd/csrc/ctx.hip
@@ -524,7 +524,8 @@
         "SBTV_CANARY", "SBTV_COLLECT_RIDE", "SBTV_EXACT", "SBTV_FFT_WAVE", "SBTV_FISTA_FUSED_STEP", "SBTV_FISTA_LAG",
         "SBTV_FUSED_VARIANT", "SBTV_GRAPH", "SBTV_INLINE_CTRL", "SBTV_PROX_SPEC", "SBTV_SAPG_DEFER",
         "SBTV_SAPG_FUSED_MYULA", "SBTV_SAPG_HOST", "SBTV_SINGLE_STEP", "SBTV_SPIN", "SBTV_TAG_SPIN_US", "SBTV_TILE_ORDER", "SBTV_SALSA_NOX", "SBTV_CSALSA_SPECTRAL",
-        "SBTV_CORAL_BATCH", "SBTV_ROWS_FOLD", "SBTV_ERR_SUBSET", "SBTV_LANES", "SBTV_LANE_COUNT", "SBTV_STAGE_THREADS", "SBTV_TEST_FAIL_SAPG", "SBTV_FUSED_STAGGER"};
+        "SBTV_CORAL_BATCH", "SBTV_ROWS_FOLD", "SBTV_ERR_SUBSET", "SBTV_LANES", "SBTV_LANE_COUNT", "SBTV_STAGE_THREADS", "SBTV_TEST_FAIL_SAPG", "SBTV_FUSED_STAGGER",
+        "SBTV_SALSA_CALLPATH" };
     if (!buf || cap == 0) return SBTV_ERR_BADARG;
     std::string s;
     int nset = 0;
diff --git a/semi-blind-image-deblurring-problems-with-tv_amd/csrc/elementwise.hip b/semi-blind-image-deblurring-problems-with-tv_amd/csrc/elementwise.hip
--- a/semi-blind-image-deblurring-problems-with-tv_amd/csrc/elementwise.hip
+++ b/semi-blind-image-deblurring-problems-with-tv_amd/csrc/elementwise.hip
@@ -34,6 +34,7 @@
     return (int)nb;
 }
 
+template <bool CLEAR>
 __global__ __launch_bounds__(EWB) void salsa_zero_start_kernel(const double *__restrict__ y, const double *__restrict__ tru,
                                                                 double *__restrict__ x, double *__restrict__ u,
                                                                 double *__restrict__ bu, double *__restrict__ accp,
@@ -47,9 +48,11 @@
         const double tv = tru ? tru[base + q] : 0.0;
         acc[0] += yv * yv;
         acc[1] += tv * tv;
-        x[base + q] = 0.0;
-        u[base + q] = 0.0;
-        bu[base + q] = 0.0;
+        if constexpr (CLEAR) {
+            x[base + q] = 0.0;
+            u[base + q] = 0.0;
+            bu[base + q] = 0.0;
+        }
     }
     ew_block_sum<2>(acc, red);
     if (threadIdx.x == 0) {
@@ -319,8 +322,12 @@
     const int G = ew_blocks(2 * P);
     SBTV_TRY(ws_get_t(ctx, "ew.zero.acc", (size_t)batch * 3 * G, accp));
     SBTV_TRY(ws_get_t(ctx, "ew.zero.post", (size_t)batch * 6 * G, postp));
-    hipLaunchKernelGGL(salsa_zero_start_kernel, dim3(G, batch), dim3(EWB), 0, ctx->stream, y, tru, x, u, bu, *accp, *postp, P,
-                       scale);
+    if (x && u && bu)
+        hipLaunchKernelGGL(salsa_zero_start_kernel<true>, dim3(G, batch), dim3(EWB), 0, ctx->stream, y, tru, x, u, bu, *accp,
+                           *postp, P, scale);
+    else
+        hipLaunchKernelGGL(salsa_zero_start_kernel<false>, dim3(G, batch), dim3(EWB), 0, ctx->stream, y, tru, (double *)nullptr,
+                           (double *)nullptr, (double *)nullptr, *accp, *postp, P, scale);
     SBTV_HIP(ctx, hipGetLastError());
     *nblk = G;
     return 0;
diff --git a/semi-blind-image-deblurring-problems-with-tv_amd/csrc/fft.hip b/semi-blind-image-deblurring-problems-with-tv_amd/csrc/fft.hip
--- a/semi-blind-image-deblurring-problems-with-tv_amd/csrc/fft.hip
+++ b/semi-blind-image-deblurring-problems-with-tv_amd/csrc/fft.hip
@@ -1015,7 +1015,8 @@
         const dim3 grid(cd.wgs, pl.batch), block(cd.threads);
         if (post.skip_x && (!post.bu_in || post.bu_in == post.bu || post.xprev))
             return fail(ctx, SBTV_ERR_BADARG, "fft_cols_inv_post: skip_x needs a separate bu_in and no xprev");
-        const int pm = 1 + (post.tru ? 2 : 0) + (post.xprev ? 4 : 0) + (post.skip_x ? 32 : 0);
+        if (post.skip_x == 2 && !x) return fail(ctx, SBTV_ERR_BADARG, "fft_cols_inv_post: skip_x = 2 stores g + bu to x");
+        const int pm = 1 + (post.tru ? 2 : 0) + (post.xprev ? 4 : 0) + (post.skip_x ? 32 : 0) + (post.skip_x == 2 ? 256 : 0);
 #define SBTV_POST_CASE(PM_)                                                                                          \
     case PM_:                                                                                                        \
         if (pl.n1 == 1024)                                                                                           \
@@ -1032,6 +1033,8 @@
             SBTV_POST_CASE(7)
             SBTV_POST_CASE(33)
             SBTV_POST_CASE(35)
+            SBTV_POST_CASE(33 + 256)
+            SBTV_POST_CASE(35 + 256)
         }
 #undef SBTV_POST_CASE
         SBTV_HIP(ctx, hipGetLastError());
@@ -1059,8 +1062,10 @@
     return {rk, rk * (pl.N / 8), pl.n1 / rk};
 }
 bool fft_rows_csalsa_ok(const FftPlan &pl) { return !pl.generic; }
+bool fft_rows_salsa0_ok(const FftPlan &pl) { return !pl.generic && pl.wave; }
 static int fft_rows_check(sbtv_ctx *ctx, const FftPlan &pl, int op) {
     if (op == OP_CSALSA && !fft_rows_csalsa_ok(pl)) return fail(ctx, SBTV_ERR_SIZE, "row pass: OP_CSALSA is not built for this plan");
+    if (op == OP_SALSA0 && !fft_rows_salsa0_ok(pl)) return fail(ctx, SBTV_ERR_SIZE, "row pass: OP_SALSA0 is not built for this plan");
     return 0;
 }
 int fft_rows_blocks(const FftPlan &pl) {
@@ -1094,6 +1099,7 @@
         SBTV_ROWS_OP(OP_ATA)
         SBTV_ROWS_OP(OP_GRADF)
         SBTV_ROWS_OP(OP_CSALSA)
+        SBTV_ROWS_OP(OP_SALSA0)
         default: break;
     }
 #undef SBTV_ROWS_OP
diff --git a/semi-blind-image-deblurring-problems-with-tv_amd/csrc/fft_wave.inc b/semi-blind-image-deblurring-problems-with-tv_amd/csrc/fft_wave.inc
--- a/semi-blind-image-deblurring-problems-with-tv_amd/csrc/fft_wave.inc
+++ b/semi-blind-image-deblurring-problems-with-tv_amd/csrc/fft_wave.inc
@@ -235,6 +235,15 @@
     return make_double2(y.x - t0, y.y - t1);
 }
 
+__device__ __forceinline__ double2 g_then_x(double2 xv, double2 bv, double *__restrict__ xdst) {
+#pragma clang fp contract(off)
+    const double2 gv = make_double2(xv.x - bv.x, xv.y - bv.y);
+    double2 go = gv;
+    asm volatile("" : "+v"(go.x), "+v"(go.y));
+    nt_store2(xdst, make_double2(go.x + bv.x, go.y + bv.y));
+    return gv;
+}
+
 template <int LOG2N, int V, int PM>
 __global__ __launch_bounds__(64 * TW, 2) void cols_inv_wave_kernel(const double2 *__restrict__ S, double *__restrict__ x,
                                                                  const double2 *__restrict__ tw_n1,
@@ -243,6 +252,8 @@
     constexpr int n = 1 << LOG2N;
     constexpr bool POST = (PM & 1) != 0, HAS_TRU = (PM & 2) != 0, HAS_XPREV = (PM & 4) != 0;
     constexpr bool NOX = (PM & 32) != 0;
+    constexpr bool XREC = (PM & 256) != 0;
+    static_assert(!XREC || NOX, "the recovered-x store belongs to the NOX bookkeeping");
     static_assert(n == 64 * V, "one wave per column");
     constexpr int REG = xseq_elems(n);
     __shared__ __attribute__((aligned(16))) double2 lds[TW * REG];
@@ -402,7 +413,12 @@
                 bv.x = bv.x + (uv.x - xv.x);
                 bv.y = bv.y + (uv.y - xv.y);
                 *reinterpret_cast<double2 *>(bup + off) = bv;
-                *reinterpret_cast<double2 *>(gp + off) = make_double2(xv.x - bv.x, xv.y - bv.y);
+                if constexpr (XREC) {
+                    const double2 gv = g_then_x(xv, bv, reinterpret_cast<double *>(out + lane + s * 64));
+                    *reinterpret_cast<double2 *>(gp + off) = gv;
+                } else {
+                    *reinterpret_cast<double2 *>(gp + off) = make_double2(xv.x - bv.x, xv.y - bv.y);
+                }
                 if constexpr (HAS_TRU) {
                     const double2 tv = tb[c & 1][q];
                     const double e0 = xv.x - tv.x, e1 = xv.y - tv.y;
@@ -443,6 +459,7 @@
     constexpr int REG = N;
     constexpr bool needH = (OP != OP_NONE);
     constexpr bool CS = (OP == OP_CSALSA);
+    constexpr bool Z0 = (OP == OP_SALSA0);
     constexpr bool needY = (OP == OP_SALSA || OP == OP_RESID || OP == OP_GRADF || OP == OP_GRAD || CS);
     constexpr bool needD = (OP == OP_GRAD);
     constexpr bool needD1 = needD || CS, noAhead = needD || CS;
@@ -489,8 +506,11 @@
     double2 v[V], sn[V], h[V], y[V], d1[needD1 ? V : 1], d2[needD ? V : 1];
     if constexpr (!needD1) d1[0] = z;
     const CsPar cp = CS ? CsPar{p.cs[0], p.cs[1], p.cs[2]} : CsPar{0.0, 0.0, 0.0};
+    double2 z0 = z;
+    if constexpr (Z0) asm volatile("" : "+v"(z0.x), "+v"(z0.y));
     auto apply = [&](double2 V_, double2 H_, double2 Y_, double2 &E_, double2 D2_, double wgt, double (&acc_)[3]) -> double2 {
         if constexpr (CS) return spec_apply_cs(V_, H_, Y_, E_, mu, cp, wgt, acc_);
+        else if constexpr (Z0) return spec_apply<OP_SALSA>(z0, H_, V_, E_, D2_, mu, wgt, acc_);
         else return spec_apply<OP>(V_, H_, Y_, E_, D2_, mu, wgt, acc_);
     };
     auto dd1 = [&](int s) -> double2 & { return d1[needD1 ? s : 0]; };
@@ -535,11 +555,16 @@
                     const double2 dB = csub(P, Q);
                     const double2 B = make_double2(0.5 * dB.y, -0.5 * dB.x);
                     double2 en = needD ? p.D1[hn] : (CS ? p.E[hn] : z);
+                    if constexpr (Z0) {
+                        p.E[uidx(0, l)] = A;
+                        p.E[hn] = B;
+                    }
                     const double2 A2 = apply(A, h[s], needY ? y[s] : z, dd1(s), dd2(s), 1.0, acc);
                     const double2 B2 = apply(B, p.H[hn], needY ? p.Y[hn] : z, en, needD ? p.D2[hn] : z, 1.0, acc);
                     if constexpr (CS) p.E[hn] = en;
                     v[s] = make_double2(A2.x - B2.y, A2.y + B2.x);
                 } else {
+                    if constexpr (Z0) p.E[uidx(k0, l)] = v[s];
                     v[s] = apply(v[s], h[s], needY ? y[s] : z, dd1(s), dd2(s), 2.0, acc);
                 }
                 if constexpr (CS) p.E[uidx(k0, t + s * T)] = d1[s];
@@ -548,6 +573,7 @@
         } else {
 #pragma unroll
             for (int s = 0; s < V; ++s) {
+                if constexpr (Z0) p.E[uidx(k0, t + s * T)] = v[s];
                 v[s] = apply(v[s], h[s], needY ? y[s] : z, dd1(s), dd2(s), 2.0, acc);
                 if constexpr (CS) p.E[uidx(k0, t + s * T)] = d1[s];
             }
@@ -581,6 +607,7 @@
     if constexpr (needH) {
 #pragma unroll
         for (int s = 0; s < V; ++s) {
+            if constexpr (Z0) p.E[uidx(k1, t + s * T)] = v[s];
             v[s] = apply(v[s], h[s], needY ? y[s] : z, dd1(s), dd2(s), 2.0, acc);
             if constexpr (CS) p.E[uidx(k1, t + s * T)] = d1[s];
         }
@@ -592,7 +619,7 @@
 #pragma unroll
         for (int s = 0; s < V; ++s) out[s_tiled(k1, ts + s * T, n1)] = v[s];
     }
-    if constexpr (needY) {
+    if constexpr (needY || Z0) {
         const int lane = threadIdx.x & 63, w = threadIdx.x >> 6;
 #pragma unroll
         for (int c = 0; c < 3; ++c) {
diff --git a/semi-blind-image-deblurring-problems-with-tv_amd/csrc/salsa.hip b/semi-blind-image-deblurring-problems-with-tv_amd/csrc/salsa.hip
--- a/semi-blind-image-deblurring-problems-with-tv_amd/csrc/salsa.hip
+++ b/semi-blind-image-deblurring-problems-with-tv_amd/csrc/salsa.hip
@@ -6,12 +6,44 @@
 
 #include "sbtv_internal.h"
 
+#ifdef SBTV_CALL_STAMPS
+static std::chrono::steady_clock::time_point g_stamp0;
+static double g_stamps[5] = {0, 0, 0, 0, 0};
+#define SBTV_STAMP(i)                                                                                              \
+    do {                                                                                                           \
+        if ((i) == 0) g_stamp0 = std::chrono::steady_clock::now();                                                 \
+        g_stamps[i] = std::chrono::duration<double>(std::chrono::steady_clock::now() - g_stamp0).count();          \
+    } while (0)
+extern "C" void sbtv_diag_call_stamps(double *out) {
+    for (int i = 0; i < 5; ++i) out[i] = g_stamps[i];
+}
+#else
+#define SBTV_STAMP(i) ((void)0)
+#endif
+
 namespace sbtv {
 
 __global__ void salsa_setup_kernel(const double *__restrict__ src, double *__restrict__ par, int npar, int *__restrict__ frozen,
-                                   int batch) {
+                                   int batch, ProxArm arm, int lam0, unsigned *__restrict__ counters) {
     for (int i = threadIdx.x; i < npar; i += blockDim.x) par[i] = src[i];
-    for (int b = threadIdx.x; b < batch; b += blockDim.x) frozen[b] = 0;
+    for (int b = threadIdx.x; b < batch; b += blockDim.x) {
+        frozen[b] = 0;
+        if (arm.ctrl) {
+            ProxCtrl c = arm.ctrl[b];
+            c.k = 0;
+            c.done = 0;
+            c.cur = 0;
+            c.maxiter = arm.maxiter;
+            c.redo = 0;
+            c.f_valid = 0;
+            c.err = 0.0;
+            c.lambda = src[lam0 + b];
+            c.tol = arm.tol;
+            c.tau = arm.tau;
+            arm.ctrl[b] = c;
+            counters[b] = 0u;
+        }
+    }
 }
 
 __global__ __launch_bounds__(256) void salsa_recover_x_kernel(const double *__restrict__ g, const double *__restrict__ bu,
@@ -65,6 +97,9 @@
     int maxiter = 0, lag = 0, nrb = 0, npb = 0, nl_prox = 0;
     bool want_mse = false, crit2 = false, zero_start = false, direct_last_ok = false, direct_last = false, nox = false,
          spec_ok = false, use_graph = false;
+    bool zs = false, fuse0 = false, xrec = false, setup1 = false;
+    int callpath = 0;
+    double *zeros = nullptr;
     double *xbuf[2] = {nullptr, nullptr}, *u = nullptr, *gb[2] = {nullptr, nullptr}, *bub[2] = {nullptr, nullptr};
     double *par = nullptr, *taps_d = nullptr, *mu_d = nullptr, *thr_d = nullptr;
     double *acc = nullptr, *postp = nullptr, *o4 = nullptr;
@@ -91,8 +126,13 @@
     } pend;
 
     int open() {
+        {
+            const char *e = getenv("SBTV_SALSA_CALLPATH");
+            callpath = (e && e[0]) ? atoi(e) & 15 : 15;
+        }
+        setup1 = (callpath & 8) != 0;
         SBTV_TRY(op_open(ctx, "salsa", M, N, batch, "Y", &op));
-        SBTV_TRY(prox_plan(ctx, M, N, batch, &pp));
+        SBTV_TRY(prox_plan(ctx, M, N, batch, &pp, "prox", !setup1));
         P = op.P;
         cnt = P * batch;
         maxiter = opts->maxiter;
@@ -119,6 +159,19 @@
             SBTV_TRY(ws_get_t(ctx, "salsa.g1", cnt, &gb[1]));
         }
         direct_last = direct_last_ok && !nox;
+        zs = (callpath & 1) && zero_start;
+        fuse0 = (callpath & 2) && zero_start && fft_rows_salsa0_ok(op.fp);
+        xrec = (callpath & 4) && nox && direct_last_ok;
+        if (zs) {
+            const size_t zb = std::max(sizeof(double) * P, sizeof(double2) * op.fp.s_img) * (size_t)batch;
+            SBTV_TRY(ws_get_t(ctx, "salsa.zeros", zb / sizeof(double), &zeros));
+            const DevBuf &zd = ctx->ws["salsa.zeros"];
+            if (ctx->salsa_zeros_ptr != zd.p || ctx->salsa_zeros_bytes != zd.bytes) {
+                SBTV_HIP(ctx, hipMemsetAsync(zd.p, 0, zd.bytes, ctx->stream));
+                ctx->salsa_zeros_ptr = zd.p;
+                ctx->salsa_zeros_bytes = zd.bytes;
+            }
+        }
         const size_t nt = (size_t)batch * taille * taille;
         npar = nt + 2 * (size_t)batch;
         SBTV_TRY(ws_get_t(ctx, "salsa.par", npar, &par));
@@ -159,8 +212,9 @@
             par_stage[nt + b] = mu[b];
             par_stage[nt + batch + b] = tau[b] / mu[b];
         }
+        const ProxArm arm{setup1 ? pp.ctrl : nullptr, nullptr, opts->TViters, opts->chambolle_tol, opts->chambolle_tau, nullptr};
         hipLaunchKernelGGL(salsa_setup_kernel, dim3(1), dim3(256), 0, ctx->stream, (const double *)f_par.at(pd), par, (int)npar,
-                           frozen_d, batch);
+                           frozen_d, batch, arm, (int)(nt + batch), pp.counters);
         SBTV_HIP(ctx, hipGetLastError());
         return 0;
     }
@@ -177,7 +231,8 @@
             std::copy(dims, dims + 6, ctx->salsa_h_dims);
             ctx->salsa_h_ptr = (const void *)op.Hs;
         }
-        SBTV_TRY(op_spectrum(ctx, op.fp, yd, nullptr, op.S, op.Ys));
+        if (fuse0) SBTV_TRY(fft_cols_fwd(ctx, op.fp, yd, nullptr, op.S));
+        else SBTV_TRY(op_spectrum(ctx, op.fp, yd, nullptr, op.S, op.Ys));
         h_numA.assign(batch, 0);
         h_numAt.assign(batch, 1);
         ctx->calls += 2LL * batch;
@@ -193,14 +248,22 @@
             SBTV_HIP(ctx, hipMemcpyAsync(g, x, sizeof(double) * cnt, hipMemcpyDeviceToDevice, ctx->stream));
             SBTV_HIP(ctx, hipMemsetAsync(bu, 0, sizeof(double) * cnt, ctx->stream));
         }
-        SBTV_TRY(prox_reset(ctx, pp, thr_d, 1.0, opts->TViters, opts->chambolle_tol, opts->chambolle_tau, false, nullptr));
+        if (!setup1)
+            SBTV_TRY(prox_reset(ctx, pp, thr_d, 1.0, opts->TViters, opts->chambolle_tol, opts->chambolle_tau, false, nullptr));
         obj_prev.assign(batch, 0.0);
         Collect c{};
         if (zero_start) {
             double *accz = nullptr, *postz = nullptr;
             int nz = 0;
-            SBTV_TRY(salsa_zero_start(ctx, yd, want_mse ? td : nullptr, x, u, bu, P, batch, (double)M * (double)N, &accz, &postz,
-                                      &nz));
+            if (zs) {
+                SBTV_TRY(salsa_zero_start(ctx, yd, want_mse ? td : nullptr, nullptr, nullptr, nullptr, P, batch,
+                                          (double)M * (double)N, &accz, &postz, &nz));
+                if (!nox) SBTV_HIP(ctx, hipMemsetAsync(bu, 0, sizeof(double) * cnt, ctx->stream));
+                if (maxiter == 0) SBTV_HIP(ctx, hipMemsetAsync(x, 0, sizeof(double) * cnt, ctx->stream));
+            } else {
+                SBTV_TRY(salsa_zero_start(ctx, yd, want_mse ? td : nullptr, x, u, bu, P, batch, (double)M * (double)N, &accz,
+                                          &postz, &nz));
+            }
             c = Collect{accz, nz, nullptr, 0, postz, nz, nullptr, 0, 0, 0ull, nullptr};
         } else {
             double *tvp = nullptr;
@@ -284,8 +347,10 @@
         const bool timed = eager && ((outer & 31) == 4 || outer == 12);
         slot_tagged[slot] = tagged;
         slot_spec[slot] = spec;
-        double *xn = (direct_last && outer == maxiter) ? x_out : xbuf[slot];
-        const double *xprev = xbuf[slot ^ 1];
+        const bool first0 = zs && outer == 1;
+        const bool store_rec = xrec && outer == maxiter;
+        double *xn = ((direct_last || store_rec) && outer == maxiter) ? x_out : xbuf[slot];
+        const double *xprev = first0 ? zeros : xbuf[slot ^ 1];
         SideJob side{};
         if (pend.valid && spec) {
             const int ps = pend.outer & 1;
@@ -316,15 +381,25 @@
         a.mu = mu_d;
         a.acc = acc;
         a.frozen = frozen_d;
-        SBTV_TRY(fft_cols_fwd_f(ctx, op.fp, u, bub[(outer - 1) & 1], op.S, frozen_d));
-        SBTV_TRY(fft_rows(ctx, op.fp, op.S, op.S, a));
+        if (fuse0 && outer == 1) {
+            a.op = OP_SALSA0;
+            a.Y = nullptr;
+            a.E = op.Ys;
+            a.frozen = nullptr;
+            SBTV_TRY(fft_rows(ctx, op.fp, op.S, op.S, a));
+        } else if (first0) {
+            SBTV_TRY(fft_rows(ctx, op.fp, reinterpret_cast<const double2 *>(zeros), op.S, a));
+        } else {
+            SBTV_TRY(fft_cols_fwd_f(ctx, op.fp, u, bub[(outer - 1) & 1], op.S, frozen_d));
+            SBTV_TRY(fft_rows(ctx, op.fp, op.S, op.S, a));
+        }
         ColsPost cp;
-        cp.u = u;
+        cp.u = first0 ? zeros : u;
         cp.bu = bub[outer & 1];
         cp.g = gb[outer & 1];
         if (nox) {
-            cp.bu_in = bub[(outer - 1) & 1];
-            cp.skip_x = 1;
+            cp.bu_in = first0 ? zeros : bub[(outer - 1) & 1];
+            cp.skip_x = store_rec ? 2 : 1;
         }
         cp.tru = td;
         cp.xprev = crit2 ? xprev : nullptr;
@@ -420,6 +495,7 @@
                     SBTV_TRY(stage_out_copy(ctx, out, src, P, flags));
                 continue;
             }
+            if (xrec && maxiter > 0 && h_nouter[b] == maxiter) continue;
             const int par = h_nouter[b] & 1;
             const bool dev_direct = direct_last_ok;
             double *dst = dev_direct ? out : xbuf[0] + (size_t)b * P;
@@ -472,9 +548,12 @@
         SBTV_TRY(pipelined_loop(ctx, &done, maxiter, lag, true, [&](int k) { return enqueue(k); }, [&](int k) { return process(k); },
                                 [&] { return active > 0; }));
         SBTV_TRY(read_initial());
+        SBTV_STAMP(1);
         SBTV_HIP(ctx, hipEventRecord(ctx->ev[1], ctx->stream));
         SBTV_TRY(result());
+        SBTV_STAMP(2);
         SBTV_HIP(ctx, hipStreamSynchronize(ctx->stream));
+        SBTV_STAMP(3);
         return finish();
     }
 };
@@ -486,6 +565,7 @@
                              const double *x_init, double *x_out, double *objective, double *distance, double *times,
                              double *mses, int *numA, int *numAt, int *n_outer, int flags) {
     if (!ctx) return SBTV_ERR_BADARG;
+    SBTV_STAMP(0);
     if (!tau || !mu) return fail(ctx, SBTV_ERR_BADARG, "SALSA_v2: missing required argument");
     SBTV_TRY(check_common(ctx, "SALSA_v2", y, taps, opts, x_init, M, N, batch, taille, "x_init", true, false));
     for (int b = 0; b < batch; ++b)
@@ -502,9 +582,11 @@
     SBTV_TRY(stage_in(ctx, "salsa.y", y, cnt, flags, &yd));
     SBTV_TRY(stage_in(ctx, "salsa.true", true_x, cnt, flags, &td));
     SBTV_TRY(stage_in(ctx, "salsa.xinit", x_init, cnt, flags, &xi));
-    return canary_epilogue(ctx, solve_with_exact_repeat(ctx, !(opts->speculate & 2), [&](bool spec) {
+    const int rc_call = canary_epilogue(ctx, solve_with_exact_repeat(ctx, !(opts->speculate & 2), [&](bool spec) {
         SalsaRun r{ctx, yd, M, N, batch, taps, taille, tau, mu, opts, td, xi, x_out, objective, distance, times, mses,
                    numA, numAt, n_outer, flags, spec};
         return r.run();
     }));
-}
+    SBTV_STAMP(4);
+    return rc_call;
+}
diff --git a/semi-blind-image-deblurring-problems-with-tv_amd/csrc/sbtv_internal.h b/semi-blind-image-deblurring-problems-with-tv_amd/csrc/sbtv_internal.h
--- a/semi-blind-image-deblurring-problems-with-tv_amd/csrc/sbtv_internal.h
+++ b/semi-blind-image-deblurring-problems-with-tv_amd/csrc/sbtv_internal.h
@@ -112,6 +112,8 @@
     std::vector<double> salsa_h_taps;
     long long salsa_h_dims[6] = {0, 0, 0, 0, 0, 0};
     const void *salsa_h_ptr = nullptr;
+    const void *salsa_zeros_ptr = nullptr;
+    size_t salsa_zeros_bytes = 0;
     std::map<int, double2 *> twiddles;
     std::map<int, double2 *> any_axes;
     bool any_attr_done = false;
@@ -388,7 +390,7 @@
     const int *order;
     int esub_off;
 };
-int prox_plan(sbtv_ctx *ctx, int M, int N, int batch, ProxPlan *plan, const char *tag = "prox");
+int prox_plan(sbtv_ctx *ctx, int M, int N, int batch, ProxPlan *plan, const char *tag = "prox", bool clear_counters = true);
 int prox_reset(sbtv_ctx *ctx, const ProxPlan &pl, const double *lambda_dev, double lambda_scale,
                int maxiter, double tol, double tau, bool keep_cur, const int *frozen);
 int prox_zero_duals(sbtv_ctx *ctx, const ProxPlan &pl);
@@ -456,6 +458,7 @@
     OP_ATA = 7,
     OP_GRADF = 8,
     OP_CSALSA = 9,
+    OP_SALSA0 = 10,
 };
 struct FftPlan {
     int M, N, batch;
@@ -516,6 +519,7 @@
 int fft_rows(sbtv_ctx *ctx, const FftPlan &pl, const double2 *Sin, double2 *Sout, const RowsArgs &a);
 int fft_rows_blocks(const FftPlan &pl);
 bool fft_rows_csalsa_ok(const FftPlan &pl);
+bool fft_rows_salsa0_ok(const FftPlan &pl);
 int spec_unpack(sbtv_ctx *ctx, const FftPlan &pl, const double2 *S, double2 *U);
 int psf_spectrum(sbtv_ctx *ctx, const FftPlan &pl, const double *taps_dev, int taille, double2 *U);
 int psf_spectrum_sets(sbtv_ctx *ctx, const FftPlan &pl, const double *const *taps_dev, int taille, double2 *const *U, int nsets);
diff --git a/semi-blind-image-deblurring-problems-with-tv_amd/csrc/tv.hip b/semi-blind-image-deblurring-problems-with-tv_amd/csrc/tv.hip
--- a/semi-blind-image-deblurring-problems-with-tv_amd/csrc/tv.hip
+++ b/semi-blind-image-deblurring-problems-with-tv_amd/csrc/tv.hip
@@ -585,7 +585,7 @@
 
 static inline bool vec_ok(const void *p, int M) { return (M % 2 == 0) && ((reinterpret_cast<uintptr_t>(p) & 15) == 0); }
 
-int prox_plan(sbtv_ctx *ctx, int M, int N, int batch, ProxPlan *pl, const char *tag) {
+int prox_plan(sbtv_ctx *ctx, int M, int N, int batch, ProxPlan *pl, const char *tag, bool clear_counters) {
     pl->M = M;
     pl->N = N;
     pl->batch = batch;
@@ -680,7 +680,7 @@
         }
     }
     SBTV_TRY(ws_get_t(ctx, (t + ".counters").c_str(), (size_t)batch, &pl->counters));
-    SBTV_HIP(ctx, hipMemsetAsync(pl->counters, 0, sizeof(unsigned) * batch, ctx->stream));
+    if (clear_counters) SBTV_HIP(ctx, hipMemsetAsync(pl->counters, 0, sizeof(unsigned) * batch, ctx->stream));
     return 0;
 }
 
```

Result: no change. 4685 SALSA outer-iterations/s (-0.7%).
